# jinlinyi/PerspectiveFields

Measured on AMD Instinct MI355X. Metric: images/sec (640x640, Paramnet-360Cities), higher is better.
Workload: dtype f32 (operands fp32 in HBM; contractions as 2-way fp16 split on the MFMA, fp32 accumulate, fp32-class accuracy); 1 GPU; BASELINE configs[2]: batch 32/GPU 640x640 Paramnet-360Cities-edina-centered, fields + ParamNet, 320x320 network inputs resident in HBM (4 distinct synthetic images tiled over the batch; the network is data independent), post-process to 640x640; global_batch=32, parallelism=dp1 (images sharded, all-gather of ParamNet scalars), weights=seeded synthetic checkpoint (no network for the trained .pth), precision=fp32, tiles=shipped tile table + static heuristic (no tuning), gathered_param_rows=32

## Files before the change

include/pf_hip.h:

```cpp
#ifndef PF_HIP_H
#define PF_HIP_H

#include <stddef.h>
#include <stdint.h>

#ifdef __cplusplus
extern "C" {
#endif

typedef struct pf_engine* pf_handle;

enum pf_status {
  PF_OK = 0,
  PF_ERR_ARG = -1,
  PF_ERR_DEVICE = -2,
  PF_ERR_WEIGHTS = -3,
  PF_ERR_WORKSPACE = -4
};

enum pf_arch {
  PF_ARCH_PARAMNET_CENTERED = 0,
  PF_ARCH_PERSNET_CLS = 1,
  PF_ARCH_PARAMNET_UNCENTERED = 2
};

#define PF_NET_SIZE 320
#define PF_PARAMS_STRIDE 8
#define PF_MAX_BATCH 81

const char* pf_version(void);
const char* pf_build_digest(void);
const char* pf_last_error(pf_handle h);

#define PF_DEVICE_NONE (-1)
int pf_create(pf_handle* out, int device, int arch);
int pf_destroy(pf_handle h);

int pf_load_tensor(pf_handle h, const char* key, const float* h_data, const int64_t* shape, int rank);
int pf_finalize_weights(pf_handle h);

int pf_output_info(pf_handle h, int* gravity_channels, int* latitude_channels, int* param_raw_outputs);

int pf_max_batch(void);

size_t pf_workspace_bytes(pf_handle h, int batch);

#define PF_PRECISION_FP32 0
#define PF_PRECISION_FP32_BF16X6 3
int pf_set_precision(pf_handle h, int mode);

int pf_set_saturation_counter(pf_handle h, void* d_counter_u32);
int pf_static_window_max(pf_handle h, float* out);

int pf_forward_u8(pf_handle h, int batch, const uint8_t* d_images_u8, float* d_pred_gravity, float* d_pred_latitude,
                  float* d_params, void* d_workspace, size_t workspace_bytes, void* stream);
int pf_forward_f32(pf_handle h, int batch, const float* d_images_f32, float* d_pred_gravity, float* d_pred_latitude,
                   float* d_params, void* d_workspace, size_t workspace_bytes, void* stream);

int pf_set_defer_params(pf_handle h, int on);
int pf_join_params(pf_handle h, void* stream);

int pf_forward_u8_graph(pf_handle h, int batch, const uint8_t* d_images_u8, float* d_pred_gravity, float* d_pred_latitude,
                        float* d_params, void* d_workspace, size_t workspace_bytes, void* stream);

size_t pf_resize_workspace_bytes(int H, int W);
int pf_resize_bilinear_u8(pf_handle h, const uint8_t* d_img, int H, int W, uint8_t* d_out_320, void* d_workspace,
                          size_t workspace_bytes, void* stream);

int pf_resize_batch_u8(pf_handle h, int batch, const uint8_t* const* h_imgs, const int32_t* h_hw, uint8_t* d_out_320,
                       void* d_workspace, size_t workspace_bytes, void* stream);

size_t pf_autotune_workspace_bytes(pf_handle h, int batch);
int pf_autotune(pf_handle h, int batch, const uint8_t* d_images_u8, float* d_pred_gravity, float* d_pred_latitude,
                float* d_params, void* d_workspace, size_t workspace_bytes, void* stream);
int pf_is_tuned(pf_handle h, int batch);
int pf_load_tile_table(pf_handle h, const char* path);
int pf_save_tile_table(pf_handle h, const char* path);

int pf_postprocess(pf_handle h, const float* d_pred_gravity, const float* d_pred_latitude, int H, int W,
                   float* d_up_out, float* d_lat_out, void* d_workspace, size_t workspace_bytes, void* stream);

#define PF_PROFILE_CLASSES 8
#define PF_PROFILE_LARGE_ONLY 0x80000000u
int pf_profile_begin(pf_handle h, unsigned class_mask);
int pf_profile_pause(pf_handle h);
int pf_profile_end(pf_handle h, double* ms, double* work, long* launches, int n);
int pf_profile_records(pf_handle h, int max_records, int* cat, double* work, float* ms, int* mnk);
#define PF_PROFILE_PHASES 5
#define PF_PHASE_BACKBONE 0
#define PF_PHASE_LOW_LEVEL 1
#define PF_PHASE_DECODERS 2
#define PF_PHASE_PARAMNET 3
#define PF_PHASE_POSTPROCESS 4
int pf_profile_phases(pf_handle h, int n, double* ms);

size_t pf_debug_tap_bytes(pf_handle h, int batch);
int pf_debug_forward_u8(pf_handle h, int batch, const uint8_t* d_in_u8, float* d_pred_gravity, float* d_pred_latitude, float* d_params, void* d_workspace,
                        size_t workspace_bytes, int flags, void* d_tap_buf, size_t tap_bytes, void* stream);
int pf_debug_taps(pf_handle h, int max_records, char* names , long long* byte_offsets, int* shapes );
int pf_debug_ranges(pf_handle h, int max_records, char* names , long long* elems, float* stats );

#define PF_DISPATCH_BATCH 0
#define PF_DISPATCH_S3_SPLIT_TAKEN 1
#define PF_DISPATCH_RB_LAUNCHES 2
#define PF_DISPATCH_SPLITK_LAUNCHES 3
#define PF_DISPATCH_SPLITK_MAX_FACTOR 4
#define PF_DISPATCH_WINO_LAUNCHES 5
#define PF_DISPATCH_WINO_HALF_LAUNCHES 6
#define PF_DISPATCH_THIN128_LAUNCHES 7
#define PF_DISPATCH_ATTN64_LAUNCHES 8
#define PF_DISPATCH_MIT_MLP_FUSED_LAUNCHES 9
#define PF_DISPATCH_LN_KERNEL_LAUNCHES 10
#define PF_DISPATCH_CONV_LAUNCHES 11
#define PF_DISPATCH_SB_TENSORS 12
#define PF_DISPATCH_FORKS 13
#define PF_DISPATCH_FORK_ALLOC_CONFLICTS 14
#define PF_DISPATCH_REAL_PEAK_BYTES 15
#define PF_DISPATCH_DRY_PEAK_BYTES 16
#define PF_DISPATCH_CNX_RB_LAUNCHES 17
#define PF_DISPATCH_COLS 18
int pf_last_dispatch(pf_handle h, int64_t* out, int n);

int pf_postprocess_batch(pf_handle h, int batch, const float* d_pred_gravity, const float* d_pred_latitude, const int32_t* h_hw,
                         float* const* h_up_out, float* const* h_lat_out, void* d_workspace, size_t workspace_bytes, void* stream);

int pf_fields_from_params(int device, const float* d_cam5, int H, int W, float* d_up, float* d_lat, void* stream);

#define PF_FIT_COL_ROLL 0
#define PF_FIT_COL_PITCH 1
#define PF_FIT_COL_VFOV 2
#define PF_FIT_COL_REL_FOCAL 3
#define PF_FIT_COL_GENERAL_VFOV 4
#define PF_FIT_COL_REL_CX 5
#define PF_FIT_COL_REL_CY 6
#define PF_FIT_COL_RMS_UP 7
#define PF_FIT_COL_RMS_LAT 8
#define PF_FIT_COL_COST 9
#define PF_FIT_COL_ITERATIONS 10
#define PF_FIT_COL_CONVERGED 11
#define PF_FIT_COL_VALID_PIXELS 12
#define PF_FIT_COLS 13
#define PF_FIT_LOSS_L2 0
#define PF_FIT_LOSS_HUBER 1
size_t pf_fit_camera_workspace_bytes(int batch, const int32_t* h_hw);
int pf_fit_camera(int device, int batch, const int32_t* h_hw, const float* const* h_up, const float* const* h_lat, const float* d_init,
                  int free_pp, int loss, float huber_delta_deg, float w_up, float w_lat, int max_iter, float* d_out, void* d_workspace,
                  size_t workspace_bytes, void* stream);

#define PF_USMFIT_COL_ROLL 0
#define PF_USMFIT_COL_PITCH 1
#define PF_USMFIT_COL_VFOV 2
#define PF_USMFIT_COL_REL_FOCAL 3
#define PF_USMFIT_COL_GENERAL_VFOV 4
#define PF_USMFIT_COL_REL_CX 5
#define PF_USMFIT_COL_REL_CY 6
#define PF_USMFIT_COL_RMS_UP 7
#define PF_USMFIT_COL_RMS_LAT 8
#define PF_USMFIT_COL_COST 9
#define PF_USMFIT_COL_ITERATIONS 10
#define PF_USMFIT_COL_CONVERGED 11
#define PF_USMFIT_COL_VALID_PIXELS 12
#define PF_USMFIT_COL_XI 13
#define PF_USMFIT_COLS 14
size_t pf_fit_camera_usm_workspace_bytes(int batch, const int32_t* h_hw);
int pf_fit_camera_usm(int device, int batch, const int32_t* h_hw, const float* const* h_up, const float* const* h_lat,
                      const float* d_init , int free_pp, int loss, float huber_delta_deg, float w_up, float w_lat,
                      int max_iter, float* d_out , void* d_workspace, size_t workspace_bytes, void* stream);

int pf_fields_from_params_usm(int device, const float* d_cam6, int H, int W, float* d_up, float* d_lat, void* stream);

#define PF_PANO_U8 0
#define PF_PANO_F32 1
int pf_pano_crop(int device, int n_pano, const void* const* h_pano, const int32_t* h_pano_hw , int dtype, int batch,
                 const int32_t* h_pano_index , const float* d_cam7 , int H, int W,
                 void* d_img , float* d_up , float* d_lat , void* stream);

#define PF_FERR_COL_UP_MEAN 0
#define PF_FERR_COL_UP_MEDIAN 1
#define PF_FERR_COL_UP_RMSE 2
#define PF_FERR_COL_UP_MAX 3
#define PF_FERR_COL_UP_FRAC_BELOW 4
#define PF_FERR_COL_LAT_MEAN 5
#define PF_FERR_COL_LAT_MEDIAN 6
#define PF_FERR_COL_LAT_RMSE 7
#define PF_FERR_COL_LAT_MAX 8
#define PF_FERR_COL_LAT_FRAC_BELOW 9
#define PF_FERR_COL_VALID_PIXELS 10
#define PF_FERR_COLS 11
#define PF_FERR_BINS 11520
#define PF_FERR_BINS_PER_DEG 64
#define PF_FERR_SUM_N 0
#define PF_FERR_SUM_E 1
#define PF_FERR_SUM_E2 2
#define PF_FERR_SUM_MAX 3
#define PF_FERR_SUM_BELOW 4
#define PF_FERR_SUMS 5
size_t pf_field_errors_workspace_bytes(int batch, const int32_t* h_hw);
int pf_field_errors(int device, int batch, const int32_t* h_hw, const float* const* h_up_pred, const float* const* h_lat_pred,
                    const float* const* h_up_gt, const float* const* h_lat_gt, float threshold_deg, double* d_out, float* const* h_err_up,
                    float* const* h_err_lat, int64_t* d_hist, double* d_hist_sums, void* d_workspace, size_t workspace_bytes, void* stream);

int pf_op_set_saturation_watch(void* d_counter_u32, float limit);
int pf_op_conv2d(int device, const float* d_x, const float* d_x2, int B, int H, int W, int C1, int C2,
                 const float* h_weight , const float* h_bias ,
                 int Cout, int KH, int KW, int stride, int pad, int act ,
                 const float* d_res1, const float* d_res2, int post_relu, int nchw_out, int tile_id ,
                 float* d_y ,
                 const uint16_t* d_x_planes , long x_plane_elems, const uint16_t* d_x2_planes, long x2_plane_elems,
                 uint16_t* d_y_planes, long y_plane_elems, int precision , void* stream);
int pf_op_linear_ln(int device, const float* d_x, long rows, int K, const float* h_weight , const float* h_bias, const float* h_gamma, const float* h_beta,
                    float eps, int N, int act, const float* d_res1, int tile_id, float* d_y, int precision, void* stream);
int pf_op_rb_linear(int device, const float* d_x, long rows, int tokens, int K, const float* h_weight , const float* h_bias, const float* h_gamma, const float* h_beta,
                    float eps, int N, int act, const float* d_res, float* d_y, int iters, float* ms_out, void* stream);
int pf_op_rb_proj_fc1(int device, const float* d_attn, float* d_x, int B, int tokens, int C, const float* h_proj_w, const float* h_proj_b, const float* h_ln2_gamma,
                      const float* h_ln2_beta, float eps, const float* h_fc1_w, const float* h_fc1_b, float* d_hidden, int iters, float* ms_out, void* stream);
int pf_op_mit_attn64(int device, const float* d_x, const float* d_kv, float* d_y, int B, int N, int M, const float* h_ln1_gamma, const float* h_ln1_beta, float eps,
                     const float* h_q_w, const float* h_q_b, const float* h_proj_w, const float* h_proj_b, int iters, float* ms_out, void* stream);
int pf_op_stem7x7(int device, const float* d_x, float* d_y, int B, int H, int W, int stride, const float* h_weight, const float* h_bias, int relu, const float* h_ln_gamma,
                  const float* h_ln_beta, float eps, int iters, float* ms_out, void* stream);
int pf_op_thin128(int device, const float* d_x, long rows, const float* h_weight, const float* h_bias, const float* d_res, float* d_y, int iters, float* ms_out, void* stream);
int pf_op_rb_srkv(int device, const float* d_x, int B, int Hr, int Wr, int C, const float* h_ln1_gamma, const float* h_ln1_beta, float eps1, const float* h_sr_w,
                  const float* h_sr_b, const float* h_srn_gamma, const float* h_srn_beta, float eps2, const float* h_kv_w, const float* h_kv_b, float* d_kv, int iters,
                  float* ms_out, void* stream);
int pf_op_cnx_mlp(int device, const float* d_d, float* d_y, long rows, int C, const float* h_w1, const float* h_b1, const float* h_ln_gamma, const float* h_ln_beta,
                  float eps, const float* h_w2, const float* h_b2, const float* h_layer_scale, int iters, float* ms_out, void* stream);
int pf_op_mit_mlp(int device, const float* d_x, float* d_y, int B, int Hs, int Ws, int C, const float* h_fc1_w, const float* h_fc1_b, const float* h_ln_gamma,
                  const float* h_ln_beta, float eps, const float* h_dw_w, const float* h_dw_b, const float* h_fc2_w, const float* h_fc2_b, int iters, float* ms_out, void* stream);
int pf_op_conv2d_bench(int device, int B, int H, int W, int Cin, int Cout, int K, int stride, int pad, int tile_id, int iters, int fmt_prec, float* ms_out);
int pf_op_split_bf16(int device, const float* d_x, long n, uint16_t* d_planes, long plane_elems, void* stream);
int pf_op_merge_bf16(int device, const uint16_t* d_planes, long plane_elems, long n, float* d_y, void* stream);
int pf_op_dwconv3x3_bench(int device, int variant, int B, int H, int W, int C, int iters, float* ms_out);
int pf_op_layernorm(int device, const float* d_x, const float* h_gamma, const float* h_beta, float* d_y, long rows, int C, float eps,
                    uint16_t* d_y_planes, long plane_elems, void* stream);
int pf_op_dwconv3x3_gelu(int device, const float* d_x, const float* h_weight , const float* h_bias, float* d_y, int B, int H, int W, int C,
                         uint16_t* d_y_planes, long plane_elems, void* stream);
int pf_op_dwconv3x3_gelu_cfg(int device, const float* d_x, const float* h_weight, const float* h_bias, float* d_y, int B, int H, int W, int C,
                             uint16_t* d_y_planes, long plane_elems, int variant, void* stream);
int pf_op_dwconv7x7(int device, const float* d_x, const float* h_weight , const float* h_bias, float* d_y, int B, int H, int W, int C, void* stream);
int pf_op_dwconv7x7_cfg(int device, const float* d_x, const float* h_weight, const float* h_bias, float* d_y, int B, int H, int W, int C,
                        int variant, int nc, int nb, int th, void* stream);
int pf_op_dwconv7x7_bench(int device, int variant, int nc, int nb, int th, int B, int H, int W, int C, int iters, float* ms_out);
int pf_op_sr_attention(int device, const float* d_q, const float* d_kv, float* d_out, int B, int N, int M, int heads,
                       uint16_t* d_out_planes, long plane_elems, void* stream);
int pf_op_sr_attention_variant(int device, int variant, const float* d_q, const float* d_kv, float* d_out, int B, int N, int M, int heads,
                               int iters, float* ms_out, void* stream);
int pf_op_upsample2x(int device, const float* d_x, float* d_y, int B, int H, int W, int C, uint16_t* d_y_planes, long plane_elems, void* stream);
int pf_op_num_conv_tiles(void);
const char* pf_op_conv_tile_name(int tile_id);

#ifdef __cplusplus
}
#endif
#endif
```

perspectivefields_amd/csrc/engine.hip:

```cpp
#include <hip/hip_runtime.h>

#include <algorithm>
#include <cmath>
#include <cstdarg>
#include <cstdio>
#include <cstdlib>
#include <cstring>
#include <map>
#include <string>
#include <unordered_map>
#include <vector>

#include "../../include/pf_hip.h"
#include "pf_kernels.h"

using namespace pf;

namespace {

}
namespace pf_host { thread_local std::string g_create_error; }
#include "host_pack.h"
using namespace pf_host;
namespace {
// ... 125 lines not shown
  bool on = false;
  unsigned mask = 0xffffffffu;
  double min_work = 0.0;
  hipEvent_t get() {
    if (used == pool.size()) { hipEvent_t e; if (hipEventCreate(&e) != hipSuccess) return nullptr; pool.push_back(e); }
    return pool[used++];
  }
  struct Mark { int phase; hipEvent_t e; };
  std::vector<Mark> marks;
  void mark(int phase, hipStream_t s) {
    if (!on || min_work > 0.0) return;
    hipEvent_t e = get();
    if (!e) return;
    (void)hipEventRecord(e, s);
    marks.push_back({phase, e});
  }
  void reset() { recs.clear(); marks.clear(); used = 0; }
  ~Profiler() { for (hipEvent_t e : pool) (void)hipEventDestroy(e); }
};
struct ProfScope {
  Profiler* p; hipStream_t s; hipEvent_t b = nullptr;
  ProfScope(Profiler* pr, hipStream_t st, int cat, double work, int m = 0, int n = 0, int k = 0, int kh = 0) : p(pr), s(st) {
    if (!p || !p->on || !((p->mask >> cat) & 1u) || work < p->min_work) { p = nullptr; return; }
    hipEvent_t a = p->get(); b = p->get();
    if (!a || !b) { p = nullptr; return; }
    (void)hipEventRecord(a, s);
    p->recs.push_back({cat, work, a, b, m, n, k, kh, 0.f});
  }
  ~ProfScope() { if (p) (void)hipEventRecord(b, s); }
};

struct ResizeTable { int ksize = 0; std::vector<int> bounds, kk; int *d_bounds = nullptr, *d_kk = nullptr; };
void resize_coeffs(int in_size, int out_size, ResizeTable* t) {
  const double scale = (double)in_size / out_size;
  const double filterscale = scale < 1.0 ? 1.0 : scale;
  const double support = 1.0 * filterscale;
  const int ksize = (int)std::ceil(support) * 2 + 1;
  t->ksize = ksize;
  t->bounds.assign((size_t)out_size * 2, 0);
  t->kk.assign((size_t)out_size * ksize, 0);
  std::vector<double> k(ksize);
  const double ss = 1.0 / filterscale;
  for (int xx = 0; xx < out_size; ++xx) {
    const double center = (xx + 0.5) * scale;
    double ww = 0.0;
    int xmin = (int)(center - support + 0.5);
    if (xmin < 0) xmin = 0;
    int xmax = (int)(center + support + 0.5);
    if (xmax > in_size) xmax = in_size;
    xmax -= xmin;
    for (int x = 0; x < ksize; ++x) k[x] = 0.0;
    for (int x = 0; x < xmax; ++x) {
      double v = (x + xmin - center + 0.5) * ss;
      if (v < 0.0) v = -v;
      const double w = v < 1.0 ? 1.0 - v : 0.0;
      k[x] = w;
      ww += w;
    }
    for (int x = 0; x < xmax; ++x)
      if (ww != 0.0) k[x] /= ww;
    for (int x = 0; x < ksize; ++x)
      t->kk[(size_t)xx * ksize + x] = k[x] < 0 ? (int)(-0.5 + k[x] * (1 << 22)) : (int)(0.5 + k[x] * (1 << 22));
    t->bounds[2 * xx] = xmin;
    t->bounds[2 * xx + 1] = xmax;
  }
}

}

struct pf_engine {
  int device = 0;
  int arch = 0;
  bool finalized = false;
  std::string err;
  std::unordered_map<std::string, HostTensor> host;
  std::vector<void*> dev_allocs;
  std::map<int, size_t> ws_cache;
  Profiler prof;
  bool autotune = false;
  std::map<std::vector<int>, int> tile_cache;
  std::map<int, bool> tuned_batches;
  std::map<int, ResizeTable> resize_tables;
  std::map<int, size_t> scratch_off, scratch_elems;
  bool split_bf16 = true;
  bool fuse_pred = true;
  bool fuse_upsample = true;
  bool fuse_ln = true;
  int thin128 = 25600;
  int stem7 = 1;
  unsigned short* ll_s7_w = nullptr; float* ll_s7_tab = nullptr; unsigned short* pe_s7_w = nullptr; float* pe_s7_tab = nullptr;
  int attn64 = 1;
  int s3_split = 1;
  int side_stream_mode = 1;
  hipStream_t side = nullptr, side2 = nullptr;
  hipEvent_t ev_fork = nullptr, ev_join = nullptr, ev_ll = nullptr;
  bool host_only = false;
  int defer_params = 0;
  hipStream_t pstream = nullptr;
  hipEvent_t ev_pn_in = nullptr, ev_pn_done = nullptr;
  bool pn_pending = false, in_capture = false;
  int pn_pending_B = 0; uintptr_t pn_pending_base = 0;
  int defer_at = 0, defer_prio = 0;
  struct PnLater { bool armed = false; int B = 0; const float* pn = nullptr; float* params = nullptr; Ctx ctx; } pn_later;
  void issue_deferred() {
    if (!pn_later.armed) return;
    pn_later.armed = false;
    paramnet(pn_later.ctx, pn_later.B, pn_later.pn, pn_later.params);
    (void)hipEventRecord(ev_pn_done, pstream);
  }
  std::map<int, size_t> pn_off;
  bool pstream_ready() {
    if (pstream) return true;
    int lo = 0, hi = 0;
    (void)hipDeviceGetStreamPriorityRange(&lo, &hi);
    const int prio = defer_prio > 0 ? hi : (defer_prio < 0 ? lo : 0);
    if ((defer_prio ? hipStreamCreateWithPriority(&pstream, hipStreamNonBlocking, prio) : hipStreamCreateWithFlags(&pstream, hipStreamNonBlocking)) != hipSuccess) { pstream = nullptr; return false; }
    if (hipEventCreateWithFlags(&ev_pn_in, hipEventDisableTiming) != hipSuccess || hipEventCreateWithFlags(&ev_pn_done, hipEventDisableTiming) != hipSuccess) {
      (void)hipStreamDestroy(pstream); pstream = nullptr; return false;
    }
    return true;
  }
  bool ll_forked = false;
  bool side_ready() {
    if (side && (side2 || side_stream_mode < 2)) return true;
    if (!side) {
      if (hipStreamCreateWithFlags(&side, hipStreamNonBlocking) != hipSuccess) { side = nullptr; return false; }
      if (hipEventCreateWithFlags(&ev_fork, hipEventDisableTiming) != hipSuccess || hipEventCreateWithFlags(&ev_join, hipEventDisableTiming) != hipSuccess ||
          hipEventCreateWithFlags(&ev_ll, hipEventDisableTiming) != hipSuccess) return false;
    }
    if (side_stream_mode >= 2 && !side2 && hipStreamCreateWithFlags(&side2, hipStreamNonBlocking) != hipSuccess) { side2 = nullptr; return false; }
    return true;
  }
  struct ForkWin { bool open = false, side_alloced = false; size_t nalloc0 = 0; };
  ForkWin fw_q, fw_ll;
  Ctx fork_open(Ctx& c, hipStream_t s, ForkWin& w) {
    Ctx c2 = c;
    c2.s = s;
    w.open = true; w.side_alloced = false; w.nalloc0 = c.nalloc;
    c.count(PF_DISPATCH_FORKS);
    return c2;
  }
  void fork_side_done(ForkWin& w, const Ctx& c2) { w.side_alloced = c2.nalloc > w.nalloc0; }
  void fork_join(Ctx& c, ForkWin& w) {
    if (!w.open) return;
    if (w.side_alloced && c.nalloc > w.nalloc0) c.count(PF_DISPATCH_FORK_ALLOC_CONFLICTS);
    w.open = false;
  }
  int64_t dispatch[PF_DISPATCH_COLS] = {};
  int splitk_mode = -1;
  int wino_half = 1;
  bool can_fork(const Ctx& c) { return side_stream_mode && !c.dry && !c.tuning && (!c.prof || c.prof->min_work > 0.0) && side_ready(); }
  bool sba_heads = false;
  int rb_chain = 60;
  int rb_min_blocks = 192;
  int num_cus = 256;
  int wino_min_hw = 20;
  int wino_min_blocks = 96;
  int wino_tile = -1;
  unsigned* d_sat = nullptr;
  float static_window_max = 0.f;
  int mit_mlp128 = 4;
  bool fuse_mit_mlp = true;
  bool fuse_cnx_mlp = true;
  int cnx_rb = 1;
  int cnx_rb_min_blocks[2] = {96, 192};
  bool fold_mlp = true;
  int nterms = NT_F16X3;
  DebugSink dbg;
  DebugSink* debug_sink = nullptr;
  struct GraphEntry { std::vector<uintptr_t> key; hipGraphExec_t exec; };
  std::vector<GraphEntry> graphs;
  bool sba = false;

  MitStage stages[4];
  ConvW ll;
  Head heads[2];
  Cnx cnx;
  bool has_param = false;
  int param_in = NET;
  float mean3[3] = {103.53f, 116.28f, 123.675f};
  float std3[3] = {1.f, 1.f, 1.f};

  int fail(int code, const std::string& m) { err = m; return code; }

  ResizeTable* resize_table(int in_size) {
    auto it = resize_tables.find(in_size);
    if (it != resize_tables.end()) return &it->second;
    ResizeTable& t = resize_tables[in_size];
    resize_coeffs(in_size, NET, &t);
    void *db = nullptr, *dk = nullptr;
    if (hipMalloc(&db, t.bounds.size() * 4) != hipSuccess || hipMalloc(&dk, t.kk.size() * 4) != hipSuccess) return nullptr;
    if (hipMemcpy(db, t.bounds.data(), t.bounds.size() * 4, hipMemcpyHostToDevice) != hipSuccess ||
        hipMemcpy(dk, t.kk.data(), t.kk.size() * 4, hipMemcpyHostToDevice) != hipSuccess) return nullptr;
    dev_allocs.push_back(db); dev_allocs.push_back(dk);
    t.d_bounds = static_cast<int*>(db); t.d_kk = static_cast<int*>(dk);
    return &t;
  }
  float* upload(const std::vector<float>& v) {
    void* d = nullptr;
    if (host_only) {
      d = malloc(v.size() * sizeof(float) + 1);
      if (!d) throw std::string("malloc failed for weights");
      std::memcpy(d, v.data(), v.size() * sizeof(float));
      dev_allocs.push_back(d);
      return static_cast<float*>(d);
    }
    if (hipMalloc(&d, v.size() * sizeof(float)) != hipSuccess) throw std::string("hipMalloc failed for weights");
    if (hipMemcpy(d, v.data(), v.size() * sizeof(float), hipMemcpyHostToDevice) != hipSuccess) throw std::string("hipMemcpy H2D failed for weights");
    dev_allocs.push_back(d);
    return static_cast<float*>(d);
  }
  unsigned short* upload_u16(const std::vector<unsigned short>& v) {
    void* d = nullptr;
    if (host_only) {
      d = malloc(v.size() * 2 + 1);
      if (!d) throw std::string("malloc failed for weights");
      std::memcpy(d, v.data(), v.size() * 2);
      dev_allocs.push_back(d);
      return static_cast<unsigned short*>(d);
    }
    if (hipMalloc(&d, v.size() * 2) != hipSuccess) throw std::string("hipMalloc failed for weights");
    if (hipMemcpy(d, v.data(), v.size() * 2, hipMemcpyHostToDevice) != hipSuccess) throw std::string("hipMemcpy H2D failed for weights");
    dev_allocs.push_back(d);
    return static_cast<unsigned short*>(d);
  }
  void upload_conv_weights(ConvW& c, const std::vector<float>& packed, int CinP, int Cout) {
    c.w = upload(packed);
    if (split_bf16 && (CinP % 32 == 0 || CinP == 4)) {
      c.wsb = upload_u16(split_bf16x3(packed));
      const F16Planes f = split_f16x2(packed, Cout);
      c.wh16 = upload_u16(f.planes);
      c.wh16_inv = upload(f.inv_scale);
    }
  }
  const HostTensor& get(const std::string& key, std::initializer_list<int64_t> shape) {
    auto it = host.find(key);
    if (it == host.end()) throw fmt("missing checkpoint tensor '%s'", key.c_str());
    HostTensor& t = it->second;
    if (t.shape != std::vector<int64_t>(shape)) {
      std::string got, want;
      for (auto d : t.shape) got += std::to_string(d) + ",";
      for (auto d : shape) want += std::to_string(d) + ",";
      throw fmt("shape mismatch for '%s': got (%s) expected (%s)", key.c_str(), got.c_str(), want.c_str());
    }
    t.used = true;
    return t;
  }
  ConvW make_conv(const std::string& wkey, const std::string& bkey, int Cout, int Cin, int K, int stride, int pad,
                  const double* out_scale = nullptr, const std::vector<float>* bias_override = nullptr) {
    ConvW c;
    const int CinP = roundup(Cin, 4);
    const HostTensor& w = get(wkey, {Cout, Cin, K, K});
    const std::vector<float> packed = pack_conv(w.data.data(), Cout, Cin, K, K, CinP, out_scale, &c.KWC, &c.KWCp);
    upload_conv_weights(c, packed, CinP, Cout);
    if (bias_override) c.b = upload(*bias_override);
    else if (!bkey.empty()) {
      std::vector<float> b = get(bkey, {Cout}).data;
      if (out_scale) for (int n = 0; n < Cout; ++n) b[n] = (float)(b[n] * out_scale[n]);
      c.b = upload(b);
    }
    c.Cout = Cout; c.Cin = CinP; c.CinReal = Cin; c.KH = c.KW = K; c.stride = stride; c.pad = pad;
    if (wino_min_hw > 0 && split_bf16 && K == 3 && stride == 1 && pad == 1 && CinP % 64 == 0 && Cout % 64 == 0 && c.KWCp == c.KWC) {
      std::vector<unsigned short> planes;
      std::vector<float> inv;
      wino_pack_weights(packed.data(), Cout, CinP, c.KWCp, &planes, &inv);
      c.wwino = upload_u16(planes);
      c.wwino_inv = upload(inv);
    }
    return c;
  }
  ConvW make_linear(const std::string& pfx, int N, int K, const double* out_scale = nullptr, const std::string& ln_pfx = "", float ln_eps = 0.f) {
    ConvW c;
    const HostTensor& w = get(pfx + ".weight", {N, K});
    std::vector<float> b = get(pfx + ".bias", {N}).data;
    if (!ln_pfx.empty() && fuse_ln && K % 32 == 0 && N % 4 == 0) {
      const std::vector<float>& g = get(ln_pfx + ".weight", {K}).data;
      const std::vector<float>& be = get(ln_pfx + ".bias", {K}).data;
      std::vector<float> wf, bf, cs;
      fold_ln_linear(w.data.data(), b.data(), g.data(), be.data(), N, K, &wf, &bf, &cs);
      b = bf;
      upload_conv_weights(c, pack_conv(wf.data(), N, K, 1, 1, K, nullptr, &c.KWC, &c.KWCp), K, N);
      c.ln_s = upload(cs);
      c.ln_eps = ln_eps;
    } else {
      upload_conv_weights(c, pack_conv(w.data.data(), N, K, 1, 1, K, out_scale, &c.KWC, &c.KWCp), K, N);
      if (out_scale) for (int n = 0; n < N; ++n) b[n] = (float)(b[n] * out_scale[n]);
    }
    c.b = upload(b);
    c.Cout = N; c.Cin = K; c.CinReal = K; c.KH = c.KW = 1; c.stride = 1; c.pad = 0;
    return c;
  }
  ConvW make_folded(const std::string& lin, const std::string& proc, int C) {
    const HostTensor& wl = get(lin + ".weight", {DEC_EMBED, C});
    const HostTensor& bl = get(lin + ".bias", {DEC_EMBED});
    const HostTensor& wp = get(proc + ".weight", {DEC_FEAT, DEC_EMBED, 3, 3});
    const HostTensor& bp = get(proc + ".bias", {DEC_FEAT});
    std::vector<float> wf((size_t)DEC_FEAT * C * 9);
    std::vector<double> T((size_t)DEC_FEAT * 9), acc(C);
    std::vector<double> wld(wl.data.begin(), wl.data.end());
    for (int o = 0; o < DEC_FEAT; ++o)
      for (int t = 0; t < 9; ++t) {
        std::fill(acc.begin(), acc.end(), 0.0);
        double tb = 0.0;
        for (int e = 0; e < DEC_EMBED; ++e) {
          const double a = wp.data[((size_t)o * DEC_EMBED + e) * 9 + t];
          const double* row = &wld[(size_t)e * C];
// ... 385 lines not shown
      std::vector<int> key = {p.M, p.Cout, p.KH, p.KW, p.Cin, p.stride, p.H, p.W, ngroups, p.nchw_out, fmt_bits + 512 * p.ln, p.act};
      auto it = tile_cache.find(key);
      if (it == tile_cache.end() && p.ln && !(c.tuning && c.tune_scratch)) { key[10] = fmt_bits; it = tile_cache.find(key); }
      if (it != tile_cache.end()) tile = it->second;
      else if (c.tuning && c.tune_scratch) { tile = tune_conv(p, c); tile_cache[key] = tile; }
    }
    if (!conv_tile_usable(p, tile)) tile = conv_default_tile(p);
    if (wino_min_hw > 0 && wino_tile >= 0 && !(c.tuning && c.tune_scratch) && p.Ho >= wino_min_hw && p.Wo >= wino_min_hw && conv_tile_usable(p, wino_tile) &&
        conv_wino_blocks(p) >= wino_min_blocks) tile = wino_tile;
    if (c.dbg && c.dbg->range) {
      const int q = c.dbg->seq++;
      for (int g = 0; g < ngroups; ++g) {
        const std::string nm = fmt("dense%03d%s %dx%d s%d %s%sM=%d N=%d K=%d", q, ngroups > 1 ? (g ? "[latitude]" : "[gravity]") : "", w.KH, w.KW, w.stride, w.ln_s ? "LN-fused " : "", tile >= 0 && strncmp(conv_tile_name(tile), "wino", 4) == 0 ? "[winograd] " : "", p.M, p.Cout, w.KH * w.KW * w.CinReal);
        range_in(c, nm + " x", calls[g].x.f, (size_t)B * (ups ? H / 2 : H) * (ups ? W / 2 : W) * p.C1);
        if (p.C2 > 0) range_in(c, nm + " x2", calls[g].x2.f, (size_t)B * H * W * p.C2);
      }
    }
    ProfScope ps(c.prof, c.s, conv_tile_is_sb(tile) ? PC_IGEMM_SB : PC_IGEMM, 2.0 * ngroups * p.M * (double)w.Cout * w.KH * w.KW * w.CinReal, p.M * ngroups, w.Cout, w.KH * w.KW * w.CinReal, w.KH);
    c.count(PF_DISPATCH_CONV_LAUNCHES);
    launch_conv_tile(p, tile, c.s);
  }
  int tune_conv(const ConvParams& p0, Ctx& c) {
    ConvParams p = p0;
    const size_t out_elems = (size_t)p.M * p.Cout;
    unsigned short* sb_scratch = reinterpret_cast<unsigned short*>(c.tune_scratch + c.tune_scratch_elems);
    for (int g = 0; g < p.groups; ++g) {
      if (p.g[g].y) p.g[g].y = c.tune_scratch + g * out_elems;
      if (p.g[g].y_sb) p.g[g].y_sb = sb_scratch + g * out_elems;
    }
    p.y_sb_plane = (c.tune_scratch_elems & ~(size_t)1) | (p0.y_sb_plane & 1);
    hipEvent_t a, b;
    if (hipEventCreate(&a) != hipSuccess || hipEventCreate(&b) != hipSuccess) return -1;
    int best = -1;
    float best_ms = 1e30f;
    for (int t = 0; t < conv_num_tiles(); ++t) {
      if (!conv_tile_usable(p, t)) continue;
      if (strncmp(conv_tile_name(t), "sbhA", 4) == 0 || strncmp(conv_tile_name(t), "sbhLA", 5) == 0 || strncmp(conv_tile_name(t), "sbhDMA", 6) == 0 || strncmp(conv_tile_name(t), "sbhREG", 6) == 0 || strncmp(conv_tile_name(t), "sbhV", 4) == 0 || strncmp(conv_tile_name(t), "sbA", 3) == 0 || strncmp(conv_tile_name(t), "sbPI_", 5) == 0 || strncmp(conv_tile_name(t), "sbI_", 4) == 0) continue;
      if (strncmp(conv_tile_name(t), "wino", 4) == 0) continue;
      if (conv_tile_bn(t) > 32 && p.Cout <= 32) continue;
      if ((long)conv_tile_bm(t) * conv_tile_bn(t) > 16L * p.M * p.Cout) continue;
      launch_conv_tile(p, t, c.s);
      float ms = 1e30f;
      bool ok = true;
      for (int rep = 0; rep < 2 && ok; ++rep) {
        (void)hipEventRecord(a, c.s);
        launch_conv_tile(p, t, c.s);
        launch_conv_tile(p, t, c.s);
        (void)hipEventRecord(b, c.s);
        ok = hipEventSynchronize(b) == hipSuccess;
        float w = 0.f;
        if (ok) { (void)hipEventElapsedTime(&w, a, b); ms = std::min(ms, w); }
      }
      if (!ok) break;
      if (ms < best_ms) { best_ms = ms; best = t; }
    }
    (void)hipEventDestroy(a); (void)hipEventDestroy(b);
    return best;
  }
  void conv(Ctx& c, const ConvW& w, Ten x, int B, int H, int W, Ten y, int act = ACT_NONE, const float* res1 = nullptr,
            const float* res2 = nullptr, int post_relu = 0, Ten x2 = Ten(), int C1 = -1, int nchw = 0) {
    ConvCall one{&w, x, y, res1, res2, x2};
    conv_g(c, 1, &one, B, H, W, act, post_relu, C1, nchw);
  }
  void gemm(Ctx& c, const ConvW& w, Ten x, long rows, Ten y, int act = ACT_NONE, const float* res1 = nullptr) {
    conv(c, w, x, 1, (int)rows, 1, y, act, res1);
  }
  void ln(Ctx& c, const LNW& l, const float* x, Ten y, long rows) {
    if (c.dry) return;
    c.count(PF_DISPATCH_LN_KERNEL_LAUNCHES);
    ProfScope ps(c.prof, c.s, PC_LAYERNORM, (4.0 + (y.f ? 4.0 : 0.0) + (y.s.p ? 6.0 : 0.0)) * rows * l.C);
    launch_layernorm(x, l.g, l.b, y.f, rows, l.C, l.eps, c.s, y.s.p, y.s.plane);
  }

  void rb_linear(Ctx& c, const RbLin& r, const float* x, long M, int tokens, float* y, const LNW* lnw = nullptr, int act = ACT_NONE, const float* res = nullptr) {
    range_in(c, fmt("rb_linear %d->%d%s", r.K, r.N, lnw ? " (LN input)" : ""), x, (size_t)M * r.K);
    if (c.dry) return;
    RbLinArgs a;
    a.x = x; a.ln_g = lnw ? lnw->g : nullptr; a.ln_b = lnw ? lnw->b : nullptr; a.ln_eps = lnw ? lnw->eps : 0.f;
    a.w = r.w; a.w_bytes = r.bytes; a.inv = r.inv; a.bias = r.b; a.res = res; a.y = y;
    a.M = (int)M; a.tokens = tokens; a.bpi = (tokens + 63) / 64; a.N = r.N; a.act = act;
    a.sat = d_sat; a.sat_limit = r.sat_limit;
    ProfScope ps(c.prof, c.s, PC_IGEMM_SB, 2.0 * M * (double)r.N * r.K, (int)M, r.N, r.K, 1);
    c.count(PF_DISPATCH_RB_LAUNCHES);
    launch_rb_linear(a, r.K, c.s);
  }

  void thin(Ctx& c, const unsigned short* wfr, const float* tab, const float* x, const float* res, float* y, long M, float sat_limit, const char* what) {
    range_in(c, fmt("thin128 %s x", what), x, (size_t)M * 128);
    if (c.dry) return;
    ThinLinArgs a;
    a.x = x; a.res = res; a.y = y; a.wfr = wfr; a.tab = tab; a.M = M; a.sat = d_sat; a.sat_limit = sat_limit;
    ProfScope ps(c.prof, c.s, PC_IGEMM_SB, 2.0 * M * 128.0 * 128.0, (int)M, 128, 128, 1);
    c.count(PF_DISPATCH_THIN128_LAUNCHES);
    launch_thin128(a, num_cus, c.s);
  }

  void stem(Ctx& c, const unsigned short* wfr, const float* tab, const float* x4, float* y, int B, int H, int W, int stride, bool relu, bool lnorm, float eps, float sat_limit, const char* what) {
    range_in(c, fmt("stem7x7 s%d %s x", stride, what), x4, (size_t)B * H * W * 4);
    if (c.dry) return;
    Stem7Args a;
    a.x = x4; a.y = y; a.wfr = wfr; a.tab = tab; a.B = B; a.H = H; a.W = W; a.stride = stride; a.Ho = (H + 6 - 7) / stride + 1; a.Wo = (W + 6 - 7) / stride + 1;
    a.relu = relu ? 1 : 0; a.ln = lnorm ? 1 : 0; a.ln_eps = eps; a.sat = lnorm ? nullptr : d_sat; a.sat_limit = sat_limit;
    const long M = (long)B * a.Ho * a.Wo;
    ProfScope ps(c.prof, c.s, PC_IGEMM_SB, 2.0 * M * 64.0 * 147.0, (int)M, 64, 147, 7);
    launch_stem7x7(a, num_cus, c.s);
  }

  void mit(Ctx& c, int B, const float* x0, Ten feats[4], const Ten* llf = nullptr) {
    const bool S = sba;
    Ten cur(const_cast<float*>(x0));
    int H = NET, W = NET;
    for (int s = 0; s < 4; ++s) {
      MitStage& st = stages[s];
      if (!c.dry && pn_later.armed && s + 1 == defer_at) issue_deferred();
      const int C = MIT_DIMS[s], heads_n = MIT_HEADS[s], sr = MIT_SR[s];
      const int Ho = (H + 2 * MIT_PP[s] - MIT_PK[s]) / MIT_PS[s] + 1, Wo = (W + 2 * MIT_PP[s] - MIT_PK[s]) / MIT_PS[s] + 1;
      const long N = (long)Ho * Wo, M = (long)B * N;
      float* x = c.alloc(M * C);
      const bool fused_mlp = !st.blocks.empty() && st.blocks[0].mlp_w && nterms == NT_F16X3 && (C != 128 || B >= mit_mlp128);
      float* xalt = fused_mlp ? c.alloc(M * C) : nullptr;
      const SbT xs = S ? c.alloc_sb(M * C) : SbT();
      if (s == 2 && llf && B >= 4 && side_stream_mode >= 2 && can_fork(c)) {
        (void)hipEventRecord(ev_ll, c.s);
        (void)hipStreamWaitEvent(side2, ev_ll, 0);
        Ctx c2 = fork_open(c, side2, fw_ll);
        conv(c2, ll, Ten(const_cast<float*>(x0)), B, NET, NET, *llf, ACT_RELU);
        (void)hipEventRecord(ev_ll, side2);
        fork_side_done(fw_ll, c2);
        ll_forked = true;
      }
      if (s == 0 && pe_s7_w && nterms == NT_F16X3 && !c.tuning && cur.f) {
        stem(c, pe_s7_w, pe_s7_tab, cur.f, x, B, H, W, MIT_PS[s], false, true, st.pen.eps, 65504.f, "patch_embed1 + norm");
      } else {
        conv(c, st.pe, cur, B, H, W, Ten(x));
        ln(c, st.pen, x, Ten(x), M);
      }
      const size_t mk = c.mark();
      const int kvh = Ho / sr, kvw = Wo / sr;
      const long Mkv = (long)B * kvh * kvw;
      const Ten xn = c.ten(M * C, !S, S);
      float* qb = c.alloc(M * C);
      const Ten ab = c.ten(M * C, !S, S);
      float* srb = c.alloc(Mkv * C);
      const Ten srn = S ? Ten(nullptr, c.alloc_sb(Mkv * C)) : Ten(srb);
      float* kvb = c.alloc(Mkv * 2 * C);
      float* hb = c.alloc(M * 4 * C);
      const Ten h2 = c.ten(M * 4 * C, !S, S);
      auto one_block = [&](Ctx& c, MitBlock& mb, int blk, int B, long M, long Mkv, float*& x, float*& xalt, const Ten& xn, float* qb, const Ten& ab, float* srb, const Ten& srn,
                           float* kvb, float* hb, const Ten& h2, int gate_B, bool may_fork) {
        const bool thin_q = mb.tq_w && M >= thin128 && nterms == NT_F16X3 && !S && !c.tuning && xn.f;
        const bool fuse64 = attn64 && mb.a64_w && nterms == NT_F16X3 && !S && !c.tuning && sr > 1;
        const long rb_blocks = (long)gate_B * ((N + 63) / 64);
        const bool use_rb = rb_chain && mb.rq.w && nterms == NT_F16X3 && !S && !c.tuning && rb_blocks >= rb_min_blocks && (rb_blocks % num_cus == 0 || rb_blocks % num_cus >= num_cus * 3 / 4);
        if (sr > 1 && use_rb && (rb_chain & 32) && mb.rsrkv.w && mb.qln.ln_s && fuse_ln) {
          const bool fork = B >= 4 && (may_fork && can_fork(c));
          if (fork) {
            (void)hipEventRecord(ev_fork, c.s);
            (void)hipStreamWaitEvent(side, ev_fork, 0);
            Ctx c2 = fork_open(c, side, fw_q);
            gemm(c2, mb.qln, Ten(x), M, Ten(qb));
            (void)hipEventRecord(ev_join, side);
            fork_side_done(fw_q, c2);
          } else {
            gemm(c, mb.qln, Ten(x), M, Ten(qb));
          }
          range_in(c, fmt("rb_srkv s%d.b%d x (LN-fused)", s + 1, blk), x, (size_t)M * C);
          if (!c.dry) {
            RbSrKvArgs a;
            a.x = x; a.ln1_g = mb.n1.g; a.ln1_b = mb.n1.b; a.ln1_eps = mb.n1.eps;
            a.w = mb.rsrkv.w; a.w_bytes = mb.rsrkv.bytes; a.sr_inv = mb.rsrkv.sr_inv; a.sr_bias = mb.rsrkv.sr_b;
            a.srn_g = mb.srn.g; a.srn_b = mb.srn.b; a.srn_eps = mb.srn.eps; a.kv_inv = mb.rsrkv.kv_inv; a.kv_bias = mb.rsrkv.kv_b;
            a.kv = kvb; a.B = B; a.Hr = kvh; a.Wr = kvw; a.bpi = (kvh * kvw + 31) / 32; a.sat = d_sat;
            ProfScope ps(c.prof, c.s, PC_IGEMM_SB, 2.0 * Mkv * (double)C * (sr * sr * C + 2 * C), (int)Mkv, 3 * C, sr * sr * C + 2 * C, sr);
            c.count(PF_DISPATCH_RB_LAUNCHES);
            launch_rb_srkv(a, C, c.s);
          }
        } else if (sr > 1 && fuse64) {
          ln(c, mb.n1, x, xn, M);
          conv(c, mb.sr, xn, B, Ho, Wo, Ten(srb));
          if (mb.kv.ln_s) {
            gemm(c, mb.kv, Ten(srb), Mkv, Ten(kvb));
          } else {
            ln(c, mb.srn, srb, srn, Mkv);
            gemm(c, mb.kv, srn, Mkv, Ten(kvb));
          }
        } else if (sr > 1) {
          const bool fork = B >= 4 && (may_fork && can_fork(c));
          if (use_rb && (rb_chain & 1) && fork) {
            (void)hipEventRecord(ev_fork, c.s);
            (void)hipStreamWaitEvent(side, ev_fork, 0);
            Ctx c2 = fork_open(c, side, fw_q);
            rb_linear(c2, mb.rq, x, M, (int)N, qb, &mb.n1);
            (void)hipEventRecord(ev_join, side);
            fork_side_done(fw_q, c2);
          }
          ln(c, mb.n1, x, xn, M);
          if (use_rb && (rb_chain & 1)) {
            if (!fork) rb_linear(c, mb.rq, x, M, (int)N, qb, &mb.n1);
          } else if (fork) {
            (void)hipEventRecord(ev_fork, c.s);
            (void)hipStreamWaitEvent(side, ev_fork, 0);
            Ctx c2 = fork_open(c, side, fw_q);
            if (thin_q) thin(c2, mb.tq_w, mb.tq_tab, xn.f, nullptr, qb, M, mb.q.sat_limit, "q"); else gemm(c2, mb.q, xn, M, Ten(qb));
            (void)hipEventRecord(ev_join, side);
            fork_side_done(fw_q, c2);
          } else {
            if (thin_q) thin(c, mb.tq_w, mb.tq_tab, xn.f, nullptr, qb, M, mb.q.sat_limit, "q"); else gemm(c, mb.q, xn, M, Ten(qb));
          }
          conv(c, mb.sr, xn, B, Ho, Wo, Ten(srb));
          if (use_rb && (rb_chain & 2)) {
            rb_linear(c, mb.rkv, srb, Mkv, kvh * kvw, kvb, &mb.srn);
          } else if (mb.kv.ln_s) {
            gemm(c, mb.kv, Ten(srb), Mkv, Ten(kvb));
          } else {
            ln(c, mb.srn, srb, srn, Mkv);
            gemm(c, mb.kv, srn, Mkv, Ten(kvb));
          }
        } else if (mb.q.ln_s && mb.kv.ln_s) {
          if (B >= 4 && (may_fork && can_fork(c))) {
            (void)hipEventRecord(ev_fork, c.s);
            (void)hipStreamWaitEvent(side, ev_fork, 0);
            Ctx c2 = fork_open(c, side, fw_q);
            gemm(c2, mb.q, Ten(x), M, Ten(qb));
            (void)hipEventRecord(ev_join, side);
            fork_side_done(fw_q, c2);
          } else {
            gemm(c, mb.q, Ten(x), M, Ten(qb));
          }
          gemm(c, mb.kv, Ten(x), M, Ten(kvb));
        } else {
          ln(c, mb.n1, x, xn, M);
          gemm(c, mb.q, xn, M, Ten(qb));
          gemm(c, mb.kv, xn, M, Ten(kvb));
        }
        if (!fuse64 && B >= 4 && (sr > 1 || (mb.q.ln_s && mb.kv.ln_s)) && (may_fork && can_fork(c))) (void)hipStreamWaitEvent(c.s, ev_join, 0);
        if (may_fork) fork_join(c, fw_q);
        if (c.dbg && c.dbg->range) {
          if (!fuse64) range_in(c, fmt("attention s%d.b%d q", s + 1, blk), qb, (size_t)M * C);
          range_in(c, fmt("attention s%d.b%d kv", s + 1, blk), kvb, (size_t)Mkv * 2 * C);
        }
        if (fuse64) {
          range_in(c, fmt("mit_attn64 s%d.b%d x (LN-fused)", s + 1, blk), x, (size_t)M * C);
          if (!c.dry) {
            MitAttn64Args a;
            a.x = x; a.kv = kvb; a.y = x; a.wfr = mb.a64_w; a.tab = mb.a64_tab; a.B = B; a.N = (int)N; a.M = kvh * kvw; a.ln_eps = mb.n1.eps; a.sat = d_sat; a.sat_limit = mb.proj.sat_limit;
            ProfScope ps(c.prof, c.s, PC_ATTN, 4.0 * M * C * (double)C + 4.0 * M * C * (kvh * kvw));
            c.count(PF_DISPATCH_ATTN64_LAUNCHES);
            launch_mit_attn64(a, num_cus, c.s);
          }
        }
        const bool pf_fused = !fuse64 && use_rb && (rb_chain & 64) && mb.rpf.w;
        if (!fuse64) {
        if (!c.dry) {
          ProfScope ps(c.prof, c.s, PC_ATTN, 4.0 * M * C * (kvh * kvw));
          launch_sr_attention(qb, kvb, ab.f, B, (int)N, kvh * kvw, heads_n, c.s, ab.s.p, ab.s.plane);
        }
        if (pf_fused) {
          range_in(c, fmt("rb_proj_fc1 s%d.b%d attn", s + 1, blk), ab.f, (size_t)M * C);
          if (!c.dry) {
            RbProjFc1Args a;
            a.attn = ab.f; a.x = x; a.w = mb.rpf.w; a.w_bytes = mb.rpf.bytes; a.proj_inv = mb.rproj.inv; a.proj_bias = mb.rproj.b;
            a.ln2_g = mb.n2.g; a.ln2_b = mb.n2.b; a.ln2_eps = mb.n2.eps; a.fc1_inv = mb.rfc1.inv; a.fc1_bias = mb.rfc1.b; a.hidden = hb;
            a.B = B; a.tokens = (int)N; a.bpi = ((int)N + 63) / 64; a.sat = d_sat; a.sat_limit = mb.rproj.sat_limit; a.hidden_limit = mb.rfc1.sat_limit;
            ProfScope ps(c.prof, c.s, PC_IGEMM_SB, 2.0 * M * (double)C * 5 * C, (int)M, 5 * C, C, 1);
            c.count(PF_DISPATCH_RB_LAUNCHES);
            launch_rb_proj_fc1(a, C, c.s);
          }
        } else if (use_rb && (rb_chain & 4)) rb_linear(c, mb.rproj, ab.f, M, (int)N, x, nullptr, ACT_NONE, x);
        else if (thin_q && mb.tp_w && ab.f) thin(c, mb.tp_w, mb.tp_tab, ab.f, x, x, M, mb.proj.sat_limit, "proj");
        else gemm(c, mb.proj, ab, M, Ten(x), ACT_NONE, x);
        }
        if (fused_mlp && mb.mlp_w) {
          range_in(c, fmt("mit_mlp s%d.b%d x (LN-fused)", s + 1, blk), x, (size_t)M * C);
          if (!c.dry) {
            ProfScope ps(c.prof, c.s, PC_IGEMM_SB, 2.0 * 2.0 * M * (double)C * 4 * C, (int)M, C, 8 * C, 9);
            c.count(PF_DISPATCH_MIT_MLP_FUSED_LAUNCHES);
            launch_mit_mlp(x, xalt, mb.mlp_w, mb.mlp_tab, B, Ho, Wo, C, mb.n2.eps, c.s, d_sat, 65504.f);
          }
          std::swap(x, xalt);
          return;
        }
        if (pf_fused) {
        } else if (use_rb && (rb_chain & 8)) {
          rb_linear(c, mb.rfc1, x, M, (int)N, hb, &mb.n2);
        } else if (mb.fc1.ln_s) {
          gemm(c, mb.fc1, Ten(x), M, Ten(hb));
        } else {
          ln(c, mb.n2, x, xn, M);
          gemm(c, mb.fc1, xn, M, Ten(hb));
        }
        if (!c.dry) {
          ProfScope ps(c.prof, c.s, PC_DW3, (4.0 + (h2.f ? 4.0 : 0.0) + (h2.s.p ? 6.0 : 0.0)) * M * 4 * C);
          launch_dwconv3x3_gelu(hb, mb.dw.w, mb.dw.b, h2.f, B, Ho, Wo, 4 * C, c.s, h2.s.p, h2.s.plane);
        }
        if (use_rb && (rb_chain & 16)) rb_linear(c, mb.rfc2, h2.f, M, (int)N, x, nullptr, ACT_NONE, x);
        else gemm(c, mb.fc2, h2, M, Ten(x), ACT_NONE, x);
            };
      const long rb_all = (long)B * ((N + 63) / 64), rb_half = rb_all / 2;
      auto rb_gate = [&](long nb) { return nb >= rb_min_blocks && (nb % num_cus == 0 || nb % num_cus >= num_cus * 3 / 4); };
      bool split = s3_split && s == 2 && sr > 1 && !S && !fused_mlp && B >= 16 && B % 2 == 0 && !c.dry && !c.dbg && !c.tuning && !st.blocks.empty() && rb_chain && nterms == NT_F16X3 &&
                         st.blocks[0].rq.w && rb_gate(rb_all) && (s3_split >= 2 || rb_gate(rb_half)) && can_fork(c);
      if (split) {
        Ctx probe = c;
        probe.dry = true; probe.rep = nullptr;
        float *px = x, *none = nullptr;
        one_block(probe, st.blocks[0], 0, B / 2, M / 2, Mkv / 2, px, none, xn, qb, ab, srb, srn, kvb, hb, h2, B, false);
        if (probe.nalloc != c.nalloc) split = false;
      }
      int blk = -1;
      if (split) {
        const int Bh = B / 2;
        const long Mh = M / 2, Mkvh = Mkv / 2;
        c.count(PF_DISPATCH_S3_SPLIT_TAKEN);
        (void)hipEventRecord(ev_fork, c.s);
        (void)hipStreamWaitEvent(side, ev_fork, 0);
        Ctx c2 = fork_open(c, side, fw_q);
        float* x2 = x + Mh * C;
        float* none = nullptr;
        for (MitBlock& mb : st.blocks) {
          ++blk;
          one_block(c, mb, blk, Bh, Mh, Mkvh, x, none, xn, qb, ab, srb, srn, kvb, hb, h2, B, false);
          one_block(c2, mb, blk, Bh, Mh, Mkvh, x2, none, Ten(xn.f ? xn.f + Mh * C : nullptr), qb + Mh * C, Ten(ab.f + Mh * C), srb + Mkvh * C, Ten(srn.f ? srn.f + Mkvh * C : nullptr),
                    kvb + Mkvh * 2 * C, hb + Mh * 4 * C, Ten(h2.f + Mh * 4 * C), B, false);
        }
        (void)hipEventRecord(ev_join, side);
        (void)hipStreamWaitEvent(c.s, ev_join, 0);
        fork_side_done(fw_q, c2);
        fork_join(c, fw_q);
      } else {
        for (MitBlock& mb : st.blocks) {
          if (blk >= 0) tap(c, fmt("mit.s%d.b%d", s + 1, blk), x, B, Ho, Wo, C);
          ++blk;
          one_block(c, mb, blk, B, M, Mkv, x, xalt, xn, qb, ab, srb, srn, kvb, hb, h2, B, true);
        }
      }
      c.release(mk);
      if (blk >= 0) tap(c, fmt("mit.s%d.b%d", s + 1, blk), x, B, Ho, Wo, C);
      ln(c, st.norm, x, Ten(x, xs), M);
      tap(c, fmt("c%d", s + 1), x, B, Ho, Wo, C);
      feats[s] = Ten(x, xs);
      cur = feats[s];
      H = Ho; W = Wo;
    }
  }

  bool pred_fused() const { return fuse_pred && arch != PF_ARCH_PERSNET_CLS && nterms == NT_F16X3 && split_bf16; }
  void heads_fwd(Ctx& c, int B, Ten feats[4], Ten llf, float* t32 , float* pg, float* pl, float* pn) {
    const bool S = sba && nterms != NT_F16X3;
    const bool SR = S || (sba_heads && !sba && nterms == NT_F16X3 && split_bf16);
    Head& hg = heads[0];
    Head& hl = heads[1];
    auto pair = [&](size_t per_head, bool want_f32, bool want_sb, Ten& a, Ten& b) {
      a = Ten(); b = Ten();
      if (want_f32) { a.f = c.alloc(2 * per_head); b.f = a.f + per_head; }
      if (want_sb) { a.s = c.alloc_sb(2 * per_head); b.s = a.s; b.s.p = a.s.p + per_head; }
    };
    const bool fuse_up = fuse_upsample && nterms == NT_F16X3 && split_bf16 && !S;
    Ten up[4][2], qfin[2];
    for (int k = 3; k >= 0; --k) {
      const int h = NET >> (k + 2);
      if (k == 0 && fuse_up) pair((size_t)B * h * h * DEC_FEAT, true, false, qfin[0], qfin[1]);
      else pair((size_t)B * 4 * h * h * DEC_FEAT, !(S && k == 0), S && k == 0, up[k][0], up[k][1]);
    }
    for (int k = 3; k >= 0; --k) {
      const int h = NET >> (k + 2);
      const size_t M = (size_t)B * h * h;
      const size_t mk = c.mark();
      Ten p0, p1;
      pair(M * DEC_FEAT, true, SR, p0, p1);
      if (fold_mlp) {
        ConvCall cc[2] = {{&hg.fold[k], feats[k], p0}, {&hl.fold[k], feats[k], p1}};
        conv_g(c, 2, cc, B, h, h, ACT_NONE, 1);
      } else {
        Ten e0, e1;
        pair(M * DEC_EMBED, !S, S, e0, e1);
        ConvCall l[2] = {{&hg.lin[k], feats[k], e0}, {&hl.lin[k], feats[k], e1}};
        conv_g(c, 2, l, 1, (int)M, 1);
        ConvCall cc[2] = {{&hg.proc[k], e0, p0}, {&hl.proc[k], e1, p1}};
        conv_g(c, 2, cc, B, h, h, ACT_NONE, 1);
      }
      Ten o0 = p0, o1 = p1;
      if (k < 3) {
        Ten t0, t1;
        pair(M * DEC_FEAT, !SR, SR, t0, t1);
        ConvCall a[2] = {{&hg.r1c1[k], p0, t0}, {&hl.r1c1[k], p1, t1}};
        conv_g(c, 2, a, B, h, h, ACT_RELU);
        pair(M * DEC_FEAT, true, SR, o0, o1);
        ConvCall b2[2] = {{&hg.r1c2[k], t0, o0, p0.f, up[k + 1][0].f}, {&hl.r1c2[k], t1, o1, p1.f, up[k + 1][1].f}};
// ... 139 lines not shown
    else conv(c, ll, Ten(x0), B, NET, NET, llf, ACT_RELU);
    tap(c, "ll", llf.f, B, NET / 2, NET / 2, LL_CH);
    const bool pf = pred_fused();
    float* tg = pf ? nullptr : c.alloc((size_t)2 * B * NET * NET * 32);
    float* tl = pf ? nullptr : tg + (size_t)B * NET * NET * 32;
    Ctx cp = c;
    cp.off = 0; cp.peak = 0;
    if (!c.dry) cp.base = c.base + pn_off[B];
    float* pn = has_param ? cp.alloc((size_t)B * NET * NET * 4) : nullptr;
    if (!c.dry && pn_pending) {
      issue_deferred();
      (void)hipStreamWaitEvent(c.s, ev_pn_done, 0);
      pn_pending = false;
    }
    const size_t mk = c.mark();
    if (!c.dry && c.prof) c.prof->mark(PH_DECODERS, c.s);
    heads_fwd(c, B, feats, llf, tg, pg, pl, pn);
    c.release(mk);
    if (arch == PF_ARCH_PERSNET_CLS) {
      conv(c, heads[0].predcls, Ten(tg), B, NET, NET, Ten(pg), ACT_NONE, nullptr, nullptr, 0, Ten(), -1, 1);
      conv(c, heads[1].predcls, Ten(tl), B, NET, NET, Ten(pl), ACT_NONE, nullptr, nullptr, 0, Ten(), -1, 1);
      if (!c.dry && c.prof) c.prof->mark(PH_END, c.s);
      return;
    }
    if (!c.dry && !pf)
      launch_pred_regression(tg, tl, heads[0].predw, heads[0].predb, heads[1].predw, heads[1].predb, pg, pl, pn, B, NET * NET, c.s);
    if (!c.dry && c.prof) c.prof->mark(has_param ? PH_PARAMNET : PH_END, c.s);
    if (has_param) {
      const bool defer = defer_params && !c.dry && (!c.prof || c.prof->min_work > 0.0) && !c.dbg && !c.tuning && !in_capture && pstream_ready();
      if (defer) {
        (void)hipEventRecord(ev_pn_in, c.s);
        (void)hipStreamWaitEvent(pstream, ev_pn_in, 0);
        cp.s = pstream;
      }
      if (defer && defer_at > 0) {
        pn_later.armed = true; pn_later.B = B; pn_later.pn = pn; pn_later.params = params; pn_later.ctx = cp;
        pn_pending = true; pn_pending_B = B; pn_pending_base = c.base;
      } else {
        paramnet(cp, B, pn, params);
        if (defer) {
          (void)hipEventRecord(ev_pn_done, pstream);
          pn_pending = true; pn_pending_B = B; pn_pending_base = c.base;
        }
      }
    }
    if (!c.dry && c.prof && has_param) c.prof->mark(PH_END, c.s);
    run_pn_peak = cp.peak;
    if (cp.max_conv_out > c.max_conv_out) c.max_conv_out = cp.max_conv_out;
  }
  size_t run_pn_peak = 0;
  std::map<int, size_t> pn_peak;

  size_t workspace_bytes(int B, bool with_scratch = false) {
    auto it = ws_cache.find(B);
    if (it == ws_cache.end()) {
      Ctx c{nullptr, 4096, 0, 0, true, nullptr};
      c.sb_planes = nterms == NT_F16X3 ? 2 : 3;
      run(c, B, nullptr, true, nullptr, nullptr, nullptr);
      const size_t main_peak = (c.peak + 255) & ~(size_t)255, total = main_peak + ((run_pn_peak + 255) & ~(size_t)255);
      pn_off[B] = main_peak;
      pn_peak[B] = (run_pn_peak + 255) & ~(size_t)255;
      ws_cache[B] = total + 4096;
      scratch_off[B] = total;
      scratch_elems[B] = c.max_conv_out;
      it = ws_cache.find(B);
    }
    return it->second + ((with_scratch || autotune) ? scratch_elems[B] * 10 + 4096 : 0);
  }
  int forward(int B, const void* in, bool is_u8, float* pg, float* pl, float* params, void* ws, size_t ws_bytes, hipStream_t s, bool tune = false) {
    if (host_only) return fail(PF_ERR_DEVICE, "this engine was created with PF_DEVICE_NONE (host side only): no forward");
    if (!finalized) return fail(PF_ERR_WEIGHTS, "pf_forward called before pf_finalize_weights");
    if (B <= 0 || !in || !pg || !pl || !ws) return fail(PF_ERR_ARG, "pf_forward: null pointer or batch <= 0");
    if (has_param && !params) return fail(PF_ERR_ARG, "pf_forward: d_params is required for a ParamNet architecture");
    if (B > PF_MAX_BATCH) return fail(PF_ERR_ARG, fmt("pf_forward: batch %d exceeds PF_MAX_BATCH = %d (32-bit byte offsets inside one activation); split the batch", B, PF_MAX_BATCH));
    const size_t need = workspace_bytes(B, tune);
    if (ws_bytes < need) return fail(PF_ERR_WORKSPACE, fmt("workspace too small: %zu < %zu bytes", ws_bytes, need));
    if (hipSetDevice(device) != hipSuccess) return fail(PF_ERR_DEVICE, "hipSetDevice failed");
    uintptr_t base = (reinterpret_cast<uintptr_t>(ws) + 255) & ~(uintptr_t)255;
    Ctx c{s, base, 0, 0, false, nullptr};
    c.sb_planes = nterms == NT_F16X3 ? 2 : 3;
    c.prof = prof.on ? &prof : nullptr;
    c.dbg = debug_sink;
    if (tune) {
      c.tuning = true;
      c.tune_scratch = reinterpret_cast<float*>(base + scratch_off[B]);
      c.tune_scratch_elems = scratch_elems[B];
    }
    std::fill(dispatch, dispatch + PF_DISPATCH_COLS, (int64_t)0);
    if (!tune) c.rep = dispatch;
    const LaunchCounts lc0 = g_launch_counts;
    g_launch_counts.splitk_max = 0;
    fw_q.open = fw_ll.open = false;
    run(c, B, in, is_u8, pg, pl, params);
    const LaunchCounts lc1 = g_launch_counts;
    g_launch_counts.splitk_max = std::max(lc0.splitk_max, lc1.splitk_max);
    dispatch[PF_DISPATCH_BATCH] = B;
    dispatch[PF_DISPATCH_SPLITK_LAUNCHES] = lc1.splitk - lc0.splitk;
    dispatch[PF_DISPATCH_SPLITK_MAX_FACTOR] = lc1.splitk_max;
    dispatch[PF_DISPATCH_WINO_LAUNCHES] = lc1.wino - lc0.wino;
    dispatch[PF_DISPATCH_WINO_HALF_LAUNCHES] = lc1.wino_half - lc0.wino_half;
    const size_t real_main = (c.peak + 255) & ~(size_t)255, real_pn = (run_pn_peak + 255) & ~(size_t)255;
    dispatch[PF_DISPATCH_REAL_PEAK_BYTES] = (int64_t)(real_main + real_pn);
    dispatch[PF_DISPATCH_DRY_PEAK_BYTES] = (int64_t)(pn_off[B] + pn_peak[B]);
    const hipError_t e = hipGetLastError();
    if (e != hipSuccess) return fail(PF_ERR_DEVICE, fmt("kernel launch failed: %s", hipGetErrorString(e)));
    if (real_main > pn_off[B] || real_pn > pn_peak[B])
      return fail(PF_ERR_WORKSPACE, fmt("the forward allocated past what pf_workspace_bytes(%d) sized: main region %zu > %zu or ParamNet region %zu > %zu bytes (the launches were issued: the workspace and outputs of this call are not to be trusted)", B, real_main, pn_off[B], real_pn, pn_peak[B]));
    return PF_OK;
  }
};

static void tune_cache_load(pf_engine* h);
static void tune_cache_save(pf_engine* h);


extern "C" {

const char* pf_version(void) { return "pf_hip 0.2 (gfx950; split-f16 / split-bf16 / fp32 MFMA)"; }

#ifndef PF_BUILD_DIGEST
#define PF_BUILD_DIGEST "unknown"
#endif
const char* pf_build_digest(void) { return PF_BUILD_DIGEST; }

const char* pf_last_error(pf_handle h) { return h ? h->err.c_str() : g_create_error.c_str(); }

int pf_create(pf_handle* out, int device, int arch) {
  if (!out) { g_create_error = "pf_create: out is NULL"; return PF_ERR_ARG; }
  *out = nullptr;
  if (arch < 0 || arch > 2) { g_create_error = fmt("pf_create: unknown arch %d", arch); return PF_ERR_ARG; }
  const bool host_only = device == PF_DEVICE_NONE;
  if (!host_only) {
    const int rc = check_device(device, &g_create_error);
    if (rc != PF_OK) return rc;
  }
  pf_engine* e = new pf_engine();
  e->device = device;
  e->host_only = host_only;
  e->arch = arch;
  if (const char* v = getenv("PF_FOLD_MLP")) e->fold_mlp = atoi(v) != 0;
  if (const char* v = getenv("PF_FUSE_UPSAMPLE")) e->fuse_upsample = atoi(v) != 0;
  if (const char* v = getenv("PF_FUSE_PRED")) e->fuse_pred = atoi(v) != 0;
  if (const char* v = getenv("PF_FUSE_LN")) e->fuse_ln = atoi(v) != 0;
  if (const char* v = getenv("PF_FUSE_CNX_MLP")) e->fuse_cnx_mlp = atoi(v) != 0;
  if (const char* v = getenv("PF_FUSE_MIT_MLP")) e->fuse_mit_mlp = atoi(v) != 0;
  if (const char* v = getenv("PF_MIT_MLP_128")) e->mit_mlp128 = atoi(v);
  if (const char* v = getenv("PF_WINO")) e->wino_min_hw = atoi(v);
  if (const char* v = getenv("PF_WINO_MIN_BLOCKS")) e->wino_min_blocks = atoi(v);
  {
    const char* wt = getenv("PF_WINO_TILE");
    for (int t = 0; t < conv_num_tiles(); ++t) if (strcmp(conv_tile_name(t), wt ? wt : "wino256x64d") == 0) e->wino_tile = t;
  }
  if (const char* v = getenv("PF_RB_CHAIN")) e->rb_chain = atoi(v);
  if (const char* v = getenv("PF_DEFER_AT")) e->defer_at = atoi(v);
  if (const char* v = getenv("PF_DEFER_PRIO")) e->defer_prio = atoi(v);
  if (!host_only) {
    hipDeviceProp_t prop;
    if (hipGetDeviceProperties(&prop, device) == hipSuccess && prop.multiProcessorCount > 0) e->num_cus = prop.multiProcessorCount;
    e->rb_min_blocks = e->num_cus * 3 / 4;
  }
  if (const char* v = getenv("PF_RB_MIN_BLOCKS")) e->rb_min_blocks = atoi(v);
  if (const char* v = getenv("PF_CNX_RB")) e->cnx_rb = atoi(v);
  if (!host_only) { e->cnx_rb_min_blocks[0] = e->num_cus * 3 / 8; e->cnx_rb_min_blocks[1] = e->num_cus * 3 / 4; }
  if (const char* v = getenv("PF_CNX_RB_MIN_BLOCKS")) e->cnx_rb_min_blocks[0] = atoi(v);
  if (const char* v = getenv("PF_CNX_RB_MIN_BLOCKS_768")) e->cnx_rb_min_blocks[1] = atoi(v);
#ifdef PF_TUNING_BUILD
#endif
  if (const char* v = getenv("PF_SIDE_STREAM")) e->side_stream_mode = atoi(v);
  if (const char* v = getenv("PF_S3_SPLIT")) e->s3_split = atoi(v);
  if (const char* v = getenv("PF_ATTN64")) e->attn64 = atoi(v);
  if (const char* v = getenv("PF_STEM7")) e->stem7 = atoi(v);
  if (const char* v = getenv("PF_THIN128")) e->thin128 = atoi(v);
  if (const char* v = getenv("PF_SBA_HEADS")) e->sba_heads = atoi(v) != 0;
  if (const char* v = getenv("PF_AUTOTUNE")) e->autotune = atoi(v) != 0;
  if (const char* v = getenv("PF_SPLIT_BF16")) e->split_bf16 = atoi(v) != 0;
  if (const char* v = getenv("PF_SBA")) e->sba = atoi(v) != 0;
  e->splitk_mode = conv_splitk_env();
  e->wino_half = conv_wino_half_env();
  if (!e->split_bf16) e->sba = false;
  if (!e->split_bf16 || e->sba) e->fuse_ln = false;
  if (!e->split_bf16 || e->sba) e->fuse_cnx_mlp = false;
  if (!e->split_bf16 || e->sba) e->fuse_mit_mlp = false;
  if (!e->split_bf16 || e->sba) e->cnx_rb = 0;

  tune_cache_load(e);
  *out = e;
  return PF_OK;
}

int pf_set_precision(pf_handle h, int mode) {
  if (!h) return PF_ERR_ARG;
  if (mode != PF_PRECISION_FP32 && mode != PF_PRECISION_FP32_BF16X6) return h->fail(PF_ERR_ARG, "pf_set_precision: unknown mode (0 = FP32 split-f16, 3 = FP32_BF16X6; the reduced-precision modes 1 / 2 of earlier versions are gone)");
  if (mode != PF_PRECISION_FP32 && !h->split_bf16) return h->fail(PF_ERR_ARG, "pf_set_precision: this mode needs the split kernels (PF_SPLIT_BF16=0 is set)");
  if (h->pn_pending) { h->issue_deferred(); (void)hipStreamSynchronize(h->pstream); h->pn_pending = false; }
  h->ws_cache.clear();
  h->nterms = mode == PF_PRECISION_FP32_BF16X6 ? 6 : NT_F16X3;
  return PF_OK;
}

int pf_set_saturation_counter(pf_handle h, void* d_counter_u32) {
  if (!h) return PF_ERR_ARG;
  h->d_sat = static_cast<unsigned*>(d_counter_u32);
  return PF_OK;
}
int pf_static_window_max(pf_handle h, float* out) {
  if (!h || !out || !h->finalized) return PF_ERR_ARG;
  *out = h->static_window_max;
  return PF_OK;
}
int pf_set_defer_params(pf_handle h, int on) {
  if (!h) return PF_ERR_ARG;
  h->defer_params = on ? 1 : 0;
  return PF_OK;
}
int pf_join_params(pf_handle h, void* stream) {
  if (!h) return PF_ERR_ARG;
  if (h->pn_pending) h->issue_deferred();
  if (h->pn_pending && hipStreamWaitEvent(static_cast<hipStream_t>(stream), h->ev_pn_done, 0) != hipSuccess) return h->fail(PF_ERR_DEVICE, "pf_join_params: hipStreamWaitEvent failed");
  return PF_OK;
}

int pf_destroy(pf_handle h) {
  if (!h) return PF_ERR_ARG;
  if (h->host_only) {
    for (void* d : h->dev_allocs) free(d);
    delete h;
    return PF_OK;
  }
  (void)hipSetDevice(h->device);
  for (void* d : h->dev_allocs) (void)hipFree(d);
  if (h->dbg.stats) (void)hipFree(h->dbg.stats);
  for (auto& g : h->graphs) (void)hipGraphExecDestroy(g.exec);
  if (h->ev_fork) (void)hipEventDestroy(h->ev_fork);
  if (h->ev_join) (void)hipEventDestroy(h->ev_join);
  if (h->ev_ll) (void)hipEventDestroy(h->ev_ll);
  if (h->side) (void)hipStreamDestroy(h->side);
  if (h->side2) (void)hipStreamDestroy(h->side2);
  if (h->pstream) { (void)hipStreamSynchronize(h->pstream); (void)hipStreamDestroy(h->pstream); }
  if (h->ev_pn_in) (void)hipEventDestroy(h->ev_pn_in);
  if (h->ev_pn_done) (void)hipEventDestroy(h->ev_pn_done);
  delete h;
  return PF_OK;
}

int pf_load_tensor(pf_handle h, const char* key, const float* data, const int64_t* shape, int rank) {
  if (!h || !key || (!data && rank > 0) || rank < 0 || rank > 4) return h ? h->fail(PF_ERR_ARG, "pf_load_tensor: bad argument") : PF_ERR_ARG;
  if (h->finalized) return h->fail(PF_ERR_WEIGHTS, "pf_load_tensor after pf_finalize_weights");
  HostTensor t;
  size_t n = 1;
  for (int i = 0; i < rank; ++i) { if (shape[i] <= 0) return h->fail(PF_ERR_ARG, "pf_load_tensor: non-positive dim"); t.shape.push_back(shape[i]); n *= (size_t)shape[i]; }
  if (data) t.data.assign(data, data + n);
  h->host[key] = std::move(t);
  return PF_OK;
}

int pf_finalize_weights(pf_handle h) {
  if (!h) return PF_ERR_ARG;
  if (h->finalized) return h->fail(PF_ERR_WEIGHTS, "weights already finalized");
  if (!h->host_only && hipSetDevice(h->device) != hipSuccess) return h->fail(PF_ERR_DEVICE, "hipSetDevice failed");
  try {
    h->build();
  } catch (const std::string& m) {
    return h->fail(PF_ERR_WEIGHTS, m);
  }
  h->finalized = true;
  return PF_OK;
}

int pf_output_info(pf_handle h, int* g, int* l, int* p) {
  if (!h) return PF_ERR_ARG;
  const bool cls = h->arch == PF_ARCH_PERSNET_CLS;
  if (g) *g = cls ? 73 : 2;
  if (l) *l = cls ? 180 : 1;
  if (p) *p = cls ? 0 : 5;
  return PF_OK;
}

int pf_max_batch(void) { return PF_MAX_BATCH; }

int pf_last_dispatch(pf_handle h, int64_t* out, int n) {
  if (!h || !out || n < PF_DISPATCH_COLS) return h ? h->fail(PF_ERR_ARG, "pf_last_dispatch: the array must hold PF_DISPATCH_COLS entries") : PF_ERR_ARG;
  std::copy(h->dispatch, h->dispatch + PF_DISPATCH_COLS, out);
  return PF_OK;
}

size_t pf_workspace_bytes(pf_handle h, int batch) {
  if (!h || batch <= 0 || batch > PF_MAX_BATCH) return 0;
  const bool was = h->has_param;
  if (!h->finalized) {
    h->has_param = h->arch != PF_ARCH_PERSNET_CLS;
    h->param_in = h->arch == PF_ARCH_PARAMNET_UNCENTERED ? 64 : NET;
    for (int s = 0; s < 4; ++s)
      if (h->stages[s].blocks.empty()) h->stages[s].blocks.resize(MIT_DEPTHS[s]);
    if (h->has_param)
      for (int s = 0; s < 4; ++s)
        if (h->cnx.blocks[s].empty()) h->cnx.blocks[s].resize(CNX_DEPTHS[s]);
  }
  const size_t n = h->workspace_bytes(batch);
  if (!h->finalized) {
    h->has_param = was;
    for (int s = 0; s < 4; ++s) { h->stages[s].blocks.clear(); h->cnx.blocks[s].clear(); }
    h->ws_cache.clear();
  }
  return n;
}

// ... 541 lines not shown
```

perspectivefields_amd/csrc/engine_ops.hip:

```cpp
#include "host_pack.h"

using namespace pf;
using namespace pf_host;

static thread_local unsigned* t_op_sat = nullptr;
static thread_local float t_op_sat_limit = 65504.f;

extern "C" {

int pf_op_set_saturation_watch(void* d_counter_u32, float limit) {
  if (d_counter_u32 && !(limit > 0.f)) { g_create_error = "pf_op_set_saturation_watch: limit must be positive"; return PF_ERR_ARG; }
  t_op_sat = static_cast<unsigned*>(d_counter_u32);
  t_op_sat_limit = d_counter_u32 ? limit : 65504.f;
  return PF_OK;
}

int pf_op_num_conv_tiles(void) { return conv_num_tiles(); }
const char* pf_op_conv_tile_name(int id) { return conv_tile_name(id); }

int pf_op_conv2d(int device, const float* x, const float* x2, int B, int H, int W, int C1, int C2, const float* hw, const float* hb,
                 int Cout, int KH, int KW, int stride, int pad, int act, const float* res1, const float* res2, int post_relu,
                 int nchw_out, int tile_id, float* y, const uint16_t* x_planes, long x_plane_elems, const uint16_t* x2_planes,
                 long x2_plane_elems, uint16_t* y_planes, long y_plane_elems, int precision_flags, void* stream) {
  const int precision = precision_flags & 15;
// ... 169 lines not shown
    float t = 0.f;
    (void)hipEventElapsedTime(&t, e0, e1);
    *ms_out = t / iters;
    (void)hipEventDestroy(e0); (void)hipEventDestroy(e1);
  }
  rc = hipGetLastError() == hipSuccess ? PF_OK : PF_ERR_DEVICE;
  tmp.sync_free(s);
  return rc;
}

int pf_op_mit_attn64(int device, const float* x, const float* kv, float* y, int B, int N, int M, const float* ln_g, const float* ln_b, float eps, const float* q_w, const float* q_b,
                     const float* p_w, const float* p_b, int iters, float* ms_out, void* stream) {
  std::string err;
  int rc = check_device(device, &err);
  if (rc != PF_OK) { g_create_error = err; return rc; }
  if (!x || !kv || !y || !ln_g || !ln_b || !q_w || !q_b || !p_w || !p_b || B <= 0 || N <= 0 || !mit_attn64_supported(64, 1, M)) {
    g_create_error = "pf_op_mit_attn64: all operands required; 1 <= kv rows <= 128";
    return PF_ERR_ARG;
  }
  hipStream_t s = static_cast<hipStream_t>(stream);
  TmpDev tmp;
  std::vector<unsigned short> wfr;
  std::vector<float> tab;
  attn64_pack(ln_g, ln_b, q_w, q_b, p_w, p_b, &wfr, &tab);
  MitAttn64Args a;
  a.x = x; a.kv = kv; a.y = y; a.wfr = tmp.up_u16(wfr); a.tab = tmp.up(tab); a.B = B; a.N = N; a.M = M; a.ln_eps = eps;
  a.sat = t_op_sat; a.sat_limit = t_op_sat_limit;
  int cus = 256;
  { hipDeviceProp_t pr; if (hipGetDeviceProperties(&pr, device) == hipSuccess && pr.multiProcessorCount > 0) cus = pr.multiProcessorCount; }
  launch_mit_attn64(a, cus, s);
  a.sat = nullptr;
  if (iters > 0 && ms_out) {
    hipEvent_t e0, e1;
    (void)hipEventCreate(&e0); (void)hipEventCreate(&e1);
    (void)hipEventRecord(e0, s);
    for (int i = 0; i < iters; ++i) launch_mit_attn64(a, cus, s);
    (void)hipEventRecord(e1, s);
    (void)hipEventSynchronize(e1);
    float t = 0.f;
    (void)hipEventElapsedTime(&t, e0, e1);
    *ms_out = t / iters;
    (void)hipEventDestroy(e0); (void)hipEventDestroy(e1);
  }
  rc = hipGetLastError() == hipSuccess ? PF_OK : PF_ERR_DEVICE;
  tmp.sync_free(s);
  return rc;
}

int pf_op_stem7x7(int device, const float* x, float* y, int B, int H, int W, int stride, const float* w, const float* bias, int relu, const float* ln_g, const float* ln_b, float eps,
                  int iters, float* ms_out, void* stream) {
  std::string err;
  int rc = check_device(device, &err);
  if (rc != PF_OK) { g_create_error = err; return rc; }
  if (!x || !y || !w || B <= 0 || H <= 0 || W <= 0 || !stem7x7_supported(3, 64, 7, stride, 3) || ((ln_g == nullptr) != (ln_b == nullptr))) {
    g_create_error = "pf_op_stem7x7: x, y, weight required; stride 2 or 4; LayerNorm gamma and beta together";
    return PF_ERR_ARG;
  }
  hipStream_t s = static_cast<hipStream_t>(stream);
  TmpDev tmp;
  std::vector<unsigned short> wfr;
  std::vector<float> tab;
  stem7x7_pack(w, nullptr, bias, ln_g, ln_b, &wfr, &tab);
  Stem7Args a;
  a.x = x; a.y = y; a.wfr = tmp.up_u16(wfr); a.tab = tmp.up(tab); a.B = B; a.H = H; a.W = W; a.stride = stride;
  a.Ho = (H + 6 - 7) / stride + 1; a.Wo = (W + 6 - 7) / stride + 1; a.relu = relu; a.ln = ln_g ? 1 : 0; a.ln_eps = eps;
  a.sat = t_op_sat; a.sat_limit = t_op_sat_limit;
  int cus = 256;
  { hipDeviceProp_t pr; if (hipGetDeviceProperties(&pr, device) == hipSuccess && pr.multiProcessorCount > 0) cus = pr.multiProcessorCount; }
  launch_stem7x7(a, cus, s);
  a.sat = nullptr;
  if (iters > 0 && ms_out) {
    hipEvent_t e0, e1;
    (void)hipEventCreate(&e0); (void)hipEventCreate(&e1);
    (void)hipEventRecord(e0, s);
    for (int i = 0; i < iters; ++i) launch_stem7x7(a, cus, s);
    (void)hipEventRecord(e1, s);
    (void)hipEventSynchronize(e1);
    float t = 0.f;
    (void)hipEventElapsedTime(&t, e0, e1);
    *ms_out = t / iters;
    (void)hipEventDestroy(e0); (void)hipEventDestroy(e1);
  }
  rc = hipGetLastError() == hipSuccess ? PF_OK : PF_ERR_DEVICE;
  tmp.sync_free(s);
  return rc;
}

int pf_op_thin128(int device, const float* x, long rows, const float* w, const float* bias, const float* res, float* y, int iters, float* ms_out, void* stream) {
  std::string err;
  int rc = check_device(device, &err);
  if (rc != PF_OK) { g_create_error = err; return rc; }
  if (!x || !y || !w || rows <= 0) { g_create_error = "pf_op_thin128: x, y, weight required"; return PF_ERR_ARG; }
  hipStream_t s = static_cast<hipStream_t>(stream);
  TmpDev tmp;
  std::vector<unsigned short> wfr;
  std::vector<float> tab;
  thin128_pack(w, bias, &wfr, &tab);
  ThinLinArgs a;
  a.x = x; a.res = res; a.y = y; a.wfr = tmp.up_u16(wfr); a.tab = tmp.up(tab); a.M = rows;
  a.sat = t_op_sat; a.sat_limit = t_op_sat_limit;
  int cus = 256;
  { hipDeviceProp_t pr; if (hipGetDeviceProperties(&pr, device) == hipSuccess && pr.multiProcessorCount > 0) cus = pr.multiProcessorCount; }
  launch_thin128(a, cus, s);
  a.sat = nullptr;
  if (iters > 0 && ms_out) {
    hipEvent_t e0, e1;
    (void)hipEventCreate(&e0); (void)hipEventCreate(&e1);
    (void)hipEventRecord(e0, s);
    for (int i = 0; i < iters; ++i) launch_thin128(a, cus, s);
    (void)hipEventRecord(e1, s);
    (void)hipEventSynchronize(e1);
    float t = 0.f;
    (void)hipEventElapsedTime(&t, e0, e1);
    *ms_out = t / iters;
    (void)hipEventDestroy(e0); (void)hipEventDestroy(e1);
  }
  rc = hipGetLastError() == hipSuccess ? PF_OK : PF_ERR_DEVICE;
  tmp.sync_free(s);
  return rc;
}

int pf_op_rb_srkv(int device, const float* x, int B, int Hr, int Wr, int C, const float* ln1_g, const float* ln1_b, float eps1, const float* sr_w, const float* sr_b,
                  const float* srn_g, const float* srn_b, float eps2, const float* kv_w, const float* kv_b, float* kv, int iters, float* ms_out, void* stream) {
  std::string err;
  int rc = check_device(device, &err);
  if (rc != PF_OK) { g_create_error = err; return rc; }
  if (!rb_srkv_supported(C, 2) || !x || !kv || !ln1_g || !ln1_b || !sr_w || !sr_b || !srn_g || !srn_b || !kv_w || !kv_b || B <= 0 || Hr <= 0 || Wr <= 0) {
    g_create_error = "pf_op_rb_srkv: C must be 320 (2 x 2 spatial reduction); all weights required";
    return PF_ERR_ARG;
  }
  hipStream_t s = static_cast<hipStream_t>(stream);
  TmpDev tmp;
  int kwc = 0, kwcp = 0;
  const std::vector<float> srp = pack_conv(sr_w, C, C, 2, 2, C, nullptr, &kwc, &kwcp);
  std::vector<unsigned short> st1, st2;
  std::vector<float> inv1, inv2;
  rb_pack_w(srp.data(), C, 2 * kwcp, 320, &st1, &inv1);
  rb_pack_w(kv_w, 2 * C, C, 320, &st2, &inv2);
  st1.resize(st1.size() - (size_t)4 * 10 * 2 * 512);
  st1.insert(st1.end(), st2.begin(), st2.end());
  RbSrKvArgs a;
  a.x = x; a.ln1_g = tmp.up(ln1_g, C); a.ln1_b = tmp.up(ln1_b, C); a.ln1_eps = eps1;
  a.w = tmp.up_u16(st1); a.w_bytes = st1.size() * 2; a.sr_inv = tmp.up(inv1); a.sr_bias = tmp.up(sr_b, C);
  a.srn_g = tmp.up(srn_g, C); a.srn_b = tmp.up(srn_b, C); a.srn_eps = eps2; a.kv_inv = tmp.up(inv2); a.kv_bias = tmp.up(kv_b, 2 * C);
  a.kv = kv; a.B = B; a.Hr = Hr; a.Wr = Wr; a.bpi = (Hr * Wr + 31) / 32;
  a.sat = t_op_sat;
  launch_rb_srkv(a, C, s);
  a.sat = nullptr;
  if (iters > 0 && ms_out) {
    hipEvent_t e0, e1;
    (void)hipEventCreate(&e0); (void)hipEventCreate(&e1);
    (void)hipEventRecord(e0, s);
    for (int i = 0; i < iters; ++i) launch_rb_srkv(a, C, s);
    (void)hipEventRecord(e1, s);
    (void)hipEventSynchronize(e1);
    float t = 0.f;
    (void)hipEventElapsedTime(&t, e0, e1);
    *ms_out = t / iters;
    (void)hipEventDestroy(e0); (void)hipEventDestroy(e1);
  }
  rc = hipGetLastError() == hipSuccess ? PF_OK : PF_ERR_DEVICE;
  tmp.sync_free(s);
  return rc;
}

int pf_op_mit_mlp(int device, const float* x, float* y, int B, int Hs, int Ws, int C, const float* w1, const float* b1, const float* lng, const float* lnb, float eps,
                  const float* wdw, const float* bdw, const float* w2, const float* b2, int iters, float* ms_out, void* stream) {
  std::string err;
  int rc = check_device(device, &err);
  if (rc != PF_OK) { g_create_error = err; return rc; }
  if (!mit_mlp_supported(C) || !x || !y || x == y || B <= 0) { g_create_error = "pf_op_mit_mlp: C must be 64 or 128, x and y different buffers"; return PF_ERR_ARG; }
  hipStream_t s = static_cast<hipStream_t>(stream);
  TmpDev tmp;
  std::vector<unsigned short> wpk;
  std::vector<float> tab2;
  mit_mlp_pack(w1, b1, lng, lnb, wdw, bdw, w2, b2, C, &wpk, &tab2);
  const unsigned short* dw = tmp.up_u16(wpk);
  const float* dt = tmp.up(tab2);
  launch_mit_mlp(x, y, dw, dt, B, Hs, Ws, C, eps, s, t_op_sat, t_op_sat_limit);
  if (iters > 0 && ms_out) {
    hipEvent_t a, b;
    (void)hipEventCreate(&a); (void)hipEventCreate(&b);
    (void)hipEventRecord(a, s);
    for (int i = 0; i < iters; ++i) launch_mit_mlp(x, y, dw, dt, B, Hs, Ws, C, eps, s);
    (void)hipEventRecord(b, s);
    (void)hipEventSynchronize(b);
    float t = 0.f;
    (void)hipEventElapsedTime(&t, a, b);
    *ms_out = t / iters;
    (void)hipEventDestroy(a); (void)hipEventDestroy(b);
  }
  rc = hipGetLastError() == hipSuccess ? PF_OK : PF_ERR_DEVICE;
  tmp.sync_free(s);
  return rc;
}

int pf_op_cnx_mlp(int device, const float* d, float* y, long rows, int C, const float* w1, const float* b1, const float* lng, const float* lnb, float eps,
                  const float* w2, const float* b2, const float* ls, int iters, float* ms_out, void* stream) {
  std::string err;
  int rc = check_device(device, &err);
  if (rc != PF_OK) { g_create_error = err; return rc; }
  if ((!cnx_mlp_supported(C) && !cnx_rb_supported(C)) || !d || !y || rows <= 0 || rows > 0x7fffffffL / (4 * C)) { g_create_error = "pf_op_cnx_mlp: C must be 96, 192, 384 or 768"; return PF_ERR_ARG; }
  hipStream_t s = static_cast<hipStream_t>(stream);
  TmpDev tmp;
  std::vector<unsigned short> wpk;
  std::vector<float> tab;
  const bool rb = cnx_rb_supported(C);
  if (rb) cnx_rb_pack(w1, b1, w2, b2, ls, C, &wpk, &tab);
  else cnx_mlp_pack(w1, b1, lng, lnb, w2, b2, ls, C, &wpk, &tab);
  const unsigned short* dw = tmp.up_u16(wpk);
  const float* dt = tmp.up(tab);
  CnxRbArgs ra{};
  if (rb) {
    ra.d = d; ra.y = y; ra.w = dw; ra.w_bytes = wpk.size() * 2; ra.tab = dt; ra.ln_g = tmp.up(lng, C); ra.ln_b = tmp.up(lnb, C); ra.ln_eps = eps; ra.M = (int)rows;
    ra.sat = t_op_sat; ra.sat_limit = t_op_sat_limit;
    if (!dw || !dt || !ra.ln_g || !ra.ln_b) { g_create_error = "pf_op_cnx_mlp: hipMalloc failed"; tmp.sync_free(s); return PF_ERR_DEVICE; }
  }
  unsigned* sat = t_op_sat;
  auto launch = [&]() { if (rb) launch_cnx_rb(ra, C, s); else launch_cnx_mlp(d, y, dw, dt, rows, C, eps, s, sat, t_op_sat_limit); };
  launch();
  sat = ra.sat = nullptr;
  if (iters > 0 && ms_out) {
    hipEvent_t a, b;
    (void)hipEventCreate(&a); (void)hipEventCreate(&b);
    (void)hipEventRecord(a, s);
    for (int i = 0; i < iters; ++i) launch();
    (void)hipEventRecord(b, s);
    (void)hipEventSynchronize(b);
    float t = 0.f;
    (void)hipEventElapsedTime(&t, a, b);
    *ms_out = t / iters;
    (void)hipEventDestroy(a); (void)hipEventDestroy(b);
  }
  rc = hipGetLastError() == hipSuccess ? PF_OK : PF_ERR_DEVICE;
  tmp.sync_free(s);
  return rc;
}

int pf_op_conv2d_bench(int device, int B, int H, int W, int Cin, int Cout, int K, int stride, int pad, int tile_id, int iters, int fmt_prec, float* ms_out) {
  const int fmt = fmt_prec & 15, precision = fmt_prec >> 4;
  std::string err;
  int rc = check_device(device, &err);
  if (rc != PF_OK) { g_create_error = err; return rc; }
  if (Cin % 4 != 0 || iters <= 0 || !ms_out) { g_create_error = "pf_op_conv2d_bench: bad argument"; return PF_ERR_ARG; }
  ConvParams p;
  p.KWC = K * Cin; p.KWCp = roundup(p.KWC, 32);
  p.B = B; p.H = H; p.W = W; p.C1 = Cin; p.C2 = 0; p.KH = K; p.KW = K; p.stride = stride; p.pad = pad;
  p.Cout = Cout; p.act = ACT_RELU; p.post_relu = 0; p.nchw_out = 0;
  p.nterms = precision == PF_PRECISION_FP32_BF16X6 ? 6 : NT_F16X3;
  p.wino_half = conv_wino_half_env();
  p.finish();
  const size_t nx = (size_t)B * H * W * Cin, nw = (size_t)Cout * K * p.KWCp, ny = (size_t)p.M * Cout;
  float *dx = nullptr, *dw = nullptr, *dy = nullptr, *db = nullptr;
  unsigned short *dsb = nullptr, *dxs = nullptr, *dys = nullptr, *dh16 = nullptr;
  float* dinv = nullptr;
  TmpDev wino_tmp;
  unsigned short* dwino = nullptr;
  float* dwino_inv = nullptr;
  if (hipMalloc(&dx, nx * 4) != hipSuccess || hipMalloc(&dw, nw * 4) != hipSuccess || hipMalloc(&dy, ny * 4) != hipSuccess ||
      hipMalloc(&db, (size_t)Cout * 4) != hipSuccess || hipMalloc(&dsb, nw * 10) != hipSuccess || hipMalloc(&dh16, nw * 4) != hipSuccess ||
      hipMalloc(&dinv, (size_t)Cout * 4) != hipSuccess ||
      (fmt >= 1 && hipMalloc(&dxs, nx * 6) != hipSuccess) || (fmt >= 2 && hipMalloc(&dys, ny * 6) != hipSuccess)) { g_create_error = "pf_op_conv2d_bench: hipMalloc failed"; return PF_ERR_DEVICE; }
  {
    std::vector<float> hw(nw), hb(Cout);
    uint32_t st = 12345u;
    auto rnd = [&]() { st = st * 1664525u + 1013904223u; return (float)((st >> 8) & 0xffff) / 32768.0f - 1.0f; };
    for (auto& v : hw) v = rnd() * 0.05f;
    for (auto& v : hb) v = rnd();
    launch_fill_random(dx, (long)nx, 777u, 1.0f, nullptr);
    (void)hipMemcpy(dw, hw.data(), nw * 4, hipMemcpyHostToDevice);
    (void)hipMemcpy(db, hb.data(), (size_t)Cout * 4, hipMemcpyHostToDevice);
    const std::vector<unsigned short> sb = split_bf16x3(hw);
    (void)hipMemcpy(dsb, sb.data(), nw * 10, hipMemcpyHostToDevice);
    const F16Planes f = split_f16x2(hw, Cout);
    (void)hipMemcpy(dh16, f.planes.data(), nw * 4, hipMemcpyHostToDevice);
    (void)hipMemcpy(dinv, f.inv_scale.data(), (size_t)Cout * 4, hipMemcpyHostToDevice);
    if (K == 3 && stride == 1 && pad == 1 && Cin % 16 == 0 && Cout % 64 == 0 && p.KWCp == p.KWC) {
      std::vector<unsigned short> planes;
      std::vector<float> inv;
      wino_pack_weights(hw.data(), Cout, Cin, p.KWCp, &planes, &inv);
      wino_tmp.sync_free(nullptr);
      dwino = wino_tmp.up_u16(planes); dwino_inv = wino_tmp.up(inv);
    }
  }
  p.g[0].x = dx; p.g[0].w = dw; p.g[0].bias = db; p.g[0].y = dy;
  if (Cin % 32 == 0 || Cin == 4) { p.g[0].w_sb = dsb; p.g[0].w_h16 = dh16; p.g[0].w_h16_inv_scale = dinv; }
  p.g[0].w_wino = dwino; p.g[0].w_wino_inv = dwino_inv;
  const size_t fbit = p.nterms == NT_F16X3 ? SB_FMT_F16 : 0;
  if (fmt >= 1) { launch_split_planes(dx, dxs, nx | fbit, (long)nx, nullptr); p.g[0].x_sb = dxs; p.x_sb_plane = nx | fbit; p.g[0].x = nullptr; }
  if (fmt >= 2) { p.g[0].y_sb = dys; p.y_sb_plane = ny | fbit; p.g[0].y = nullptr; }
  if (!conv_tile_usable(p, tile_id) && tile_id >= 0) { *ms_out = -1.f; (void)hipFree(dx); (void)hipFree(dw); (void)hipFree(dy); (void)hipFree(db); (void)hipFree(dsb); (void)hipFree(dxs); (void)hipFree(dys); (void)hipFree(dh16); (void)hipFree(dinv); wino_tmp.sync_free(nullptr); return PF_OK; }
  hipEvent_t a, b;
  (void)hipEventCreate(&a); (void)hipEventCreate(&b);
  launch_conv_tile(p, tile_id, nullptr);
  launch_conv_tile(p, tile_id, nullptr);
  (void)hipEventRecord(a, nullptr);
  for (int i = 0; i < iters; ++i) launch_conv_tile(p, tile_id, nullptr);
  (void)hipEventRecord(b, nullptr);
  (void)hipEventSynchronize(b);
  float t = 0.f;
  (void)hipEventElapsedTime(&t, a, b);
  *ms_out = t / iters;
  if (getenv("PF_WINO_STAMPS") && strncmp(conv_tile_name(tile_id), "wino", 4) == 0) {
    unsigned long long* ds = nullptr;
    if (hipMalloc(&ds, 8 * 128 * 8) == hipSuccess) {
      (void)hipMemset(ds, 0, 8 * 128 * 8);
// ... 221 lines not shown
```

perspectivefields_amd/csrc/pf_kernels.h:

```cpp
#pragma once
#include <vector>
#include <hip/hip_runtime.h>
#include <stddef.h>
#include <stdint.h>

namespace pf {

enum Act { ACT_NONE = 0, ACT_RELU = 1, ACT_GELU = 2 };
#if defined(__HIPCC__)
__device__ __forceinline__ void sat_watch4(unsigned* sat, float limit, float a, float b, float c, float d) {
  const float mx = fmaxf(fmaxf(fabsf(a), fabsf(b)), fmaxf(fabsf(c), fabsf(d)));
  const float s = (a + b) + (c + d);
  if (!(mx <= limit) || s != s) atomicAdd(sat, 1u);
}
__device__ __forceinline__ float sat_acc4(float amax, float a, float b, float c, float d) {
  return __builtin_fmaxf(__builtin_fmaxf(__builtin_fmaxf(amax, __builtin_fabsf(a)), __builtin_fabsf(b)), __builtin_fmaxf(__builtin_fabsf(c), __builtin_fabsf(d)));
}
__device__ __forceinline__ void sat_flush(unsigned* sat, float limit, float amax) {
  if (sat && amax > limit) atomicAdd(sat, 1u);
}
#endif
#if defined(__HIP_DEVICE_COMPILE__)
#define PF_NO_PK_F32 __attribute__((target("no-packed-fp32-ops")))
#else
// ... 100 lines not shown
void launch_dwconv3x3_gelu_variant(int variant, const float* x, const float* w9c, const float* bias, float* y, int B, int H, int W, int C, hipStream_t s,
                                   unsigned short* y_sb = nullptr, size_t sb_plane = 0);
void launch_dwconv7x7(const float* x, const float* w49c, const float* bias, float* y, int B, int H, int W, int C, hipStream_t s);
void launch_dwconv7x7_cfg(int variant, int nc, int nb, int th, const float* x, const float* w49c, const float* bias, float* y, int B, int H, int W, int C, hipStream_t s);

void launch_sr_attention(const float* q, const float* kv, float* out, int B, int N, int M, int heads, hipStream_t s,
                         unsigned short* out_sb = nullptr, size_t sb_plane = 0);

void launch_sr_attention_variant(int variant, const float* q, const float* kv, float* out, int B, int N, int M, int heads, hipStream_t s,
                                 unsigned short* out_sb = nullptr, size_t sb_plane = 0);

struct MitAttn64Args {
  const float* x = nullptr;
  const float* kv = nullptr;
  float* y = nullptr;
  const unsigned short* wfr = nullptr;
  const float* tab = nullptr;
  int B = 0, N = 0, M = 0, QT = 1;
  float ln_eps = 1e-6f;
  unsigned* sat = nullptr;
  float sat_limit = 65504.f;
};
bool mit_attn64_supported(int C, int heads, int kv_rows);
void launch_mit_attn64(const MitAttn64Args& a, int num_cus, hipStream_t s);
void attn64_pack(const float* ln_g, const float* ln_b, const float* q_w, const float* q_b, const float* p_w, const float* p_b, std::vector<unsigned short>* wfr, std::vector<float>* tab);

struct Stem7Args {
  const float* x = nullptr;
  float* y = nullptr;
  const unsigned short* wfr = nullptr;
  const float* tab = nullptr;
  int B = 0, H = 0, W = 0, Ho = 0, Wo = 0, stride = 2, relu = 0, ln = 0, QT = 1;
  float ln_eps = 1e-5f;
  unsigned* sat = nullptr;
  float sat_limit = 65504.f;
};
bool stem7x7_supported(int Cin, int Cout, int K, int stride, int pad);
void launch_stem7x7(const Stem7Args& a, int num_cus, hipStream_t s);
void stem7x7_pack(const float* w, const double* out_scale, const float* bias, const float* ln_g, const float* ln_b, std::vector<unsigned short>* wfr, std::vector<float>* tab);

struct ThinLinArgs {
  const float* x = nullptr;
  const float* res = nullptr;
  float* y = nullptr;
  const unsigned short* wfr = nullptr;
  const float* tab = nullptr;
  long M = 0;
  int QT = 1;
  unsigned* sat = nullptr;
  float sat_limit = 65504.f;
};
bool thin128_supported(int K, int N);
void launch_thin128(const ThinLinArgs& a, int num_cus, hipStream_t s);
void thin128_pack(const float* w, const float* bias, std::vector<unsigned short>* wfr, std::vector<float>* tab);

void launch_upsample2x(const float* x, float* y, int B, int H, int W, int C, hipStream_t s, unsigned short* y_sb = nullptr, size_t sb_plane = 0);

void launch_split_planes(const float* x, unsigned short* y_sb, size_t sb_plane, long n, hipStream_t s);
void launch_merge_planes(const unsigned short* x_sb, size_t sb_plane, float* y, long n, hipStream_t s);
void launch_fill_random(float* p, long n, unsigned seed, float scale, hipStream_t s);
void launch_range_stats(const float* x, long n, float* out4 , hipStream_t s);

void launch_prep_u8(const uint8_t* in, float* out, long npix, const float* mean3, const float* std3, hipStream_t s);
void launch_prep_f32_nchw(const float* in, float* out, int B, int HW, const float* mean3, const float* std3, hipStream_t s);

void launch_resize_u8(const uint8_t* in, int H, int W, uint8_t* tmp, uint8_t* out, int OH, int OW, const int* bh, const int* kh, int ksh,
                      const int* bv, const int* kv, int ksv, hipStream_t s);

struct ResizeBatch {
  static constexpr int MAX = 32;
  int n;
  int H[MAX], W[MAX], ksh[MAX], ksv[MAX];
  const uint8_t* in[MAX];
  uint8_t* tmp[MAX];
  uint8_t* out[MAX];
  const int* bh[MAX]; const int* kh[MAX];
  const int* bv[MAX]; const int* kv[MAX];
};
void launch_resize_batch_u8(const ResizeBatch& rb, int OH, int OW, hipStream_t s);

void launch_pred_regression(const float* tg, const float* tl, const float* wg, const float* bg, const float* wl, const float* bl,
                            float* pred_g_nchw, float* pred_l_nchw, float* pn_in_nhwc4, int B, int HW, hipStream_t s);

void launch_decode_cls(const float* logit_g, int ng, const float* logit_l, int nl, float* dec_g, float* dec_l, int B, int HW, hipStream_t s);

void launch_postprocess(const float* g2, const float* l1, int h, int w, float* up_out, float* lat_out, int H, int W, int lat_is_sin, hipStream_t s);

struct PostBatch {
  static constexpr int MAX = 32;
  int n;
  int H[MAX], W[MAX];
  float rh[MAX], rw[MAX], sxs[MAX], sys[MAX];
  const float* g2[MAX];
  const float* l1[MAX];
  float* up[MAX];
  float* lat[MAX];
};
void launch_postprocess_batch(PostBatch& pb, int h, int w, int lat_is_sin, hipStream_t s);

void launch_nearest_nhwc4(const float* x, float* y, int B, int H, int W, int Ho, int Wo, hipStream_t s);

bool cnx_mlp_supported(int C);
bool cnx_mlp_preferred(int C);
void launch_cnx_mlp(const float* d, float* y, const unsigned short* wpk, const float* tab, long M, int C, float eps, hipStream_t s, unsigned* sat = nullptr, float sat_limit = 65504.f);
struct CnxRbArgs {
  const float* d;
  float* y;
  const unsigned short* w;
  size_t w_bytes;
  const float* tab;
  const float* ln_g;
  const float* ln_b;
  float ln_eps;
  int M;
  unsigned* sat = nullptr;
  float sat_limit = 65504.f;
};
bool cnx_rb_supported(int C);
int cnx_rb_rows(int C);
void launch_cnx_rb(const CnxRbArgs& a, int C, hipStream_t s);
bool mit_mlp_supported(int C);
bool mit_mlp_preferred(int C, int with128);
int mit_mlp_chunk_bytes(int C);
void launch_mit_mlp(const float* x, float* y, const unsigned short* wpk, const float* tab2, int B, int Hs, int Ws, int C, float eps, hipStream_t s, unsigned* sat = nullptr, float sat_limit = 65504.f);
struct RbLinArgs {
  const float* x;
  const float* ln_g;
  const float* ln_b;
  float ln_eps;
  const unsigned short* w;
  size_t w_bytes;
  const float* inv;
  const float* bias;
  const float* res;
  float* y;
  int M, tokens, bpi;
  int N, act;
  unsigned* sat = nullptr;
  float sat_limit = 65504.f;
  unsigned long long* stamps = nullptr;
};
bool rb_linear_supported(int K, int N);
struct RbSrKvArgs {
  const float* x;
  const float* ln1_g; const float* ln1_b; float ln1_eps;
  const unsigned short* w;
  size_t w_bytes;
  const float* sr_inv; const float* sr_bias;
  const float* srn_g; const float* srn_b; float srn_eps;
  const float* kv_inv; const float* kv_bias;
  float* kv;
  int B, Hr, Wr, bpi;
  unsigned* sat = nullptr;
};
bool rb_srkv_supported(int C, int sr);
struct RbProjFc1Args {
  const float* attn;
  float* x;
  const unsigned short* w;
  size_t w_bytes;
  const float* proj_inv; const float* proj_bias;
  const float* ln2_g; const float* ln2_b; float ln2_eps;
  const float* fc1_inv; const float* fc1_bias;
  float* hidden;
  int B, tokens, bpi;
  unsigned* sat = nullptr;
  float sat_limit = 65504.f, hidden_limit = 65504.f;
};
void launch_rb_proj_fc1(const RbProjFc1Args& a, int C, hipStream_t s);
void launch_rb_srkv(const RbSrKvArgs& a, int C, hipStream_t s);
void launch_rb_linear(const RbLinArgs& a, int K, hipStream_t s);
void launch_gap_ln_head(const float* x, const float* g, const float* b, const float* w, const float* hb, float* out, int B, int HW, int C, int nout, float eps, hipStream_t s);

void launch_fields_from_params(const float* cam5, int H, int W, float* up, float* lat, hipStream_t s);

void launch_paramnet_scalars(const float* raw, int nraw, float* out8, int B, int mode, hipStream_t s);

struct PinholeFit;
struct UsmFit;
constexpr int FIT_STATE = 40, USMFIT_STATE = 48;
constexpr int FIT_REC = 24, USMFIT_REC = 32;
struct FitParams {
  int free_pp, loss;
  float huber_delta, w_up, w_lat;
};
struct FitBatch {
  static constexpr int MAX = 32;
  int n;
  int H[MAX], W[MAX], nblk[MAX];
  const float* up[MAX];
  const float* lat[MAX];
  double* part[MAX];
  double* state;
  float* out;
  const float* init;
};
inline int fit_blocks_per_image(int H, int W) {
  const long nb = ((long)H * W + 4095) / 4096;
  return (int)(nb < 1 ? 1 : nb > 256 ? 256 : nb);
}
template <class Fit>
void launch_fit_init(const FitBatch& fb, const FitParams& prm, hipStream_t s);
template <class Fit>
void launch_fit_iteration(const FitBatch& fb, const FitParams& prm, hipStream_t s);
void launch_fields_usm(const float* cam6, int H, int W, float* up, float* lat, hipStream_t s);

struct PanoBatch {
  static constexpr int MAX = 32;
  int n, H, W;
  int tpr, tiles_x, tiles_y;
  int vec;
  const void* pano[MAX];
  int Hp[MAX], Wp[MAX];
  const float* cam;
  void* img;
  float* up;
  float* lat;
};
void launch_pano_crop(const PanoBatch& pb, int dtype, hipStream_t s);

constexpr int FERR_REC = 10;
constexpr int FERR_LEVEL_BINS = 2048;
constexpr int FERR_SEL = 4;
struct FerrState {
  double sums[2][5];
  unsigned long long rank[FERR_SEL];
  unsigned prefix[FERR_SEL];
};
struct FerrBatch {
  static constexpr int MAX = 32;
  int n;
  int H[MAX], W[MAX], nblk[MAX];
  int vec[MAX];
  const float* up_pred[MAX];
  const float* lat_pred[MAX];
  const float* up_gt[MAX];
  const float* lat_gt[MAX];
  float* err_up[MAX];
  float* err_lat[MAX];
  double* part[MAX];
  unsigned* hist[MAX];
  FerrState* state;
  double* out;
  float threshold;
};
int ferr_blocks_per_image(int H, int W);
void launch_field_errors(const FerrBatch& fb, hipStream_t s);
void launch_field_errors_hist(const FerrBatch& fb, long long* d_hist, double* d_hist_sums, hipStream_t s);

}
```

perspectivefields_amd/csrc/rb_chain.hip:

```cpp
#include <stdlib.h>

#include "rb_common.h"

namespace pf {

template <class G, bool RES, int ACT>
__device__ __forceinline__ void rb_chain_epilogue_store(float* y, int ldy, const float* tabs_inv, const float* tabs_bias, float* scratch, f32x16 (&acc)[G::NACC], int n0, int m0, int nrows,
                                                        int wave, int lane, unsigned* sat = nullptr, float sat_limit = 65504.f) {
  const int l31 = lane & 31, hi = lane >> 5;
  const int rrow = lane >> 3, c4 = lane & 7;
#pragma unroll
  for (int idx = 0; idx < G::NACC; ++idx) {
    int rt, ct;
    bool own;
    rb_tile_of<G>(idx, wave, rt, ct, own);
#pragma unroll
    for (int g = 0; g < 4; ++g)
      *reinterpret_cast<float4*>(scratch + l31 * 32 + (((2 * g + hi) ^ (l31 & 7)) << 2)) = make_float4(acc[idx][4 * g], acc[idx][4 * g + 1], acc[idx][4 * g + 2], acc[idx][4 * g + 3]);
    __builtin_amdgcn_wave_barrier();
    const int n = n0 + ct * 32 + c4 * 4;
    const float4 iv = *reinterpret_cast<const float4*>(tabs_inv + n), bb = *reinterpret_cast<const float4*>(tabs_bias + n);
    float4 v[4];
#pragma unroll
    for (int i = 0; i < 4; ++i) {
      const int row = rrow + 8 * i;
      v[i] = *reinterpret_cast<const float4*>(scratch + row * 32 + ((c4 ^ (row & 7)) << 2));
    }
    __builtin_amdgcn_wave_barrier();
#pragma unroll
    for (int i = 0; i < 4; ++i) {
      const int ml = rt * 32 + rrow + 8 * i;
      const float4 w = make_float4(fmaf(v[i].x, iv.x, bb.x), fmaf(v[i].y, iv.y, bb.y), fmaf(v[i].z, iv.z, bb.z), fmaf(v[i].w, iv.w, bb.w));
      if (own && ml < nrows) {
        if (sat) sat_watch4(sat, sat_limit, w.x, w.y, w.z, w.w);
        *reinterpret_cast<float4*>(y + (size_t)(m0 + ml) * ldy + n) = w;
      }
    }
  }
}

template <int C>
__global__ __launch_bounds__(256, 1) void rb_srkv_kernel(const RbSrKvArgs p) {
  using G = RbGeo<2, true, 1>;
  static_assert(C == 320, "geometry: one 320-column pass");
  constexpr int KC = C / 16;
  constexpr int CPT = KC / 4;
  constexpr int HALF = 2 * KC;
  __shared__ __attribute__((aligned(16))) unsigned char As[HALF * G::CHS];
  __shared__ __attribute__((aligned(16))) float tabs[2 * C + 4 * C];
  __shared__ __attribute__((aligned(16))) float red[2][4][32];
  __shared__ __attribute__((aligned(16))) float escr[4 * 1024];
  const int tid = threadIdx.x, lane = tid & 63, wave = __builtin_amdgcn_readfirstlane(tid >> 6);
  const int l31 = lane & 31, hi = lane >> 5;
  const int img = blockIdx.x / p.bpi, j = blockIdx.x - img * p.bpi;
  const int ntok = p.Hr * p.Wr;
  const int r0 = j * 32, nrows = min(32, ntok - r0);
  const int Wm = 2 * p.Wr;

  RbW<G> W;
  W.init(p.w, p.w_bytes, wave, lane);

  const int sr_ = tid >> 2, sq = tid & 3;
  const int red_t = r0 + min(sr_ & 31, nrows - 1);
  const int oy = red_t / p.Wr, ox = red_t - oy * p.Wr;
  auto stage_half = [&](int half, bool first) {
    const int tap = 2 * half + (sr_ >> 5), ky = tap >> 1, kx = tap & 1;
    const float* xr = p.x + ((size_t)img * (4 * ntok) + (size_t)(2 * oy + ky) * Wm + 2 * ox + kx) * C;
    float4 v[CPT][4];
#pragma unroll
    for (int i = 0; i < CPT; ++i)
#pragma unroll
      for (int e = 0; e < 4; ++e) v[i][e] = *reinterpret_cast<const float4*>(xr + 16 * (sq + 4 * i) + 4 * e);
    if (first) {
      for (int i = tid; i < C / 4; i += 256) {
        reinterpret_cast<float4*>(tabs)[i] = reinterpret_cast<const float4*>(p.sr_inv)[i];
        reinterpret_cast<float4*>(tabs + C)[i] = reinterpret_cast<const float4*>(p.sr_bias)[i];
      }
      for (int i = tid; i < 2 * C / 4; i += 256) {
        reinterpret_cast<float4*>(tabs + 2 * C)[i] = reinterpret_cast<const float4*>(p.kv_inv)[i];
        reinterpret_cast<float4*>(tabs + 4 * C)[i] = reinterpret_cast<const float4*>(p.kv_bias)[i];
      }
      W.prologue();
      }
    float s = 0.f;
#pragma unroll
    for (int i = 0; i < CPT; ++i)
#pragma unroll
      for (int e = 0; e < 4; ++e) s += (v[i][e].x + v[i][e].y) + (v[i][e].z + v[i][e].w);
    s += __shfl_xor(s, 1); s += __shfl_xor(s, 2);
    const float mu = s * (1.0f / C);
    float ss = 0.f;
#pragma unroll
    for (int i = 0; i < CPT; ++i)
#pragma unroll
      for (int e = 0; e < 4; ++e) {
        v[i][e] = make_float4(v[i][e].x - mu, v[i][e].y - mu, v[i][e].z - mu, v[i][e].w - mu);
        ss = fmaf(v[i][e].x, v[i][e].x, fmaf(v[i][e].y, v[i][e].y, fmaf(v[i][e].z, v[i][e].z, fmaf(v[i][e].w, v[i][e].w, ss))));
      }
    ss += __shfl_xor(ss, 1); ss += __shfl_xor(ss, 2);
    const float rs = 1.0f / sqrtf(ss * (1.0f / C) + p.ln1_eps);
#pragma unroll
    for (int i = 0; i < CPT; ++i) {
#pragma unroll
      for (int e = 0; e < 4; ++e) {
        const float4 g = *reinterpret_cast<const float4*>(p.ln1_g + 16 * (sq + 4 * i) + 4 * e), b = *reinterpret_cast<const float4*>(p.ln1_b + 16 * (sq + 4 * i) + 4 * e);
        v[i][e] = make_float4(fmaf(v[i][e].x * rs, g.x, b.x), fmaf(v[i][e].y * rs, g.y, b.y), fmaf(v[i][e].z * rs, g.z, b.z), fmaf(v[i][e].w * rs, g.w, b.w));
      }
      rb_store_chunk(As + ((sr_ >> 5) * KC + sq + 4 * i) * G::CHS, sr_ & 31, v[i]);
    }
  };

  f32x16 acc[G::NACC];
#pragma unroll
  for (int i = 0; i < G::NACC; ++i)
#pragma unroll
    for (int e = 0; e < 16; ++e) acc[i][e] = 0.f;
  RbA<G> A[2];
#pragma unroll 1
  for (int half = 0; half < 2; ++half) {
    if (half) __syncthreads();
    stage_half(half, half == 0);
    __syncthreads();
    A[0].read(As, lane, 0);
#pragma unroll 1
    for (int s = 0; s < HALF; s += RB_D) {
#pragma unroll
      for (int d = 0; d < RB_D; ++d) {
        const int nx = s + d + 1 == HALF ? 0 : s + d + 1;
        rb_step<G>(acc, W, d, A[d & 1], A[(d + 1) & 1], As + nx * G::CHS, lane, 0);
      }
    }
  }

  float ps = 0.f;
#pragma unroll
  for (int idx = 0; idx < G::NACC; ++idx) {
    int rt, ct;
    bool own;
    rb_tile_of<G>(idx, wave, rt, ct, own);
#pragma unroll
    for (int g = 0; g < 4; ++g) {
      const int n = ct * 32 + 8 * g + 4 * hi;
      const float4 iv = *reinterpret_cast<const float4*>(tabs + n), bb = *reinterpret_cast<const float4*>(tabs + C + n);
      acc[idx][4 * g] = fmaf(acc[idx][4 * g], iv.x, bb.x); acc[idx][4 * g + 1] = fmaf(acc[idx][4 * g + 1], iv.y, bb.y);
      acc[idx][4 * g + 2] = fmaf(acc[idx][4 * g + 2], iv.z, bb.z); acc[idx][4 * g + 3] = fmaf(acc[idx][4 * g + 3], iv.w, bb.w);
      if (own) ps += (acc[idx][4 * g] + acc[idx][4 * g + 1]) + (acc[idx][4 * g + 2] + acc[idx][4 * g + 3]);
    }
  }
  ps += __shfl_xor(ps, 32);
  if (hi == 0) red[0][wave][l31] = ps;
  __syncthreads();
  const float mu = ((red[0][0][l31] + red[0][1][l31]) + (red[0][2][l31] + red[0][3][l31])) * (1.0f / C);
  float pq = 0.f;
#pragma unroll
  for (int idx = 0; idx < G::NACC; ++idx) {
    int rt, ct;
    bool own;
    rb_tile_of<G>(idx, wave, rt, ct, own);
#pragma unroll
    for (int r = 0; r < 16; ++r) {
      acc[idx][r] -= mu;
      if (own) pq = fmaf(acc[idx][r], acc[idx][r], pq);
    }
  }
  pq += __shfl_xor(pq, 32);
  if (hi == 0) red[1][wave][l31] = pq;
  __syncthreads();
  const float rs = 1.0f / sqrtf(((red[1][0][l31] + red[1][1][l31]) + (red[1][2][l31] + red[1][3][l31])) * (1.0f / C) + p.srn_eps);
#pragma unroll
  for (int idx = 0; idx < G::NACC; ++idx) {
    int rt, ct;
    bool own;
    rb_tile_of<G>(idx, wave, rt, ct, own);
    if (!own) continue;
#pragma unroll
    for (int g = 0; g < 4; ++g) {
      const int n = ct * 32 + 8 * g + 4 * hi;
      const float4 gm = *reinterpret_cast<const float4*>(p.srn_g + n), be = *reinterpret_cast<const float4*>(p.srn_b + n);
      const float4 y = make_float4(fmaf(acc[idx][4 * g] * rs, gm.x, be.x), fmaf(acc[idx][4 * g + 1] * rs, gm.y, be.y), fmaf(acc[idx][4 * g + 2] * rs, gm.z, be.z),
                                   fmaf(acc[idx][4 * g + 3] * rs, gm.w, be.w));
      uint2 h, l;
      split4_f16(y, h, l);
      unsigned char* d = As + (2 * ct + (g >> 1)) * G::CHS + (l31 + 32 * (g & 1)) * 16 + 8 * hi;
      *reinterpret_cast<uint2*>(d) = h;
      *reinterpret_cast<uint2*>(d + 1024) = l;
    }
  }
  __syncthreads();

  const int m0 = img * ntok + r0;
  A[0].read(As, lane, 0);
#pragma unroll 1
  for (int ps2 = 0; ps2 < 2; ++ps2) {
#pragma unroll
    for (int i = 0; i < G::NACC; ++i)
#pragma unroll
      for (int e = 0; e < 16; ++e) acc[i][e] = 0.f;
#pragma unroll 1
    for (int s = 0; s < KC; s += RB_D) {
#pragma unroll
      for (int d = 0; d < RB_D; ++d) {
        const int nx = s + d + 1 == KC ? 0 : s + d + 1;
        rb_step<G>(acc, W, d, A[d & 1], A[(d + 1) & 1], As + nx * G::CHS, lane, 0);
      }
    }
    rb_chain_epilogue_store<G, false, ACT_NONE>(p.kv, 2 * C, tabs + 2 * C, tabs + 4 * C, escr + wave * 1024, acc, ps2 * G::COLS, m0, nrows, wave, lane, p.sat, 4094.f);
  }
}

template <int C>
__global__ __launch_bounds__(256, 1) void rb_proj_fc1_kernel(const RbProjFc1Args p) {
  using G = RbGeo<2, true, 2>;
  static_assert(C == 320, "geometry: 320-column passes");
  constexpr int KC = C / 16, CPT = KC / 4, H4 = 4 * C;
  __shared__ __attribute__((aligned(16))) unsigned char As[KC * G::CHS];
  __shared__ __attribute__((aligned(16))) float tabs[2 * C + 2 * H4];
  __shared__ __attribute__((aligned(16))) float red[2][4][64];
  __shared__ __attribute__((aligned(16))) float escr[4 * 1024];
  const int tid = threadIdx.x, lane = tid & 63, wave = __builtin_amdgcn_readfirstlane(tid >> 6);
  const int l31 = lane & 31, hi = lane >> 5;
  const int img = blockIdx.x / p.bpi, j = blockIdx.x - img * p.bpi;
  const int nrows = min(RB_ROWS, p.tokens - j * RB_ROWS);
  const int m0 = img * p.tokens + j * RB_ROWS;

  RbW<G> W;
  W.init(p.w, p.w_bytes, wave, lane);
  {
    const int r = tid >> 2, q = tid & 3;
    const float* ar = p.attn + (size_t)(m0 + min(r, nrows - 1)) * C;
    float4 v[CPT][4];
#pragma unroll
    for (int i = 0; i < CPT; ++i)
#pragma unroll
      for (int e = 0; e < 4; ++e) v[i][e] = *reinterpret_cast<const float4*>(ar + 16 * (q + 4 * i) + 4 * e);
    for (int i = tid; i < C / 4; i += 256) {
      reinterpret_cast<float4*>(tabs)[i] = reinterpret_cast<const float4*>(p.proj_inv)[i];
      reinterpret_cast<float4*>(tabs + C)[i] = reinterpret_cast<const float4*>(p.proj_bias)[i];
    }
    for (int i = tid; i < H4 / 4; i += 256) {
      reinterpret_cast<float4*>(tabs + 2 * C)[i] = reinterpret_cast<const float4*>(p.fc1_inv)[i];
      reinterpret_cast<float4*>(tabs + 2 * C + H4)[i] = reinterpret_cast<const float4*>(p.fc1_bias)[i];
    }
    W.prologue();
#pragma unroll
    for (int i = 0; i < CPT; ++i) rb_store_chunk(As + (q + 4 * i) * G::CHS, r, v[i]);
  }
  __syncthreads();

  const int xr = wave & 1;
  f32x16 acc[G::NACC];
#pragma unroll
  for (int i = 0; i < G::NACC; ++i)
#pragma unroll
    for (int e = 0; e < 16; ++e) acc[i][e] = 0.f;
  RbA<G> A[2];
  A[0].read(As, lane, xr);
#pragma unroll 1
  for (int s = 0; s < KC; s += RB_D) {
#pragma unroll
    for (int d = 0; d < RB_D; ++d) {
      const int nx = s + d + 1 == KC ? 0 : s + d + 1;
      rb_step<G>(acc, W, d, A[d & 1], A[(d + 1) & 1], As + nx * G::CHS, lane, xr);
    }
  }

  float ps[2] = {0.f, 0.f};
#pragma unroll
  for (int idx = 0; idx < G::NACC; ++idx) {
    int rt, ct;
    bool own;
    rb_tile_of<G>(idx, wave, rt, ct, own);
    const float* xrow = p.x + (size_t)(m0 + min(rt * 32 + l31, nrows - 1)) * C;
    float4 rr[4];
#pragma unroll
    for (int g = 0; g < 4; ++g) rr[g] = *reinterpret_cast<const float4*>(xrow + ct * 32 + 8 * g + 4 * hi);
    float t = 0.f;
#pragma unroll
    for (int g = 0; g < 4; ++g) {
      const int n = ct * 32 + 8 * g + 4 * hi;
      const float4 iv = *reinterpret_cast<const float4*>(tabs + n), bb = *reinterpret_cast<const float4*>(tabs + C + n);
      acc[idx][4 * g] = fmaf(acc[idx][4 * g], iv.x, bb.x) + rr[g].x; acc[idx][4 * g + 1] = fmaf(acc[idx][4 * g + 1], iv.y, bb.y) + rr[g].y;
      acc[idx][4 * g + 2] = fmaf(acc[idx][4 * g + 2], iv.z, bb.z) + rr[g].z; acc[idx][4 * g + 3] = fmaf(acc[idx][4 * g + 3], iv.w, bb.w) + rr[g].w;
      t += (acc[idx][4 * g] + acc[idx][4 * g + 1]) + (acc[idx][4 * g + 2] + acc[idx][4 * g + 3]);
    }
    if (idx < 2 * G::CTW) ps[idx & 1] += t;
    else { if (xr) ps[1] += t; else ps[0] += t; }
  }
  {
    const int rrow = lane >> 3, c4 = lane & 7;
    float* scratch = escr + wave * 1024;
#pragma unroll
    for (int idx = 0; idx < G::NACC; ++idx) {
      int rt, ct;
      bool own;
      rb_tile_of<G>(idx, wave, rt, ct, own);
#pragma unroll
      for (int g = 0; g < 4; ++g)
        *reinterpret_cast<float4*>(scratch + l31 * 32 + (((2 * g + hi) ^ (l31 & 7)) << 2)) = make_float4(acc[idx][4 * g], acc[idx][4 * g + 1], acc[idx][4 * g + 2], acc[idx][4 * g + 3]);
      __builtin_amdgcn_wave_barrier();
      float4 v[4];
#pragma unroll
      for (int i = 0; i < 4; ++i) {
        const int row = rrow + 8 * i;
        v[i] = *reinterpret_cast<const float4*>(scratch + row * 32 + ((c4 ^ (row & 7)) << 2));
      }
      __builtin_amdgcn_wave_barrier();
#pragma unroll
      for (int i = 0; i < 4; ++i) {
        const int ml = rt * 32 + rrow + 8 * i;
        if (ml < nrows) {
          if (p.sat) sat_watch4(p.sat, p.sat_limit, v[i].x, v[i].y, v[i].z, v[i].w);
          *reinterpret_cast<float4*>(p.x + (size_t)(m0 + ml) * C + ct * 32 + c4 * 4) = v[i];
        }
      }
    }
  }
  ps[0] += __shfl_xor(ps[0], 32); ps[1] += __shfl_xor(ps[1], 32);
  if (hi == 0) { red[0][wave][l31] = ps[0]; red[0][wave][32 + l31] = ps[1]; }
  __syncthreads();
  float mu[2], pq[2] = {0.f, 0.f};
#pragma unroll
  for (int rt = 0; rt < 2; ++rt) mu[rt] = ((red[0][0][rt * 32 + l31] + red[0][1][rt * 32 + l31]) + (red[0][2][rt * 32 + l31] + red[0][3][rt * 32 + l31])) * (1.0f / C);
#pragma unroll
  for (int idx = 0; idx < G::NACC; ++idx) {
    const float m = idx < 2 * G::CTW ? mu[idx & 1] : (xr ? mu[1] : mu[0]);
    float t = 0.f;
#pragma unroll
    for (int r = 0; r < 16; ++r) { acc[idx][r] -= m; t = fmaf(acc[idx][r], acc[idx][r], t); }
    if (idx < 2 * G::CTW) pq[idx & 1] += t;
    else { if (xr) pq[1] += t; else pq[0] += t; }
  }
  pq[0] += __shfl_xor(pq[0], 32); pq[1] += __shfl_xor(pq[1], 32);
  if (hi == 0) { red[1][wave][l31] = pq[0]; red[1][wave][32 + l31] = pq[1]; }
  __syncthreads();
  float rs[2];
#pragma unroll
  for (int rt = 0; rt < 2; ++rt)
    rs[rt] = 1.0f / sqrtf(((red[1][0][rt * 32 + l31] + red[1][1][rt * 32 + l31]) + (red[1][2][rt * 32 + l31] + red[1][3][rt * 32 + l31])) * (1.0f / C) + p.ln2_eps);
#pragma unroll
  for (int idx = 0; idx < G::NACC; ++idx) {
    int rt, ct;
    bool own;
    rb_tile_of<G>(idx, wave, rt, ct, own);
    const float r_ = idx < 2 * G::CTW ? rs[idx & 1] : (xr ? rs[1] : rs[0]);
#pragma unroll
    for (int g = 0; g < 4; ++g) {
      const int n = ct * 32 + 8 * g + 4 * hi;
      const float4 gm = *reinterpret_cast<const float4*>(p.ln2_g + n), be = *reinterpret_cast<const float4*>(p.ln2_b + n);
      const float4 y = make_float4(fmaf(acc[idx][4 * g] * r_, gm.x, be.x), fmaf(acc[idx][4 * g + 1] * r_, gm.y, be.y), fmaf(acc[idx][4 * g + 2] * r_, gm.z, be.z),
                                   fmaf(acc[idx][4 * g + 3] * r_, gm.w, be.w));
      uint2 h, l;
      split4_f16(y, h, l);
      unsigned char* d = As + (2 * ct + (g >> 1)) * G::CHS + rt * 2048 + (l31 + 32 * (g & 1)) * 16 + 8 * hi;
      *reinterpret_cast<uint2*>(d) = h;
      *reinterpret_cast<uint2*>(d + 1024) = l;
    }
  }
  __syncthreads();

  A[0].read(As, lane, xr);
#pragma unroll 1
  for (int ps2 = 0; ps2 < 4; ++ps2) {
#pragma unroll
    for (int i = 0; i < G::NACC; ++i)
#pragma unroll
      for (int e = 0; e < 16; ++e) acc[i][e] = 0.f;
#pragma unroll 1
    for (int s = 0; s < KC; s += RB_D) {
#pragma unroll
      for (int d = 0; d < RB_D; ++d) {
        const int nx = s + d + 1 == KC ? 0 : s + d + 1;
        rb_step<G>(acc, W, d, A[d & 1], A[(d + 1) & 1], As + nx * G::CHS, lane, xr);
      }
    }
    rb_chain_epilogue_store<G, false, ACT_NONE>(p.hidden, H4, tabs + 2 * C, tabs + 2 * C + H4, escr + wave * 1024, acc, ps2 * G::COLS, m0, nrows, wave, lane, p.sat, p.hidden_limit);
  }
}

bool rb_srkv_supported(int C, int sr) { return C == 320 && sr == 2; }

void launch_rb_proj_fc1(const RbProjFc1Args& a, int C, hipStream_t s) {
  const dim3 grid((unsigned)(a.B * a.bpi)), block(256);
  if (C == 320) hipLaunchKernelGGL((rb_proj_fc1_kernel<320>), grid, block, 0, s, a);
}

void launch_rb_srkv(const RbSrKvArgs& a, int C, hipStream_t s) {
  const dim3 grid((unsigned)(a.B * a.bpi)), block(256);
  if (C == 320) hipLaunchKernelGGL((rb_srkv_kernel<320>), grid, block, 0, s, a);
}

}
```

perspectivefields_amd/engine.py:

```python
from __future__ import annotations

import ctypes
import os
from typing import Dict, Optional, Tuple

import numpy as np

from .build import LIB as LIB_PATH

_HERE = os.path.dirname(os.path.abspath(__file__))
TILE_TABLE = os.path.join(_HERE, "tuned", "gfx950_tiles.txt")
NET = 320
PARAMS_STRIDE = 8

PF_OK = 0
DISPATCH_COLUMNS = ("batch", "s3_split_taken", "rb_launches", "splitk_launches", "splitk_max_factor", "wino_launches", "wino_half_launches", "thin128_launches",
                    "attn64_launches", "mit_mlp_fused_launches", "ln_kernel_launches", "conv_launches", "sb_tensors", "forks", "fork_alloc_conflicts",
                    "real_peak_bytes", "dry_peak_bytes", "cnx_rb_launches")
_STATUS = {0: "PF_OK", -1: "PF_ERR_ARG", -2: "PF_ERR_DEVICE", -3: "PF_ERR_WEIGHTS", -4: "PF_ERR_WORKSPACE"}

_c = ctypes
_P = _c.c_void_p
_SIGNATURES = {
    "pf_version": (_c.c_char_p, []),
    "pf_last_error": (_c.c_char_p, [_P]),
    "pf_create": (_c.c_int, [_c.POINTER(_P), _c.c_int, _c.c_int]),
    "pf_destroy": (_c.c_int, [_P]),
    "pf_load_tensor": (_c.c_int, [_P, _c.c_char_p, _P, _c.POINTER(_c.c_int64), _c.c_int]),
    "pf_finalize_weights": (_c.c_int, [_P]),
    "pf_output_info": (_c.c_int, [_P, _c.POINTER(_c.c_int), _c.POINTER(_c.c_int), _c.POINTER(_c.c_int)]),
    "pf_max_batch": (_c.c_int, []),
    "pf_workspace_bytes": (_c.c_size_t, [_P, _c.c_int]),
    "pf_last_dispatch": (_c.c_int, [_P, _c.POINTER(_c.c_int64), _c.c_int]),
    "pf_forward_u8": (_c.c_int, [_P, _c.c_int, _P, _P, _P, _P, _P, _c.c_size_t, _P]),
    "pf_forward_f32": (_c.c_int, [_P, _c.c_int, _P, _P, _P, _P, _P, _c.c_size_t, _P]),
    "pf_set_saturation_counter": (_c.c_int, [_P, _P]),
    "pf_static_window_max": (_c.c_int, [_P, _c.POINTER(_c.c_float)]),
    "pf_set_defer_params": (_c.c_int, [_P, _c.c_int]),
    "pf_join_params": (_c.c_int, [_P, _P]),
    "pf_forward_u8_graph": (_c.c_int, [_P, _c.c_int, _P, _P, _P, _P, _P, _c.c_size_t, _P]),
    "pf_resize_workspace_bytes": (_c.c_size_t, [_c.c_int, _c.c_int]),
    "pf_resize_bilinear_u8": (_c.c_int, [_P, _P, _c.c_int, _c.c_int, _P, _P, _c.c_size_t, _P]),
    "pf_resize_batch_u8": (_c.c_int, [_P, _c.c_int, _P, _P, _P, _P, _c.c_size_t, _P]),
    "pf_autotune": (_c.c_int, [_P, _c.c_int, _P, _P, _P, _P, _P, _c.c_size_t, _P]),
    "pf_is_tuned": (_c.c_int, [_P, _c.c_int]),
    "pf_autotune_workspace_bytes": (_c.c_size_t, [_P, _c.c_int]),
    "pf_load_tile_table": (_c.c_int, [_P, _c.c_char_p]),
    "pf_save_tile_table": (_c.c_int, [_P, _c.c_char_p]),
    "pf_build_digest": (_c.c_char_p, []),
    "pf_set_precision": (_c.c_int, [_P, _c.c_int]),
    "pf_postprocess": (_c.c_int, [_P, _P, _P, _c.c_int, _c.c_int, _P, _P, _P, _c.c_size_t, _P]),
    "pf_postprocess_batch": (_c.c_int, [_P, _c.c_int, _P, _P, _P, _P, _P, _P, _c.c_size_t, _P]),
    "pf_fields_from_params": (_c.c_int, [_c.c_int, _P, _c.c_int, _c.c_int, _P, _P, _P]),
    "pf_fit_camera_workspace_bytes": (_c.c_size_t, [_c.c_int, _P]),
    "pf_fit_camera": (_c.c_int, [_c.c_int, _c.c_int, _P, _P, _P, _P, _c.c_int, _c.c_int, _c.c_float, _c.c_float, _c.c_float, _c.c_int, _P, _P, _c.c_size_t, _P]),
    "pf_fit_camera_usm_workspace_bytes": (_c.c_size_t, [_c.c_int, _P]),
    "pf_fit_camera_usm": (_c.c_int, [_c.c_int, _c.c_int, _P, _P, _P, _P, _c.c_int, _c.c_int, _c.c_float, _c.c_float, _c.c_float, _c.c_int, _P, _P, _c.c_size_t, _P]),
    "pf_fields_from_params_usm": (_c.c_int, [_c.c_int, _P, _c.c_int, _c.c_int, _P, _P, _P]),
    "pf_pano_crop": (_c.c_int, [_c.c_int, _c.c_int, _P, _P, _c.c_int, _c.c_int, _P, _P, _c.c_int, _c.c_int, _P, _P, _P, _P]),
    "pf_field_errors_workspace_bytes": (_c.c_size_t, [_c.c_int, _P]),
    "pf_field_errors": (_c.c_int, [_c.c_int, _c.c_int, _P, _P, _P, _P, _P, _c.c_float, _P, _P, _P, _P, _P, _P, _c.c_size_t, _P]),
    "pf_profile_begin": (_c.c_int, [_P, _c.c_uint]),
    "pf_profile_pause": (_c.c_int, [_P]),
    "pf_profile_end": (_c.c_int, [_P, _c.POINTER(_c.c_double), _c.POINTER(_c.c_double), _c.POINTER(_c.c_long), _c.c_int]),
    "pf_profile_records": (_c.c_int, [_P, _c.c_int, _c.POINTER(_c.c_int), _c.POINTER(_c.c_double), _c.POINTER(_c.c_float), _c.POINTER(_c.c_int)]),
    "pf_profile_phases": (_c.c_int, [_P, _c.c_int, _c.POINTER(_c.c_double)]),
    "pf_debug_tap_bytes": (_c.c_size_t, [_P, _c.c_int]),
    "pf_debug_forward_u8": (_c.c_int, [_P, _c.c_int, _P, _P, _P, _P, _P, _c.c_size_t, _c.c_int, _P, _c.c_size_t, _P]),
    "pf_debug_taps": (_c.c_int, [_P, _c.c_int, _P, _c.POINTER(_c.c_longlong), _c.POINTER(_c.c_int)]),
    "pf_debug_ranges": (_c.c_int, [_P, _c.c_int, _P, _c.POINTER(_c.c_longlong), _c.POINTER(_c.c_float)]),
    "pf_op_set_saturation_watch": (_c.c_int, [_P, _c.c_float]),
    "pf_op_conv2d": (_c.c_int, [_c.c_int, _P, _P, _c.c_int, _c.c_int, _c.c_int, _c.c_int, _c.c_int, _P, _P,
                                _c.c_int, _c.c_int, _c.c_int, _c.c_int, _c.c_int, _c.c_int, _P, _P, _c.c_int,
                                _c.c_int, _c.c_int, _P, _P, _c.c_long, _P, _c.c_long, _P, _c.c_long, _c.c_int, _P]),
    "pf_op_conv2d_bench": (_c.c_int, [_c.c_int] * 12 + [_c.POINTER(_c.c_float)]),
    "pf_op_split_bf16": (_c.c_int, [_c.c_int, _P, _c.c_long, _P, _c.c_long, _P]),
    "pf_op_merge_bf16": (_c.c_int, [_c.c_int, _P, _c.c_long, _c.c_long, _P, _P]),
    "pf_op_dwconv3x3_bench": (_c.c_int, [_c.c_int] * 7 + [_c.POINTER(_c.c_float)]),
    "pf_op_layernorm": (_c.c_int, [_c.c_int, _P, _P, _P, _P, _c.c_long, _c.c_int, _c.c_float, _P, _c.c_long, _P]),
    "pf_op_dwconv3x3_gelu": (_c.c_int, [_c.c_int, _P, _P, _P, _P, _c.c_int, _c.c_int, _c.c_int, _c.c_int, _P, _c.c_long, _P]),
    "pf_op_mit_mlp": (_c.c_int, [_c.c_int, _P, _P, _c.c_int, _c.c_int, _c.c_int, _c.c_int, _P, _P, _P, _P, _c.c_float, _P, _P, _P, _P, _c.c_int, _c.POINTER(_c.c_float), _P]),
    "pf_op_cnx_mlp": (_c.c_int, [_c.c_int, _P, _P, _c.c_long, _c.c_int, _P, _P, _P, _P, _c.c_float, _P, _P, _P, _c.c_int, _c.POINTER(_c.c_float), _P]),
    "pf_op_rb_linear": (_c.c_int, [_c.c_int, _P, _c.c_long, _c.c_int, _c.c_int, _P, _P, _P, _P, _c.c_float, _c.c_int, _c.c_int, _P, _P, _c.c_int, _c.POINTER(_c.c_float), _P]),
    "pf_op_rb_proj_fc1": (_c.c_int, [_c.c_int, _P, _P, _c.c_int, _c.c_int, _c.c_int, _P, _P, _P, _P, _c.c_float, _P, _P, _P, _c.c_int, _c.POINTER(_c.c_float), _P]),
    "pf_op_mit_attn64": (_c.c_int, [_c.c_int, _P, _P, _P, _c.c_int, _c.c_int, _c.c_int, _P, _P, _c.c_float, _P, _P, _P, _P, _c.c_int, _c.POINTER(_c.c_float), _P]),
    "pf_op_stem7x7": (_c.c_int, [_c.c_int, _P, _P, _c.c_int, _c.c_int, _c.c_int, _c.c_int, _P, _P, _c.c_int, _P, _P, _c.c_float, _c.c_int, _c.POINTER(_c.c_float), _P]),
    "pf_op_thin128": (_c.c_int, [_c.c_int, _P, _c.c_long, _P, _P, _P, _P, _c.c_int, _c.POINTER(_c.c_float), _P]),
    "pf_op_rb_srkv": (_c.c_int, [_c.c_int, _P, _c.c_int, _c.c_int, _c.c_int, _c.c_int, _P, _P, _c.c_float, _P, _P, _P, _P, _c.c_float, _P, _P, _P, _c.c_int, _c.POINTER(_c.c_float), _P]),
    "pf_op_linear_ln": (_c.c_int, [_c.c_int, _P, _c.c_long, _c.c_int, _P, _P, _P, _P, _c.c_float, _c.c_int, _c.c_int, _P, _c.c_int, _P, _c.c_int, _P]),
    "pf_op_dwconv3x3_gelu_cfg": (_c.c_int, [_c.c_int, _P, _P, _P, _P, _c.c_int, _c.c_int, _c.c_int, _c.c_int, _P, _c.c_long, _c.c_int, _P]),
    "pf_op_dwconv7x7": (_c.c_int, [_c.c_int, _P, _P, _P, _P, _c.c_int, _c.c_int, _c.c_int, _c.c_int, _P]),
    "pf_op_dwconv7x7_cfg": (_c.c_int, [_c.c_int, _P, _P, _P, _P, _c.c_int, _c.c_int, _c.c_int, _c.c_int, _c.c_int, _c.c_int, _c.c_int, _c.c_int, _P]),
    "pf_op_dwconv7x7_bench": (_c.c_int, [_c.c_int] * 10 + [_c.POINTER(_c.c_float)]),
    "pf_op_sr_attention": (_c.c_int, [_c.c_int, _P, _P, _P, _c.c_int, _c.c_int, _c.c_int, _c.c_int, _P, _c.c_long, _P]),
    "pf_op_sr_attention_variant": (_c.c_int, [_c.c_int, _c.c_int, _P, _P, _P, _c.c_int, _c.c_int, _c.c_int, _c.c_int, _c.c_int, _c.POINTER(_c.c_float), _P]),
    "pf_op_upsample2x": (_c.c_int, [_c.c_int, _P, _P, _c.c_int, _c.c_int, _c.c_int, _c.c_int, _P, _c.c_long, _P]),
    "pf_op_num_conv_tiles": (_c.c_int, []),
    "pf_op_conv_tile_name": (_c.c_char_p, [_c.c_int]),
}

_lib = None


class PfError(RuntimeError):
    pass


def load_library(path: Optional[str] = None):
    global _lib
    if _lib is not None and path is None:
        return _lib
    p = path or LIB_PATH
    want = None
    if path is None:
        from . import build as _build

        stamp = os.path.join(os.path.dirname(LIB_PATH), "libpf_hip.digest")
        try:
            want = None if os.environ.get("PF_SKIP_DIGEST_CHECK") == "1" else _build._digest()
        except OSError:
            want = None
        have = open(stamp).read() if os.path.exists(stamp) else None
        if not os.path.exists(p) or (want is not None and have != want):
            try:
                import fcntl

                os.makedirs(os.path.dirname(LIB_PATH), exist_ok=True)
                with open(os.path.join(os.path.dirname(LIB_PATH), ".build.lock"), "w") as lk:
                    fcntl.flock(lk, fcntl.LOCK_EX)
                    _build.build(verbose=False)
            except Exception as e:
                what = "not found" if not os.path.exists(p) else "is stale (built from different sources)"
                raise PfError(
                    f"{p} {what} and could not be built ({e}); the HIP extension is required, there is no CPU fallback. "
                    "Build it with `python -m perspectivefields_amd.build` (needs hipcc)."
                ) from e
    if not os.path.exists(p):
        raise PfError(f"{p} not found: the HIP extension is not built and there is no CPU fallback.")
    lib = ctypes.CDLL(p)
    for name, (res, args) in _SIGNATURES.items():
        fn = getattr(lib, name)
        fn.restype = res
        fn.argtypes = args
    if path is None:
        got = lib.pf_build_digest().decode()
        if want is not None and got != want:
            raise PfError(f"{p} was built from different sources (library digest {got[:12]}, sources {want[:12]}): rebuild with `python -m perspectivefields_amd.build --force`")
        _lib = lib
    return lib


def declared_symbols():
    return list(_SIGNATURES)


def _stream_ptr():
    import torch

    return ctypes.c_void_p(torch.cuda.current_stream().cuda_stream)


def _check(rc: int, handle=None, what: str = ""):
    if rc != PF_OK:
        lib = load_library()
        msg = lib.pf_last_error(handle)
        raise PfError(f"{what}: {_STATUS.get(rc, rc)}: {msg.decode() if msg else ''}")


def _dev_index(device) -> int:
    import torch

    d = torch.device(device)
    if d.type != "cuda":
        raise PfError(f"the PerspectiveFields HIP engine needs a GPU device, got '{d}' (no CPU fallback)")
    return d.index if d.index is not None else torch.cuda.current_device()


class Engine:

    def __init__(self, arch_id: int, device):
        import torch

        if not torch.cuda.is_available():
            raise PfError("no GPU visible to PyTorch-ROCm: the HIP engine cannot run (no CPU fallback)")
        self.lib = load_library()
        self.device = torch.device("cuda", _dev_index(device))
        self.arch_id = arch_id
        self._h = ctypes.c_void_p()
        _check(self.lib.pf_create(ctypes.byref(self._h), self.device.index, arch_id), None, "pf_create")
        self._ws = None
        self._scratch_stream = {}
        self._finalized = False
        self.precision = "fp32"
        self.max_batch = int(self.lib.pf_max_batch())
        self.graph_max_batch = int(os.environ.get("PF_GRAPH_MAX_BATCH", "0"))
        self.defer_params = False
        self._deferred = []
        self._graph_bufs = {}
        with torch.cuda.device(self.device):
            self._sat = torch.zeros(1, dtype=torch.int32, device=self.device)
        _check(self.lib.pf_set_saturation_counter(self._h, self._sat.data_ptr()), self._h, "pf_set_saturation_counter")
        self.sat_seen = 0
        g, l, p = ctypes.c_int(), ctypes.c_int(), ctypes.c_int()
        self.lib.pf_output_info(self._h, ctypes.byref(g), ctypes.byref(l), ctypes.byref(p))
        self.gravity_channels, self.latitude_channels, self.param_outputs = g.value, l.value, p.value

    def __del__(self):
        try:
            if getattr(self, "_h", None) and self._h.value:
                self.lib.pf_destroy(self._h)
                self._h = ctypes.c_void_p()
        except Exception:
            pass

    def load_state_dict(self, state_dict: Dict[str, object]):
        for key, val in state_dict.items():
            arr = val.detach().cpu().numpy() if hasattr(val, "detach") else np.asarray(val)
            if key.endswith("num_batches_tracked"):
                arr = np.zeros((), dtype=np.float32)
            arr = np.ascontiguousarray(arr, dtype=np.float32)
            shape = (ctypes.c_int64 * max(arr.ndim, 1))(*arr.shape)
            _check(
                self.lib.pf_load_tensor(self._h, key.encode(), arr.ctypes.data_as(ctypes.c_void_p), shape, arr.ndim),
                self._h, f"pf_load_tensor({key})",
            )
        _check(self.lib.pf_finalize_weights(self._h), self._h, "pf_finalize_weights")
        self._finalized = True
        table = os.environ.get("PF_TILE_TABLE", TILE_TABLE)
        if table and os.path.exists(table):
            self.tile_table_entries = self.lib.pf_load_tile_table(self._h, table.encode())

    def autotune(self, batch: int, save_to: Optional[str] = None) -> None:
        import torch

        with torch.cuda.device(self.device):
            x = torch.randint(0, 256, (batch, NET, NET, 3), dtype=torch.uint8, device=self.device)
            pg = torch.empty((batch, self.gravity_channels, NET, NET), dtype=torch.float32, device=self.device)
            pl = torch.empty((batch, self.latitude_channels, NET, NET), dtype=torch.float32, device=self.device)
            params = torch.empty((batch, PARAMS_STRIDE), dtype=torch.float32, device=self.device) if self.param_outputs else None
            ws = self._workspace(int(self.lib.pf_autotune_workspace_bytes(self._h, batch)))
            rc = self.lib.pf_autotune(self._h, batch, x.data_ptr(), pg.data_ptr(), pl.data_ptr(),
# ... 290 lines not shown
```

perspectivefields_amd/ops.py:

```python
from __future__ import annotations

import contextlib
import ctypes

import numpy as np

from .engine import PfError, _check, _stream_ptr, load_library


def _np(a):
    if a is None:
        return None
    a = a.detach().cpu().numpy() if hasattr(a, "detach") else np.asarray(a)
    return np.ascontiguousarray(a, dtype=np.float32)


def _hp(a):
    return a.ctypes.data_as(ctypes.c_void_p) if a is not None else None


def _dp(t):
    return t.data_ptr() if t is not None else None


@contextlib.contextmanager
def saturation_watch(limit=65504.0):
    import torch

    lib = load_library()
    counter = torch.zeros(1, dtype=torch.int32, device=torch.device("cuda", torch.cuda.current_device()))
    _check(lib.pf_op_set_saturation_watch(counter.data_ptr(), float(limit)), None, "pf_op_set_saturation_watch")
    try:
        yield counter
    finally:
        lib.pf_op_set_saturation_watch(None, 0.0)


class Planes:

    def __init__(self, shape, device, fmt="bf16x3"):
        import torch

        self.shape = tuple(shape)
        self.fmt = fmt
        self.numel = int(np.prod(self.shape))
        stride = (self.numel + 127) // 128 * 128
        self.plane_elems = stride | (1 if fmt == "f16x2" else 0)
        self.data = torch.zeros((2 if fmt == "f16x2" else 3) * stride, dtype=torch.int16, device=device)

    def data_ptr(self):
        return self.data.data_ptr()

    def merge(self):
        import torch

        lib = load_library()
        y = torch.empty(self.shape, dtype=torch.float32, device=self.data.device)
        _check(lib.pf_op_merge_bf16(self.data.device.index, self.data_ptr(), self.plane_elems, self.numel, y.data_ptr(), _stream_ptr()), None, "pf_op_merge_bf16")
        return y


def split_planes(x, fmt="bf16x3"):
    lib = load_library()
    x = x.contiguous()
    pl = Planes(x.shape, x.device, fmt)
    _check(lib.pf_op_split_bf16(x.device.index, x.data_ptr(), x.numel(), pl.data_ptr(), pl.plane_elems, _stream_ptr()), None, "pf_op_split_bf16")
    return pl


def _pl(planes):
    return (planes.data_ptr(), planes.plane_elems) if planes is not None else (None, 0)


def conv2d(x, weight, bias=None, stride=1, pad=0, act=0, res1=None, res2=None, post_relu=False, x2=None, nchw_out=False, tile=-1,
           planes_in=False, planes_out=False, precision=0, planes_fmt="bf16x3", splitk=True):
    import torch

    lib = load_library()
    x = x.contiguous()
    B, H, W, C1 = x.shape
    C2 = 0 if x2 is None else x2.shape[-1]
    w = _np(weight)
    Cout, Cin, KH, KW = w.shape
    if Cin != C1 + C2:
        raise PfError(f"weight Cin {Cin} != {C1}+{C2}")
    Ho = (H + 2 * pad - KH) // stride + 1
    Wo = (W + 2 * pad - KW) // stride + 1
    shape = (B, Cout, Ho, Wo) if nchw_out else (B, Ho, Wo, Cout)
    b = _np(bias)
    x2 = x2.contiguous() if x2 is not None else None
    xp = split_planes(x, planes_fmt) if planes_in else None
    x2p = split_planes(x2, planes_fmt) if (planes_in and x2 is not None) else None
    yp = Planes(shape, x.device, planes_fmt) if planes_out else None
    y = None if planes_out else torch.empty(shape, dtype=torch.float32, device=x.device)
    rc = lib.pf_op_conv2d(
        x.device.index, None if planes_in else x.data_ptr(), None if planes_in else _dp(x2), B, H, W, C1, C2, _hp(w), _hp(b),
        Cout, KH, KW, stride, pad, act, _dp(res1), _dp(res2), int(post_relu), int(nchw_out), tile, _dp(y),
        *_pl(xp), *_pl(x2p), *_pl(yp), precision + (0 if splitk else 16), _stream_ptr(),
    )
    _check(rc, None, "pf_op_conv2d")
    return yp.merge() if planes_out else y


def linear(x, weight, bias=None, act=0, res1=None, tile=-1):
    K = x.shape[-1]
    rows = x.numel() // K
    w = _np(weight)
    y = conv2d(x.reshape(1, rows, 1, K), w.reshape(w.shape[0], K, 1, 1), bias, act=act,
               res1=None if res1 is None else res1.reshape(1, rows, 1, -1), tile=tile)
    return y.reshape(*x.shape[:-1], w.shape[0])


def linear_ln(x, weight, bias, gamma, beta, eps, act=0, res1=None, tile=-1, precision=0):
    import torch

    lib = load_library()
    x = x.contiguous()
    K = x.shape[-1]
    rows = x.numel() // K
    w, b, g, be = _np(weight), _np(bias), _np(gamma), _np(beta)
    N = w.shape[0]
    y = torch.empty((*x.shape[:-1], N), dtype=torch.float32, device=x.device)
    _check(lib.pf_op_linear_ln(x.device.index, x.data_ptr(), rows, K, _hp(w), _hp(b), _hp(g), _hp(be), float(eps), N, act, _dp(res1), tile, y.data_ptr(), precision,
                               _stream_ptr()), None, "pf_op_linear_ln")
    return y


def rb_linear(x, weight, bias, tokens, gamma=None, beta=None, eps=1e-6, act=0, res=None, iters=0):
    import torch

    lib = load_library()
    x = x.contiguous()
    K = x.shape[-1]
    rows = x.numel() // K
    w, b = _np(weight), _np(bias)
    g, be = (_np(gamma), _np(beta)) if gamma is not None else (None, None)
    N = w.shape[0]
    y = torch.empty((*x.shape[:-1], N), dtype=torch.float32, device=x.device)
    ms = ctypes.c_float()
    _check(lib.pf_op_rb_linear(x.device.index, x.data_ptr(), rows, tokens, K, _hp(w), _hp(b), _hp(g), _hp(be), float(eps), N,
                               act, _dp(res), y.data_ptr(), iters, ctypes.byref(ms), _stream_ptr()), None, "pf_op_rb_linear")
    return ms.value if iters > 0 else y


def rb_proj_fc1(attn, x, proj_w, proj_b, ln2_g, ln2_b, eps, fc1_w, fc1_b, tokens, iters=0):
    import torch

    lib = load_library()
    attn = attn.contiguous()
    x1 = x.contiguous().clone()
    rows, C = attn.shape
    hidden = torch.empty((rows, 4 * C), dtype=torch.float32, device=attn.device)
    ms = ctypes.c_float()
    a = [_np(t) for t in (proj_w, proj_b, ln2_g, ln2_b, fc1_w, fc1_b)]
    _check(lib.pf_op_rb_proj_fc1(attn.device.index, attn.data_ptr(), x1.data_ptr(), rows // tokens, tokens, C, _hp(a[0]), _hp(a[1]), _hp(a[2]), _hp(a[3]), float(eps), _hp(a[4]), _hp(a[5]),
                                 hidden.data_ptr(), iters, ctypes.byref(ms), _stream_ptr()), None, "pf_op_rb_proj_fc1")
    return ms.value if iters > 0 else (x1, hidden)


def rb_srkv(x, ln1_g, ln1_b, eps1, sr_w, sr_b, srn_g, srn_b, eps2, kv_w, kv_b, iters=0):
    import torch

    lib = load_library()
    x = x.contiguous()
    B, H, W, C = x.shape
    kv = torch.empty((B, (H // 2) * (W // 2), 2 * C), dtype=torch.float32, device=x.device)
    ms = ctypes.c_float()
    a = [_np(t) for t in (ln1_g, ln1_b, sr_w, sr_b, srn_g, srn_b, kv_w, kv_b)]
    _check(lib.pf_op_rb_srkv(x.device.index, x.data_ptr(), B, H // 2, W // 2, C, _hp(a[0]), _hp(a[1]), float(eps1), _hp(a[2]), _hp(a[3]), _hp(a[4]), _hp(a[5]), float(eps2),
                             _hp(a[6]), _hp(a[7]), kv.data_ptr(), iters, ctypes.byref(ms), _stream_ptr()), None, "pf_op_rb_srkv")
    return ms.value if iters > 0 else kv


def mit_attn64(x, kv, ln_gamma, ln_beta, eps, q_w, q_b, proj_w, proj_b, iters=0, inplace=False):
    import torch

    lib = load_library()
    x, kv = x.contiguous(), kv.contiguous()
    B, N, C = x.shape
    y = x if inplace else torch.empty_like(x)
    ms = ctypes.c_float()
    g, b, qw, qb, pw, pb = (_np(t) for t in (ln_gamma, ln_beta, q_w, q_b, proj_w, proj_b))
    _check(lib.pf_op_mit_attn64(x.device.index, x.data_ptr(), kv.data_ptr(), y.data_ptr(), B, N, kv.shape[1], _hp(g), _hp(b), eps, _hp(qw), _hp(qb), _hp(pw), _hp(pb),
                                iters, ctypes.byref(ms), _stream_ptr()), None, "pf_op_mit_attn64")
    return (y, ms.value) if iters > 0 else y


def stem7x7(x4, weight, bias, stride, relu=False, ln_gamma=None, ln_beta=None, eps=1e-5, iters=0):
    import torch

    lib = load_library()
    x4 = x4.contiguous()
    B, H, W, _ = x4.shape
    Ho, Wo = (H + 6 - 7) // stride + 1, (W + 6 - 7) // stride + 1
    y = torch.empty((B, Ho, Wo, 64), dtype=torch.float32, device=x4.device)
    ms = ctypes.c_float()
    w, b = _np(weight), _np(bias)
    g, be = (_np(ln_gamma), _np(ln_beta)) if ln_gamma is not None else (None, None)
    _check(lib.pf_op_stem7x7(x4.device.index, x4.data_ptr(), y.data_ptr(), B, H, W, stride, _hp(w), _hp(b), 1 if relu else 0, _hp(g), _hp(be), float(eps), iters, ctypes.byref(ms),
                             _stream_ptr()), None, "pf_op_stem7x7")
    return (y, ms.value) if iters > 0 else y


def thin128(x, weight, bias, res=None, iters=0, inplace=False):
    import torch

    lib = load_library()
    x = x.contiguous()
    rows = x.numel() // 128
    y = res if (inplace and res is not None) else torch.empty_like(x)
    ms = ctypes.c_float()
    w, b = _np(weight), _np(bias)
    _check(lib.pf_op_thin128(x.device.index, x.data_ptr(), rows, _hp(w), _hp(b), _dp(res), y.data_ptr(), iters, ctypes.byref(ms), _stream_ptr()), None, "pf_op_thin128")
    return (y, ms.value) if iters > 0 else y


def mit_mlp(x, fc1_w, fc1_b, ln_gamma, ln_beta, eps, dw_w, dw_b, fc2_w, fc2_b, iters=0):
    import torch

    lib = load_library()
    x = x.contiguous()
    B, Hs, Ws, C = x.shape
    y = torch.empty_like(x)
    ms = ctypes.c_float()
    a = [_np(v) for v in (fc1_w, fc1_b, ln_gamma, ln_beta, dw_w, dw_b, fc2_w, fc2_b)]
    _check(lib.pf_op_mit_mlp(x.device.index, x.data_ptr(), y.data_ptr(), B, Hs, Ws, C, _hp(a[0]), _hp(a[1]), _hp(a[2]), _hp(a[3]), float(eps), _hp(a[4]), _hp(a[5]), _hp(a[6]), _hp(a[7]),
                             iters, ctypes.byref(ms), _stream_ptr()), None, "pf_op_mit_mlp")
    return ms.value if iters > 0 else y


def cnx_mlp(d, y, w1, b1, ln_gamma, ln_beta, eps, w2, b2, layer_scale, iters=0):
    lib = load_library()
    d = d.contiguous()
    out = y.contiguous().clone()
    rows, C = d.shape
    ms = ctypes.c_float()
    a = [_np(v) for v in (w1, b1, ln_gamma, ln_beta, w2, b2, layer_scale)]
    _check(lib.pf_op_cnx_mlp(d.device.index, d.data_ptr(), out.data_ptr(), rows, C, _hp(a[0]), _hp(a[1]), _hp(a[2]), _hp(a[3]), float(eps), _hp(a[4]), _hp(a[5]), _hp(a[6]),
                             iters, ctypes.byref(ms), _stream_ptr()), None, "pf_op_cnx_mlp")
    return ms.value if iters > 0 else out


def layernorm(x, gamma, beta, eps, planes_out=False):
    import torch

    lib = load_library()
    x = x.contiguous()
    C = x.shape[-1]
    y = None if planes_out else torch.empty_like(x)
    yp = Planes(x.shape, x.device) if planes_out else None
    g, b = _np(gamma), _np(beta)
    _check(lib.pf_op_layernorm(x.device.index, x.data_ptr(), _hp(g), _hp(b), _dp(y), x.numel() // C, C, eps, *_pl(yp), _stream_ptr()), None, "pf_op_layernorm")
    return yp.merge() if planes_out else y


def dwconv3x3_gelu(x, weight, bias, planes_out=False, variant=None):
    import torch

    lib = load_library()
    x = x.contiguous()
    B, H, W, C = x.shape
    y = None if planes_out else torch.empty_like(x)
    yp = Planes(x.shape, x.device) if planes_out else None
    w, b = _np(weight), _np(bias)
    if variant is not None:
        _check(lib.pf_op_dwconv3x3_gelu_cfg(x.device.index, x.data_ptr(), _hp(w), _hp(b), _dp(y), B, H, W, C, *_pl(yp), int(variant), _stream_ptr()), None, "pf_op_dwconv3x3_gelu_cfg")
        return yp.merge() if planes_out else y
    _check(lib.pf_op_dwconv3x3_gelu(x.device.index, x.data_ptr(), _hp(w), _hp(b), _dp(y), B, H, W, C, *_pl(yp), _stream_ptr()), None, "pf_op_dwconv3x3_gelu")
    return yp.merge() if planes_out else y


def dwconv7x7(x, weight, bias, variant=None, nc=0, nb=0, th=0):
    import torch

    lib = load_library()
    x = x.contiguous()
    B, H, W, C = x.shape
    y = torch.empty_like(x)
    w, b = _np(weight), _np(bias)
    if variant is None:
        _check(lib.pf_op_dwconv7x7(x.device.index, x.data_ptr(), _hp(w), _hp(b), y.data_ptr(), B, H, W, C, _stream_ptr()), None, "pf_op_dwconv7x7")
    else:
        _check(lib.pf_op_dwconv7x7_cfg(x.device.index, x.data_ptr(), _hp(w), _hp(b), y.data_ptr(), B, H, W, C, variant, nc, nb, th, _stream_ptr()), None, "pf_op_dwconv7x7_cfg")
    return y


def dwconv7x7_bench(variant, B, H, W, C, nc=0, nb=0, th=0, iters=10, device=0):
    lib = load_library()
    ms = ctypes.c_float()
    _check(lib.pf_op_dwconv7x7_bench(device, variant, nc, nb, th, B, H, W, C, iters, ctypes.byref(ms)), None, "pf_op_dwconv7x7_bench")
    return ms.value


def sr_attention(q, kv, heads, planes_out=False):
    import torch

    lib = load_library()
    q, kv = q.contiguous(), kv.contiguous()
    B, N, C = q.shape
    M = kv.shape[1]
    out = None if planes_out else torch.empty_like(q)
    op = Planes(q.shape, q.device) if planes_out else None
    _check(lib.pf_op_sr_attention(q.device.index, q.data_ptr(), kv.data_ptr(), _dp(out), B, N, M, heads, *_pl(op), _stream_ptr()), None, "pf_op_sr_attention")
    return op.merge() if planes_out else out


def sr_attention_variant(q, kv, heads, variant, iters=0):
    import torch

    lib = load_library()
    q, kv = q.contiguous(), kv.contiguous()
    B, N, C = q.shape
    out = torch.empty_like(q)
    ms = ctypes.c_float()
    _check(lib.pf_op_sr_attention_variant(q.device.index, variant, q.data_ptr(), kv.data_ptr(), out.data_ptr(), B, N, kv.shape[1], heads, iters,
                                          ctypes.byref(ms), _stream_ptr()), None, "pf_op_sr_attention_variant")
    return (out, ms.value) if iters > 0 else out


def upsample2x(x, planes_out=False):
    import torch

    lib = load_library()
    x = x.contiguous()
    B, H, W, C = x.shape
    shape = (B, 2 * H, 2 * W, C)
# ... 24 lines not shown
```

Baseline: 1755 images/sec.

## Fuse spatial-reduction KV and Q projection into one heterogeneous-block kernel

Adds an rb_qkv kernel whose grid holds both the LN-fused spatial-reduction KV blocks, now indexed linearly across images, and the LN+Q projection blocks, so one launch replaces the srkv launch plus the separate Q GEMM or side-stream fork. The goal is fewer launches and no fork/join for the stage-3 attention Q/KV, with the Q blocks filling CUs left idle by the small KV grid. It is on by default when the srkv form would be taken. In exchange the combined kernel carries the larger shared-memory footprint, and KV and Q blocks have unequal work, which may unbalance the grid.

```diff
diff --git a/include/pf_hip.h b/include/pf_hip.h
--- a/include/pf_hip.h
+++ b/include/pf_hip.h
@@ -118,7 +118,8 @@
 #define PF_DISPATCH_REAL_PEAK_BYTES 15
 #define PF_DISPATCH_DRY_PEAK_BYTES 16
 #define PF_DISPATCH_CNX_RB_LAUNCHES 17
-#define PF_DISPATCH_COLS 18
+#define PF_DISPATCH_RB_QKV_LAUNCHES 18
+#define PF_DISPATCH_COLS 19
 int pf_last_dispatch(pf_handle h, int64_t* out, int n);
 
 int pf_postprocess_batch(pf_handle h, int batch, const float* d_pred_gravity, const float* d_pred_latitude, const int32_t* h_hw,
@@ -222,6 +223,9 @@
 int pf_op_rb_srkv(int device, const float* d_x, int B, int Hr, int Wr, int C, const float* h_ln1_gamma, const float* h_ln1_beta, float eps1, const float* h_sr_w,
                   const float* h_sr_b, const float* h_srn_gamma, const float* h_srn_beta, float eps2, const float* h_kv_w, const float* h_kv_b, float* d_kv, int iters,
                   float* ms_out, void* stream);
+int pf_op_rb_qkv(int device, const float* d_x, int B, int Hr, int Wr, int C, const float* h_ln1_gamma, const float* h_ln1_beta, float eps1, const float* h_sr_w,
+                 const float* h_sr_b, const float* h_srn_gamma, const float* h_srn_beta, float eps2, const float* h_kv_w, const float* h_kv_b, const float* h_q_w,
+                 const float* h_q_b, float* d_kv, float* d_q, int iters, float* ms_out, void* stream);
 int pf_op_cnx_mlp(int device, const float* d_d, float* d_y, long rows, int C, const float* h_w1, const float* h_b1, const float* h_ln_gamma, const float* h_ln_beta,
                   float eps, const float* h_w2, const float* h_b2, const float* h_layer_scale, int iters, float* ms_out, void* stream);
 int pf_op_mit_mlp(int device, const float* d_x, float* d_y, int B, int Hs, int Ws, int C, const float* h_fc1_w, const float* h_fc1_b, const float* h_ln_gamma,
diff --git a/perspectivefields_amd/csrc/engine.hip b/perspectivefields_amd/csrc/engine.hip
--- a/perspectivefields_amd/csrc/engine.hip
+++ b/perspectivefields_amd/csrc/engine.hip
@@ -301,6 +301,7 @@
   bool can_fork(const Ctx& c) { return side_stream_mode && !c.dry && !c.tuning && (!c.prof || c.prof->min_work > 0.0) && side_ready(); }
   bool sba_heads = false;
   int rb_chain = 60;
+  int rb_qkv = 1;
   int rb_min_blocks = 192;
   int num_cus = 256;
   int wino_min_hw = 20;
@@ -992,7 +993,25 @@
         const bool fuse64 = attn64 && mb.a64_w && nterms == NT_F16X3 && !S && !c.tuning && sr > 1;
         const long rb_blocks = (long)gate_B * ((N + 63) / 64);
         const bool use_rb = rb_chain && mb.rq.w && nterms == NT_F16X3 && !S && !c.tuning && rb_blocks >= rb_min_blocks && (rb_blocks % num_cus == 0 || rb_blocks % num_cus >= num_cus * 3 / 4);
-        if (sr > 1 && use_rb && (rb_chain & 32) && mb.rsrkv.w && mb.qln.ln_s && fuse_ln) {
+        const bool srkv_form = sr > 1 && use_rb && (rb_chain & 32) && mb.rsrkv.w && mb.qln.ln_s && fuse_ln;
+        const bool qkv_form = rb_qkv && sr > 1 && (rb_chain & 32) && mb.rsrkv.w && mb.rq.w && fuse_ln && nterms == NT_F16X3 && !S && !c.tuning && Ho == 2 * kvh && Wo == 2 * kvw &&
+                              (srkv_form || rb_qkv >= 2);
+        if (qkv_form) {
+          range_in(c, fmt("rb_srkv s%d.b%d x (LN-fused)", s + 1, blk), x, (size_t)M * C);
+          if (!c.dry) {
+            RbQkvArgs a;
+            a.kv.x = x; a.kv.ln1_g = mb.n1.g; a.kv.ln1_b = mb.n1.b; a.kv.ln1_eps = mb.n1.eps;
+            a.kv.w = mb.rsrkv.w; a.kv.w_bytes = mb.rsrkv.bytes; a.kv.sr_inv = mb.rsrkv.sr_inv; a.kv.sr_bias = mb.rsrkv.sr_b;
+            a.kv.srn_g = mb.srn.g; a.kv.srn_b = mb.srn.b; a.kv.srn_eps = mb.srn.eps; a.kv.kv_inv = mb.rsrkv.kv_inv; a.kv.kv_bias = mb.rsrkv.kv_b;
+            a.kv.kv = kvb; a.kv.B = B; a.kv.Hr = kvh; a.kv.Wr = kvw; a.kv.bpi = 0; a.kv.sat = d_sat;
+            a.q_w = mb.rq.w; a.q_w_bytes = mb.rq.bytes; a.q_inv = mb.rq.inv; a.q_bias = mb.rq.b; a.q = qb; a.q_limit = mb.rq.sat_limit;
+            a.M = (int)M; a.nkv = (int)((Mkv + 31) / 32);
+            ProfScope ps(c.prof, c.s, PC_IGEMM_SB, 2.0 * Mkv * (double)C * (sr * sr * C + 2 * C) + 2.0 * M * (double)C * C, (int)Mkv, 3 * C, sr * sr * C + 2 * C, sr);
+            c.count(PF_DISPATCH_RB_LAUNCHES);
+            c.count(PF_DISPATCH_RB_QKV_LAUNCHES);
+            launch_rb_qkv(a, C, c.s);
+          }
+        } else if (srkv_form) {
           const bool fork = B >= 4 && (may_fork && can_fork(c));
           if (fork) {
             (void)hipEventRecord(ev_fork, c.s);
@@ -1073,7 +1092,7 @@
           gemm(c, mb.q, xn, M, Ten(qb));
           gemm(c, mb.kv, xn, M, Ten(kvb));
         }
-        if (!fuse64 && B >= 4 && (sr > 1 || (mb.q.ln_s && mb.kv.ln_s)) && (may_fork && can_fork(c))) (void)hipStreamWaitEvent(c.s, ev_join, 0);
+        if (!qkv_form && !fuse64 && B >= 4 && (sr > 1 || (mb.q.ln_s && mb.kv.ln_s)) && (may_fork && can_fork(c))) (void)hipStreamWaitEvent(c.s, ev_join, 0);
         if (may_fork) fork_join(c, fw_q);
         if (c.dbg && c.dbg->range) {
           if (!fuse64) range_in(c, fmt("attention s%d.b%d q", s + 1, blk), qb, (size_t)M * C);
@@ -1519,6 +1538,7 @@
     for (int t = 0; t < conv_num_tiles(); ++t) if (strcmp(conv_tile_name(t), wt ? wt : "wino256x64d") == 0) e->wino_tile = t;
   }
   if (const char* v = getenv("PF_RB_CHAIN")) e->rb_chain = atoi(v);
+  if (const char* v = getenv("PF_RB_QKV")) e->rb_qkv = atoi(v);
   if (const char* v = getenv("PF_DEFER_AT")) e->defer_at = atoi(v);
   if (const char* v = getenv("PF_DEFER_PRIO")) e->defer_prio = atoi(v);
   if (!host_only) {
diff --git a/perspectivefields_amd/csrc/engine_ops.hip b/perspectivefields_amd/csrc/engine_ops.hip
--- a/perspectivefields_amd/csrc/engine_ops.hip
+++ b/perspectivefields_amd/csrc/engine_ops.hip
@@ -345,6 +345,55 @@
     (void)hipEventCreate(&e0); (void)hipEventCreate(&e1);
     (void)hipEventRecord(e0, s);
     for (int i = 0; i < iters; ++i) launch_rb_srkv(a, C, s);
+    (void)hipEventRecord(e1, s);
+    (void)hipEventSynchronize(e1);
+    float t = 0.f;
+    (void)hipEventElapsedTime(&t, e0, e1);
+    *ms_out = t / iters;
+    (void)hipEventDestroy(e0); (void)hipEventDestroy(e1);
+  }
+  rc = hipGetLastError() == hipSuccess ? PF_OK : PF_ERR_DEVICE;
+  tmp.sync_free(s);
+  return rc;
+}
+
+int pf_op_rb_qkv(int device, const float* x, int B, int Hr, int Wr, int C, const float* ln1_g, const float* ln1_b, float eps1, const float* sr_w, const float* sr_b,
+                 const float* srn_g, const float* srn_b, float eps2, const float* kv_w, const float* kv_b, const float* q_w, const float* q_b, float* kv, float* q, int iters,
+                 float* ms_out, void* stream) {
+  std::string err;
+  int rc = check_device(device, &err);
+  if (rc != PF_OK) { g_create_error = err; return rc; }
+  if (!rb_srkv_supported(C, 2) || !x || !kv || !q || !ln1_g || !ln1_b || !sr_w || !sr_b || !srn_g || !srn_b || !kv_w || !kv_b || !q_w || !q_b || B <= 0 || Hr <= 0 || Wr <= 0 ||
+      (long)B * Hr * Wr * 4 > 0x7fffffffL / C) {
+    g_create_error = "pf_op_rb_qkv: C must be 320 (2 x 2 spatial reduction); all weights required";
+    return PF_ERR_ARG;
+  }
+  hipStream_t s = static_cast<hipStream_t>(stream);
+  TmpDev tmp;
+  int kwc = 0, kwcp = 0;
+  const std::vector<float> srp = pack_conv(sr_w, C, C, 2, 2, C, nullptr, &kwc, &kwcp);
+  std::vector<unsigned short> st1, st2, stq;
+  std::vector<float> inv1, inv2, invq;
+  rb_pack_w(srp.data(), C, 2 * kwcp, 320, &st1, &inv1);
+  rb_pack_w(kv_w, 2 * C, C, 320, &st2, &inv2);
+  rb_pack_w(q_w, C, C, 320, &stq, &invq);
+  st1.resize(st1.size() - (size_t)4 * 10 * 2 * 512);
+  st1.insert(st1.end(), st2.begin(), st2.end());
+  RbQkvArgs a;
+  a.kv.x = x; a.kv.ln1_g = tmp.up(ln1_g, C); a.kv.ln1_b = tmp.up(ln1_b, C); a.kv.ln1_eps = eps1;
+  a.kv.w = tmp.up_u16(st1); a.kv.w_bytes = st1.size() * 2; a.kv.sr_inv = tmp.up(inv1); a.kv.sr_bias = tmp.up(sr_b, C);
+  a.kv.srn_g = tmp.up(srn_g, C); a.kv.srn_b = tmp.up(srn_b, C); a.kv.srn_eps = eps2; a.kv.kv_inv = tmp.up(inv2); a.kv.kv_bias = tmp.up(kv_b, 2 * C);
+  a.kv.kv = kv; a.kv.B = B; a.kv.Hr = Hr; a.kv.Wr = Wr; a.kv.bpi = 0;
+  a.q_w = tmp.up_u16(stq); a.q_w_bytes = stq.size() * 2; a.q_inv = tmp.up(invq); a.q_bias = tmp.up(q_b, C); a.q = q;
+  a.M = B * Hr * Wr * 4; a.nkv = (B * Hr * Wr + 31) / 32;
+  a.kv.sat = t_op_sat; a.kv.kv_limit = fminf(4094.f, t_op_sat_limit); a.q_limit = fminf(8188.f, t_op_sat_limit);
+  launch_rb_qkv(a, C, s);
+  a.kv.sat = nullptr;
+  if (iters > 0 && ms_out) {
+    hipEvent_t e0, e1;
+    (void)hipEventCreate(&e0); (void)hipEventCreate(&e1);
+    (void)hipEventRecord(e0, s);
+    for (int i = 0; i < iters; ++i) launch_rb_qkv(a, C, s);
     (void)hipEventRecord(e1, s);
     (void)hipEventSynchronize(e1);
     float t = 0.f;
diff --git a/perspectivefields_amd/csrc/pf_kernels.h b/perspectivefields_amd/csrc/pf_kernels.h
--- a/perspectivefields_amd/csrc/pf_kernels.h
+++ b/perspectivefields_amd/csrc/pf_kernels.h
@@ -276,8 +276,18 @@
   float* kv;
   int B, Hr, Wr, bpi;
   unsigned* sat = nullptr;
+  float kv_limit = 4094.f;
 };
 bool rb_srkv_supported(int C, int sr);
+struct RbQkvArgs {
+  RbSrKvArgs kv;
+  const unsigned short* q_w;
+  size_t q_w_bytes;
+  const float* q_inv; const float* q_bias;
+  float* q;
+  int M, nkv;
+  float q_limit = 65504.f;
+};
 struct RbProjFc1Args {
   const float* attn;
   float* x;
@@ -293,6 +303,7 @@
 };
 void launch_rb_proj_fc1(const RbProjFc1Args& a, int C, hipStream_t s);
 void launch_rb_srkv(const RbSrKvArgs& a, int C, hipStream_t s);
+void launch_rb_qkv(const RbQkvArgs& a, int C, hipStream_t s);
 void launch_rb_linear(const RbLinArgs& a, int K, hipStream_t s);
 void launch_gap_ln_head(const float* x, const float* g, const float* b, const float* w, const float* hb, float* out, int B, int HW, int C, int nout, float eps, hipStream_t s);
 
diff --git a/perspectivefields_amd/csrc/rb_chain.hip b/perspectivefields_amd/csrc/rb_chain.hip
--- a/perspectivefields_amd/csrc/rb_chain.hip
+++ b/perspectivefields_amd/csrc/rb_chain.hip
@@ -39,49 +39,49 @@
   }
 }
 
-template <int C>
-__global__ __launch_bounds__(256, 1) void rb_srkv_kernel(const RbSrKvArgs p) {
+template <int C, bool LIN>
+__device__ __forceinline__ void rb_srkv_body(const RbSrKvArgs& p, int blk, unsigned char* As, float* tabs , float (*red)[4][32], float* escr) {
   using G = RbGeo<2, true, 1>;
   static_assert(C == 320, "geometry: one 320-column pass");
   constexpr int KC = C / 16;
   constexpr int CPT = KC / 4;
   constexpr int HALF = 2 * KC;
-  __shared__ __attribute__((aligned(16))) unsigned char As[HALF * G::CHS];
-  __shared__ __attribute__((aligned(16))) float tabs[2 * C + 4 * C];
-  __shared__ __attribute__((aligned(16))) float red[2][4][32];
-  __shared__ __attribute__((aligned(16))) float escr[4 * 1024];
   const int tid = threadIdx.x, lane = tid & 63, wave = __builtin_amdgcn_readfirstlane(tid >> 6);
   const int l31 = lane & 31, hi = lane >> 5;
-  const int img = blockIdx.x / p.bpi, j = blockIdx.x - img * p.bpi;
   const int ntok = p.Hr * p.Wr;
-  const int r0 = j * 32, nrows = min(32, ntok - r0);
+  const int img = LIN ? 0 : blk / p.bpi;
+  const int r0 = LIN ? blk * 32 : (blk - img * p.bpi) * 32;
+  const int nrows = min(32, (LIN ? p.B * ntok : ntok) - r0);
   const int Wm = 2 * p.Wr;
 
   RbW<G> W;
   W.init(p.w, p.w_bytes, wave, lane);
 
   const int sr_ = tid >> 2, sq = tid & 3;
-  const int red_t = r0 + min(sr_ & 31, nrows - 1);
+  const int row_t = r0 + min(sr_ & 31, nrows - 1);
+  const int img_t = LIN ? row_t / ntok : img;
+  const int red_t = LIN ? row_t - img_t * ntok : row_t;
   const int oy = red_t / p.Wr, ox = red_t - oy * p.Wr;
-  auto stage_half = [&](int half, bool first) {
+  auto load_rows = [&](int half, float4 (&v)[CPT][4]) {
     const int tap = 2 * half + (sr_ >> 5), ky = tap >> 1, kx = tap & 1;
-    const float* xr = p.x + ((size_t)img * (4 * ntok) + (size_t)(2 * oy + ky) * Wm + 2 * ox + kx) * C;
-    float4 v[CPT][4];
+    const float* xr = p.x + ((size_t)img_t * (4 * ntok) + (size_t)(2 * oy + ky) * Wm + 2 * ox + kx) * C;
 #pragma unroll
     for (int i = 0; i < CPT; ++i)
 #pragma unroll
       for (int e = 0; e < 4; ++e) v[i][e] = *reinterpret_cast<const float4*>(xr + 16 * (sq + 4 * i) + 4 * e);
-    if (first) {
-      for (int i = tid; i < C / 4; i += 256) {
-        reinterpret_cast<float4*>(tabs)[i] = reinterpret_cast<const float4*>(p.sr_inv)[i];
-        reinterpret_cast<float4*>(tabs + C)[i] = reinterpret_cast<const float4*>(p.sr_bias)[i];
-      }
-      for (int i = tid; i < 2 * C / 4; i += 256) {
-        reinterpret_cast<float4*>(tabs + 2 * C)[i] = reinterpret_cast<const float4*>(p.kv_inv)[i];
-        reinterpret_cast<float4*>(tabs + 4 * C)[i] = reinterpret_cast<const float4*>(p.kv_bias)[i];
-      }
-      W.prologue();
-      }
+  };
+  auto first_loads = [&]() {
+    for (int i = tid; i < C / 4; i += 256) {
+      reinterpret_cast<float4*>(tabs)[i] = reinterpret_cast<const float4*>(p.sr_inv)[i];
+      reinterpret_cast<float4*>(tabs + C)[i] = reinterpret_cast<const float4*>(p.sr_bias)[i];
+    }
+    for (int i = tid; i < 2 * C / 4; i += 256) {
+      reinterpret_cast<float4*>(tabs + 2 * C)[i] = reinterpret_cast<const float4*>(p.kv_inv)[i];
+      reinterpret_cast<float4*>(tabs + 4 * C)[i] = reinterpret_cast<const float4*>(p.kv_bias)[i];
+    }
+    W.prologue();
+  };
+  auto ln_store = [&](float4 (&v)[CPT][4]) {
     float s = 0.f;
 #pragma unroll
     for (int i = 0; i < CPT; ++i)
@@ -116,11 +116,7 @@
 #pragma unroll
     for (int e = 0; e < 16; ++e) acc[i][e] = 0.f;
   RbA<G> A[2];
-#pragma unroll 1
-  for (int half = 0; half < 2; ++half) {
-    if (half) __syncthreads();
-    stage_half(half, half == 0);
-    __syncthreads();
+  auto k_loop = [&]() {
     A[0].read(As, lane, 0);
 #pragma unroll 1
     for (int s = 0; s < HALF; s += RB_D) {
@@ -129,6 +125,30 @@
         const int nx = s + d + 1 == HALF ? 0 : s + d + 1;
         rb_step<G>(acc, W, d, A[d & 1], A[(d + 1) & 1], As + nx * G::CHS, lane, 0);
       }
+    }
+  };
+  if constexpr (LIN) {
+    float4 v0[CPT][4], v1[CPT][4];
+    load_rows(0, v0);
+    first_loads();
+    load_rows(1, v1);
+    ln_store(v0);
+    __syncthreads();
+    k_loop();
+    __syncthreads();
+    ln_store(v1);
+    __syncthreads();
+    k_loop();
+  } else {
+#pragma unroll 1
+    for (int half = 0; half < 2; ++half) {
+      if (half) __syncthreads();
+      float4 v[CPT][4];
+      load_rows(half, v);
+      if (half == 0) first_loads();
+      ln_store(v);
+      __syncthreads();
+      k_loop();
     }
   }
 
@@ -204,8 +224,104 @@
         rb_step<G>(acc, W, d, A[d & 1], A[(d + 1) & 1], As + nx * G::CHS, lane, 0);
       }
     }
-    rb_chain_epilogue_store<G, false, ACT_NONE>(p.kv, 2 * C, tabs + 2 * C, tabs + 4 * C, escr + wave * 1024, acc, ps2 * G::COLS, m0, nrows, wave, lane, p.sat, 4094.f);
-  }
+    rb_chain_epilogue_store<G, false, ACT_NONE>(p.kv, 2 * C, tabs + 2 * C, tabs + 4 * C, escr + wave * 1024, acc, ps2 * G::COLS, m0, nrows, wave, lane, p.sat, p.kv_limit);
+  }
+}
+
+static constexpr int RB_SRKV_AS = 2 * (320 / 16) * RbGeo<2, true, 1>::CHS;
+static constexpr int RB_Q_AS = (320 / 16) * RbGeo<2, true>::CHS;
+
+template <int C>
+__global__ __launch_bounds__(256, 1) void rb_srkv_kernel(const RbSrKvArgs p) {
+  __shared__ __attribute__((aligned(16))) unsigned char As[RB_SRKV_AS];
+  __shared__ __attribute__((aligned(16))) float tabs[2 * C + 4 * C];
+  __shared__ __attribute__((aligned(16))) float red[2][4][32];
+  __shared__ __attribute__((aligned(16))) float escr[4 * 1024];
+  rb_srkv_body<C, false>(p, (int)blockIdx.x, As, tabs, red, escr);
+}
+
+template <int C>
+__device__ __forceinline__ void rb_q_body(const RbQkvArgs& p, int j, unsigned char* As, float* tabs , float* escr) {
+  using G = RbGeo<2, true>;
+  static_assert(C == 320, "geometry: one 320-column pass");
+  constexpr int KC = C / 16, CPT = KC / 4;
+  const int tid = threadIdx.x, lane = tid & 63, wave = __builtin_amdgcn_readfirstlane(tid >> 6);
+  const int m0 = j * RB_ROWS, nrows = min(RB_ROWS, p.M - m0);
+
+  RbW<G> W;
+  W.init(p.q_w, p.q_w_bytes, wave, lane);
+  {
+    const int r = tid >> 2, q = tid & 3;
+    const float* xr = p.kv.x + (size_t)(m0 + min(r, nrows - 1)) * C;
+    float4 v[CPT][4];
+#pragma unroll
+    for (int i = 0; i < CPT; ++i)
+#pragma unroll
+      for (int e = 0; e < 4; ++e) v[i][e] = *reinterpret_cast<const float4*>(xr + 16 * (q + 4 * i) + 4 * e);
+    const int tk = min(tid, C / 4 - 1);
+    const float4 t_iv = reinterpret_cast<const float4*>(p.q_inv)[tk], t_bb = reinterpret_cast<const float4*>(p.q_bias)[tk];
+    W.prologue();
+    float s = 0.f;
+#pragma unroll
+    for (int i = 0; i < CPT; ++i)
+#pragma unroll
+      for (int e = 0; e < 4; ++e) s += (v[i][e].x + v[i][e].y) + (v[i][e].z + v[i][e].w);
+    s += __shfl_xor(s, 1); s += __shfl_xor(s, 2);
+    const float mu = s * (1.0f / C);
+    float ss = 0.f;
+#pragma unroll
+    for (int i = 0; i < CPT; ++i)
+#pragma unroll
+      for (int e = 0; e < 4; ++e) {
+        v[i][e] = make_float4(v[i][e].x - mu, v[i][e].y - mu, v[i][e].z - mu, v[i][e].w - mu);
+        ss = fmaf(v[i][e].x, v[i][e].x, fmaf(v[i][e].y, v[i][e].y, fmaf(v[i][e].z, v[i][e].z, fmaf(v[i][e].w, v[i][e].w, ss))));
+      }
+    ss += __shfl_xor(ss, 1); ss += __shfl_xor(ss, 2);
+    const float rs = 1.0f / sqrtf(ss * (1.0f / C) + p.kv.ln1_eps);
+#pragma unroll
+    for (int i = 0; i < CPT; ++i) {
+#pragma unroll
+      for (int e = 0; e < 4; ++e) {
+        const float4 g = *reinterpret_cast<const float4*>(p.kv.ln1_g + 16 * (q + 4 * i) + 4 * e), b = *reinterpret_cast<const float4*>(p.kv.ln1_b + 16 * (q + 4 * i) + 4 * e);
+        v[i][e] = make_float4(fmaf(v[i][e].x * rs, g.x, b.x), fmaf(v[i][e].y * rs, g.y, b.y), fmaf(v[i][e].z * rs, g.z, b.z), fmaf(v[i][e].w * rs, g.w, b.w));
+      }
+      rb_store_chunk(As + (q + 4 * i) * G::CHS, r, v[i]);
+    }
+    if (tid < C / 4) {
+      reinterpret_cast<float4*>(tabs)[tid] = t_iv;
+      reinterpret_cast<float4*>(tabs + C)[tid] = t_bb;
+    }
+  }
+  __syncthreads();
+
+  const int xr = wave & 1;
+  f32x16 acc[G::NACC];
+#pragma unroll
+  for (int i = 0; i < G::NACC; ++i)
+#pragma unroll
+    for (int e = 0; e < 16; ++e) acc[i][e] = 0.f;
+  RbA<G> A[2];
+  A[0].read(As, lane, xr);
+#pragma unroll 1
+  for (int s = 0; s < KC; s += RB_D) {
+#pragma unroll
+    for (int d = 0; d < RB_D; ++d) {
+      const int nx = s + d + 1 == KC ? 0 : s + d + 1;
+      rb_step<G>(acc, W, d, A[d & 1], A[(d + 1) & 1], As + nx * G::CHS, lane, xr);
+    }
+  }
+  rb_chain_epilogue_store<G, false, ACT_NONE>(p.q, C, tabs, tabs + C, escr + wave * 1024, acc, 0, m0, nrows, wave, lane, p.kv.sat, p.q_limit);
+}
+
+template <int C>
+__global__ __launch_bounds__(256, 1) void rb_qkv_kernel(const RbQkvArgs p) {
+  __shared__ __attribute__((aligned(16))) unsigned char As[RB_SRKV_AS > RB_Q_AS ? RB_SRKV_AS : RB_Q_AS];
+  __shared__ __attribute__((aligned(16))) float tabs[2 * C + 4 * C];
+  __shared__ __attribute__((aligned(16))) float red[2][4][32];
+  __shared__ __attribute__((aligned(16))) float escr[4 * 1024];
+  const int b = (int)blockIdx.x;
+  if (b < p.nkv) rb_srkv_body<C, true>(p.kv, b, As, tabs, red, escr);
+  else rb_q_body<C>(p, b - p.nkv, As, tabs, escr);
 }
 
 template <int C>
@@ -384,6 +500,11 @@
   if (C == 320) hipLaunchKernelGGL((rb_proj_fc1_kernel<320>), grid, block, 0, s, a);
 }
 
+void launch_rb_qkv(const RbQkvArgs& a, int C, hipStream_t s) {
+  const dim3 grid((unsigned)(a.nkv + (a.M + RB_ROWS - 1) / RB_ROWS)), block(256);
+  if (C == 320) hipLaunchKernelGGL((rb_qkv_kernel<320>), grid, block, 0, s, a);
+}
+
 void launch_rb_srkv(const RbSrKvArgs& a, int C, hipStream_t s) {
   const dim3 grid((unsigned)(a.B * a.bpi)), block(256);
   if (C == 320) hipLaunchKernelGGL((rb_srkv_kernel<320>), grid, block, 0, s, a);
diff --git a/perspectivefields_amd/engine.py b/perspectivefields_amd/engine.py
--- a/perspectivefields_amd/engine.py
+++ b/perspectivefields_amd/engine.py
@@ -16,7 +16,7 @@
 PF_OK = 0
 DISPATCH_COLUMNS = ("batch", "s3_split_taken", "rb_launches", "splitk_launches", "splitk_max_factor", "wino_launches", "wino_half_launches", "thin128_launches",
                     "attn64_launches", "mit_mlp_fused_launches", "ln_kernel_launches", "conv_launches", "sb_tensors", "forks", "fork_alloc_conflicts",
-                    "real_peak_bytes", "dry_peak_bytes", "cnx_rb_launches")
+                    "real_peak_bytes", "dry_peak_bytes", "cnx_rb_launches", "rb_qkv_launches")
 _STATUS = {0: "PF_OK", -1: "PF_ERR_ARG", -2: "PF_ERR_DEVICE", -3: "PF_ERR_WEIGHTS", -4: "PF_ERR_WORKSPACE"}
 
 _c = ctypes
@@ -87,6 +87,7 @@
     "pf_op_stem7x7": (_c.c_int, [_c.c_int, _P, _P, _c.c_int, _c.c_int, _c.c_int, _c.c_int, _P, _P, _c.c_int, _P, _P, _c.c_float, _c.c_int, _c.POINTER(_c.c_float), _P]),
     "pf_op_thin128": (_c.c_int, [_c.c_int, _P, _c.c_long, _P, _P, _P, _P, _c.c_int, _c.POINTER(_c.c_float), _P]),
     "pf_op_rb_srkv": (_c.c_int, [_c.c_int, _P, _c.c_int, _c.c_int, _c.c_int, _c.c_int, _P, _P, _c.c_float, _P, _P, _P, _P, _c.c_float, _P, _P, _P, _c.c_int, _c.POINTER(_c.c_float), _P]),
+    "pf_op_rb_qkv": (_c.c_int, [_c.c_int, _P, _c.c_int, _c.c_int, _c.c_int, _c.c_int, _P, _P, _c.c_float, _P, _P, _P, _P, _c.c_float, _P, _P, _P, _P, _P, _P, _c.c_int, _c.POINTER(_c.c_float), _P]),
     "pf_op_linear_ln": (_c.c_int, [_c.c_int, _P, _c.c_long, _c.c_int, _P, _P, _P, _P, _c.c_float, _c.c_int, _c.c_int, _P, _c.c_int, _P, _c.c_int, _P]),
     "pf_op_dwconv3x3_gelu_cfg": (_c.c_int, [_c.c_int, _P, _P, _P, _P, _c.c_int, _c.c_int, _c.c_int, _c.c_int, _P, _c.c_long, _c.c_int, _P]),
     "pf_op_dwconv7x7": (_c.c_int, [_c.c_int, _P, _P, _P, _P, _c.c_int, _c.c_int, _c.c_int, _c.c_int, _P]),
diff --git a/perspectivefields_amd/ops.py b/perspectivefields_amd/ops.py
--- a/perspectivefields_amd/ops.py
+++ b/perspectivefields_amd/ops.py
@@ -172,6 +172,23 @@
     return ms.value if iters > 0 else kv
 
 
+def rb_qkv(x, ln1_g, ln1_b, eps1, sr_w, sr_b, srn_g, srn_b, eps2, kv_w, kv_b, q_w, q_b, iters=0):
+    import torch
+
+    lib = load_library()
+    x = x.contiguous()
+    B, H, W, C = x.shape
+    if H % 2 or W % 2:
+        raise ValueError("rb_qkv: the token map must have even height and width")
+    kv = torch.empty((B, (H // 2) * (W // 2), 2 * C), dtype=torch.float32, device=x.device)
+    q = torch.empty((B, H * W, C), dtype=torch.float32, device=x.device)
+    ms = ctypes.c_float()
+    a = [_np(t) for t in (ln1_g, ln1_b, sr_w, sr_b, srn_g, srn_b, kv_w, kv_b, q_w, q_b)]
+    _check(lib.pf_op_rb_qkv(x.device.index, x.data_ptr(), B, H // 2, W // 2, C, _hp(a[0]), _hp(a[1]), float(eps1), _hp(a[2]), _hp(a[3]), _hp(a[4]), _hp(a[5]), float(eps2),
+                            _hp(a[6]), _hp(a[7]), _hp(a[8]), _hp(a[9]), kv.data_ptr(), q.data_ptr(), iters, ctypes.byref(ms), _stream_ptr()), None, "pf_op_rb_qkv")
+    return ms.value if iters > 0 else (kv, q)
+
+
 def mit_attn64(x, kv, ln_gamma, ln_beta, eps, q_w, q_b, proj_w, proj_b, iters=0, inplace=False):
     import torch
 
```

Result: no change. 1769 images/sec, median of 6 (+0.8%).
